# Fedomn/sqlrs

Hardware: AMD Instinct MI355X
Metric: Mrows/sec for filter->hash-join->group-by pipeline; achieved HBM GB/s vs peak (higher is better)
Workload: dtype int64 keys / f64 sum; 1 GPU; C5 filter(val>0.5) -> hash-join(fact x dim on int64 key) -> group-by(key) COUNT,SUM(f64); fact_rows=1000000000, dim_rows=10000000, groups=10000000, parallelism=single GPU

## Files before the change

### sqlrs_amd/csrc/agg_partition.hip

```cpp
#include <algorithm>
#include <cstdlib>
#include <cstring>

#include "agg_partition.hpp"
#include "device_utils.hpp"
#include "radix_part.hpp"

namespace sq {

#ifndef PART_WG_N
#define PART_WG_N 512
#endif
constexpr int PART_WG = PART_WG_N;
#ifndef DENSE_WG_N
#define DENSE_WG_N 1024
#endif
constexpr int DENSE_WG = DENSE_WG_N;
#ifndef HOT_MIN_PEERS_N
#define HOT_MIN_PEERS_N 8
#endif
constexpr int HOT_MIN_PEERS = HOT_MIN_PEERS_N;
constexpr uint64_t LDS_EMPTY = ~0ull;

__device__ __forceinline__ uint32_t bucket_of(uint64_t h, uint32_t P) {
// ... 196 lines not shown
}

struct SplitTables {
  unsigned long long *key = nullptr;
  unsigned int *first = nullptr;
  unsigned long long *acc = nullptr;
  uint32_t nsplit = 0;
};

__global__ void split_init_kernel(SplitTables stb, int64_t total, int n_acc, LdsAggParams prm) {
  int64_t i = blockIdx.x * (int64_t)blockDim.x + threadIdx.x;
  if (i >= total) return;
  stb.key[i] = LDS_EMPTY;
  stb.first[i] = 0xffffffffu;
  for (int a = 0; a < n_acc; a++) stb.acc[(size_t)a * total + i] = acc_identity_cell(prm.code[a] & 7);
}

__global__ void split_emit_kernel(SplitTables stb, uint32_t nslots, uint32_t cap, int n_acc,
                                  unsigned long long *out_count, uint64_t *__restrict__ gkey,
                                  uint32_t *__restrict__ gfirst, uint8_t *__restrict__ gvalid,
                                  uint64_t *__restrict__ gacc, int64_t gcap) {
  const int64_t total = (int64_t)stb.nsplit * nslots;
  int64_t i = blockIdx.x * (int64_t)blockDim.x + threadIdx.x;
  if (i >= total) return;
  unsigned int first = stb.first[i];
  if (first == 0xffffffffu) return;
  const uint32_t s = (uint32_t)(i % nslots);
  unsigned long long base = atomicAdd(out_count, 1ull);
  if ((int64_t)base >= gcap) return;
  gkey[base] = s == cap + 1 ? LDS_EMPTY : stb.key[i];
  gfirst[base] = first;
  if (gvalid) gvalid[base] = s == cap ? 0 : 1;
  for (int a = 0; a < n_acc; a++) gacc[(size_t)a * gcap + base] = stb.acc[(size_t)a * total + i];
}

template <int NV, bool FLAGS, bool JOIN, int NACC, int C0, int C1, bool PACK, bool REC = false>
__global__ __launch_bounds__(PART_WG) void lds_agg_kernel(
    LdsAggParams prm, const uint64_t *__restrict__ pk, const uint32_t *__restrict__ pi,
    const uint64_t *__restrict__ pv0, const uint64_t *__restrict__ pv1,
    const uint8_t *__restrict__ pf, const uint32_t *__restrict__ work , uint32_t P,
    int64_t n, unsigned long long *out_count, uint64_t *__restrict__ gkey,
    uint32_t *__restrict__ gfirst, uint8_t *__restrict__ gvalid, uint64_t *__restrict__ gacc,
    int64_t gcap, unsigned long long *ov_count, uint32_t *__restrict__ ov_rows,
    const uint64_t *__restrict__ bk, const uint8_t *__restrict__ bf, const uint32_t *__restrict__ bbstart,
    KeyPack kp, SplitTables stb) {
  extern __shared__ __attribute__((aligned(16))) unsigned long long tab[];
  __shared__ unsigned int s_cnt, s_join_fail;
  __shared__ unsigned long long s_base;
  const uint32_t b = work[4 * blockIdx.x];
  const int64_t lo = work[4 * blockIdx.x + 1];
  const int64_t hi = work[4 * blockIdx.x + 2];
  const uint32_t split = work[4 * blockIdx.x + 3];
  const uint32_t cap = prm.cap, mask = cap - 1, nslots = cap + 2;
  const int n_acc = NACC >= 0 ? NACC : prm.n_acc;
  auto code_of = [&](int a) { return NACC >= 0 ? (a == 0 ? C0 : C1) : prm.code[a]; };
  unsigned long long *tkey = tab;
  unsigned long long *tacc = tab + nslots;
  unsigned int *tfirst = (unsigned int *)(tacc + (size_t)n_acc * nslots);
  AggRows<NV> cur, nxt;
  if (lo < hi) {
    if (REC) lds_agg_load_rec<NV>(pk, lo + threadIdx.x, hi, cur);
    else lds_agg_load<NV, FLAGS, PACK>(pk, pi, pv0, pv1, pf, lo + threadIdx.x, hi, cur);
  }
  for (uint32_t s = threadIdx.x; s < nslots; s += PART_WG) {
    tkey[s] = LDS_EMPTY;
    tfirst[s] = 0xffffffffu;
#pragma unroll
    for (int a = 0; a < PART_MAX_ACC; a++) {
      if (a >= n_acc) break;
      tacc[(size_t)a * nslots + s] = acc_identity_cell(code_of(a) & 7);
    }
  }
  if (threadIdx.x == 0) {
    s_cnt = 0;
    s_join_fail = 0;
  }
  __syncthreads();
  if (JOIN) {
    if (*(volatile unsigned long long *)(ov_count + 1) != 0) return;
    const int64_t blo = bbstart[b], bhi = bbstart[b + 1];
    for (int64_t i = blo + threadIdx.x; i < bhi; i += PART_WG) {
      uint64_t key = bk[i];
      bool valid = bf ? (bf[i] & 1) : true;
      if (!valid) {
        if (atomicExch(&tkey[cap], 1ull) != LDS_EMPTY) s_join_fail = 1;
      } else if (key == LDS_EMPTY) {
        if (atomicExch(&tkey[cap + 1], 1ull) != LDS_EMPTY) s_join_fail = 1;
      } else {
        uint32_t s = slot_hash(key) & mask;
        uint32_t probes = 0;
        while (true) {
          unsigned long long prev = atomicCAS(&tkey[s], LDS_EMPTY, (unsigned long long)key);
          if (prev == key) s_join_fail = 1;
          if (prev == LDS_EMPTY || prev == key) break;
          s = (s + 1) & mask;
          if (++probes >= cap) {
            s_join_fail = 1;
            break;
          }
        }
      }
    }
    __syncthreads();
    if (s_join_fail) {
      if (threadIdx.x == 0) atomicExch(ov_count + 1, 1ull);
      return;
    }
  }
  __builtin_amdgcn_s_waitcnt(0x0F70);
  for (int64_t base = lo; base < hi; base += (int64_t)LDS_U * PART_WG) {
    const int64_t i0 = base + threadIdx.x;
    if (REC) lds_agg_load_rec<NV>(pk, i0 + (int64_t)LDS_U * PART_WG, hi, nxt);
    else lds_agg_load<NV, FLAGS, PACK>(pk, pi, pv0, pv1, pf, i0 + (int64_t)LDS_U * PART_WG, hi, nxt);
    uint32_t slot[LDS_U];
    unsigned long long seen[LDS_U];
    uint32_t sentinel = 0;
    if (PACK) {
#pragma unroll
      for (int u = 0; u < LDS_U; u++) {
        if (!JOIN && packed_off(kp, cur.k[u]) == kp.kmask) sentinel |= 1u << u;
        cur.id[u] = packed_row(kp, cur.k[u]);
        cur.k[u] = packed_key(kp, cur.k[u]);
      }
    }
#pragma unroll
    for (int u = 0; u < LDS_U; u++) {
      uint32_t s = slot_hash(cur.k[u]) & mask;
      if (FLAGS && !(cur.f[u] & 1)) s = cap;
      else if (cur.k[u] == LDS_EMPTY) s = cap + 1;
      slot[u] = s;
      seen[u] = tkey[s];
    }
#pragma unroll
    for (int u = 0; u < LDS_U; u++) {
      bool act = i0 + (int64_t)u * PART_WG < hi && !((sentinel >> u) & 1u);
      const uint64_t key = cur.k[u];
      uint32_t s = slot[u];
      unsigned long long c = seen[u];
      if (act) {
        if (s >= cap) {
          if (JOIN && c == LDS_EMPTY) act = false;
        } else if (JOIN) {
          uint32_t probes = 0;
          while (c != key && c != LDS_EMPTY && ++probes < cap) {
            s = (s + 1) & mask;
            c = tkey[s];
          }
          if (c != key) act = false;
        } else {
          uint32_t probes = 0;
          while (true) {
            if (c == key) break;
            if (c == LDS_EMPTY) {
              unsigned long long prev = atomicCAS(&tkey[s], LDS_EMPTY, (unsigned long long)key);
              if (prev == LDS_EMPTY || prev == key) break;
            }
            s = (s + 1) & mask;
            if (++probes >= cap) {
              unsigned long long o = atomicAdd(ov_count, 1ull);
              ov_rows[o] = cur.id[u];
              act = false;
              break;
            }
            c = tkey[s];
          }
        }
      }
      const uint64_t actm = __ballot(act);
      if (actm) {
        const int first = __builtin_ctzll(actm);
        const uint32_t s0 = (uint32_t)__shfl((int)s, first, 64);
        const bool hot = act && s == s0;
        const uint64_t peers = __ballot(hot);
        if (__popcll(peers) >= HOT_MIN_PEERS) {
          const uint32_t idmin = wave_min_u32_dpp(hot ? cur.id[u] : 0xffffffffu);
          if (lane_id() == first) atomicMin(&tfirst[s0], idmin);
#pragma unroll
          for (int a = 0; a < PART_MAX_ACC; a++) {
            if (a >= n_acc) break;
            const int code = code_of(a), kind = code & 7, src = code >> 3;
            const bool in = hot && (!FLAGS || (cur.f[u] & (2 << src)));
            const uint64_t v = (NV >= 2 && src) ? cur.v1[u] : cur.v0[u];
            unsigned long long *cell = tacc + (size_t)a * nslots + s0;
            const uint64_t inm = __ballot(in);
            uint64_t red;
            switch (kind) {
            case AK_COUNT: red = (uint64_t)__popcll(inm); break;
            case AK_SUM_I64: red = wave_sum_u64_dpp(in ? v : 0ull); break;
            case AK_SUM_F64: red = (uint64_t)__double_as_longlong(wave_sum_f64_dpp(in ? __longlong_as_double((long long)v) : 0.0)); break;
            case AK_MIN_I64: red = wave_min_u64(in ? i64_to_ordered((int64_t)v) : ~0ull); break;
            case AK_MIN_F64: red = wave_min_u64(in ? f64_to_ordered(__longlong_as_double((long long)v)) : ~0ull); break;
            case AK_MAX_I64: red = wave_max_u64(in ? i64_to_ordered((int64_t)v) : 0ull); break;
            default: red = wave_max_u64(in ? f64_to_ordered(__longlong_as_double((long long)v)) : 0ull);
            }
            if (lane_id() == first && inm) {
              switch (kind) {
              case AK_COUNT:
              case AK_SUM_I64: atomicAdd(cell, (unsigned long long)red); break;
              case AK_SUM_F64: unsafeAtomicAdd((double *)cell, __longlong_as_double((long long)red)); break;
              case AK_MIN_I64:
              case AK_MIN_F64: atomicMin(cell, (unsigned long long)red); break;
              default: atomicMax(cell, (unsigned long long)red);
              }
            }
          }
          act = act && !hot;
        }
      }
      if (act) {
        if (cur.id[u] < tfirst[s]) atomicMin(&tfirst[s], cur.id[u]);
#pragma unroll
        for (int a = 0; a < PART_MAX_ACC; a++) {
          if (a >= n_acc) break;
          const int code = code_of(a);
          const int src = code >> 3;
          if (FLAGS && !(cur.f[u] & (2 << src))) continue;
          uint64_t v = (NV >= 2 && src) ? cur.v1[u] : cur.v0[u];
          acc_apply(code & 7, tacc + (size_t)a * nslots + s, v);
        }
      }
    }
    cur = nxt;
  }
  __syncthreads();
  if (split != 0xffffffffu) {
    unsigned long long *gk = stb.key + (size_t)split * nslots;
    unsigned int *gf = stb.first + (size_t)split * nslots;
    for (uint32_t s = threadIdx.x; s < nslots; s += PART_WG) {
      unsigned int first = tfirst[s];
      if (first == 0xffffffffu) continue;
      uint32_t g = s;
      bool placed = true;
      if (s < cap) {
        const unsigned long long key = tkey[s];
        g = slot_hash(key) & mask;
        uint32_t probes = 0;
        while (true) {
          unsigned long long prev = atomicCAS(&gk[g], LDS_EMPTY, key);
          if (prev == LDS_EMPTY || prev == key) break;
          g = (g + 1) & mask;
          if (++probes >= cap) {
            placed = false;
            break;
          }
        }
      }
      if (!placed) {
        unsigned long long o = atomicAdd(out_count, 1ull);
        if ((int64_t)o < gcap) {
          gkey[o] = tkey[s];
          gfirst[o] = first;
          if (gvalid) gvalid[o] = 1;
#pragma unroll
          for (int a = 0; a < PART_MAX_ACC; a++) {
            if (a >= n_acc) break;
            gacc[(size_t)a * gcap + o] = tacc[(size_t)a * nslots + s];
          }
        }
        atomicExch(ov_count + 2, 1ull);
        continue;
      }
      atomicMin(&gf[g], first);
#pragma unroll
      for (int a = 0; a < PART_MAX_ACC; a++) {
        if (a >= n_acc) break;
        unsigned long long *cell = stb.acc + ((size_t)a * stb.nsplit + split) * nslots + g;
        const unsigned long long v = tacc[(size_t)a * nslots + s];
        switch (code_of(a) & 7) {
        case AK_COUNT:
        case AK_SUM_I64: atomicAdd(cell, v); break;
        case AK_SUM_F64: unsafeAtomicAdd((double *)cell, __longlong_as_double((long long)v)); break;
        case AK_MIN_I64:
        case AK_MIN_F64: atomicMin(cell, v); break;
        default: atomicMax(cell, v);
        }
      }
    }
    return;
  }
  unsigned int mine = 0;
  for (uint32_t s = threadIdx.x; s < nslots; s += PART_WG) mine += tfirst[s] != 0xffffffffu;
  unsigned int my_off = atomicAdd(&s_cnt, mine);
  __syncthreads();
  if (threadIdx.x == 0) s_base = atomicAdd(out_count, (unsigned long long)s_cnt);
  __syncthreads();
  unsigned long long base = s_base + my_off;
  for (uint32_t s = threadIdx.x; s < nslots; s += PART_WG) {
    unsigned int first = tfirst[s];
    if (first == 0xffffffffu) continue;
    if ((int64_t)base < gcap) {
      gkey[base] = s == cap + 1 ? LDS_EMPTY : tkey[s];
      gfirst[base] = first;
      if (gvalid) gvalid[base] = s == cap ? 0 : 1;
#pragma unroll
      for (int a = 0; a < PART_MAX_ACC; a++) {
        if (a >= n_acc) break;
        gacc[(size_t)a * gcap + base] = tacc[(size_t)a * nslots + s];
      }
    }
    base++;
  }
}

constexpr int SED_SLOTS = 16, SED_GROUPS = 16;
__global__ __launch_bounds__(SED_SLOTS * SED_GROUPS) void split_emit_dense_kernel(
    SplitTables stb, const uint32_t *__restrict__ split_bucket, const uint32_t *__restrict__ chunk_lo, uint32_t nbuckets_split,
    uint32_t R, KeyPack kp, LdsAggParams prm, int n_acc, unsigned long long *out_count, uint64_t *__restrict__ gkey,
    uint32_t *__restrict__ gfirst, uint64_t *__restrict__ gacc, int64_t gcap) {
  __shared__ unsigned int s_first[SED_GROUPS][SED_SLOTS];
  __shared__ unsigned long long s_acc[PART_MAX_ACC][SED_GROUPS][SED_SLOTS];
  const uint32_t tiles_per_bucket = (R + SED_SLOTS - 1) / SED_SLOTS;
  const uint32_t t = blockIdx.x / tiles_per_bucket, sl = threadIdx.x % SED_SLOTS, cg = threadIdx.x / SED_SLOTS;
  const uint32_t s = (blockIdx.x % tiles_per_bucket) * SED_SLOTS + sl;
  if (t >= nbuckets_split) return;
  const int64_t total = (int64_t)stb.nsplit * R;
  unsigned int first = 0xffffffffu;
  unsigned long long acc[PART_MAX_ACC];
  for (int a = 0; a < n_acc; a++) acc[a] = acc_identity_cell(prm.code[a] & 7);
  if (s < R) {
    const uint32_t c1 = chunk_lo[t + 1];
    for (uint32_t c = chunk_lo[t] + cg; c < c1; c += SED_GROUPS) {
      const unsigned int f = stb.first[(size_t)c * R + s];
      if (f == 0xffffffffu) continue;
      first = min(first, f);
      for (int a = 0; a < n_acc; a++) {
        const unsigned long long v = stb.acc[(size_t)a * total + (size_t)c * R + s];
        switch (prm.code[a] & 7) {
        case AK_COUNT:
        case AK_SUM_I64: acc[a] += v; break;
        case AK_SUM_F64: acc[a] = (unsigned long long)__double_as_longlong(__longlong_as_double((long long)acc[a]) + __longlong_as_double((long long)v)); break;
        case AK_MIN_I64:
        case AK_MIN_F64: acc[a] = min(acc[a], v); break;
        default: acc[a] = max(acc[a], v);
        }
      }
    }
  }
  s_first[cg][sl] = first;
  for (int a = 0; a < n_acc; a++) s_acc[a][cg][sl] = acc[a];
  __syncthreads();
  if (cg != 0 || s >= R) return;
  for (int g = 1; g < SED_GROUPS; g++) {
    const unsigned int f = s_first[g][sl];
    if (f == 0xffffffffu) continue;
    first = min(first, f);
    for (int a = 0; a < n_acc; a++) {
      const unsigned long long v = s_acc[a][g][sl];
      switch (prm.code[a] & 7) {
      case AK_COUNT:
      case AK_SUM_I64: acc[a] += v; break;
      case AK_SUM_F64: acc[a] = (unsigned long long)__double_as_longlong(__longlong_as_double((long long)acc[a]) + __longlong_as_double((long long)v)); break;
      case AK_MIN_I64:
      case AK_MIN_F64: acc[a] = min(acc[a], v); break;
      default: acc[a] = max(acc[a], v);
      }
    }
  }
  if (first == 0xffffffffu) return;
  unsigned int mlt = 1;
  if (prm.partner_mult) mlt = prm.partner_mult[((uint64_t)split_bucket[t] << kp.rbits) + s];
  unsigned long long base = atomicAdd(out_count, 1ull);
  if ((int64_t)base >= gcap) return;
  gkey[base] = kp.kmin + ((uint64_t)split_bucket[t] << kp.rbits) + s;
  gfirst[base] = first;
  for (int a = 0; a < n_acc; a++) gacc[(size_t)a * gcap + base] = prm.partner_mult ? acc_times(prm.code[a] & 7, acc[a], mlt) : acc[a];
}

template <int NV, bool JOIN, int NACC, int C0, int C1, bool REC = false>
__global__ __launch_bounds__(DENSE_WG) void lds_agg_dense_kernel(
    LdsAggParams prm, const uint64_t *__restrict__ pk, const uint64_t *__restrict__ pv0,
    const uint32_t *__restrict__ work, unsigned long long *out_count, uint64_t *__restrict__ gkey,
    uint32_t *__restrict__ gfirst, uint64_t *__restrict__ gacc, int64_t gcap, KeyPack kp, SplitTables stb) {
  extern __shared__ __attribute__((aligned(16))) unsigned long long tab[];
  __shared__ unsigned int s_cnt;
  __shared__ unsigned long long s_base;
  const uint32_t b = work[4 * blockIdx.x];
  const int64_t lo = work[4 * blockIdx.x + 1];
  const int64_t hi = work[4 * blockIdx.x + 2];
  const uint32_t split = work[4 * blockIdx.x + 3];
  const uint32_t R = prm.cap, mask = R - 1;
  const int n_acc = NACC >= 0 ? NACC : prm.n_acc;
  auto code_of = [&](int a) { return NACC >= 0 ? (a == 0 ? C0 : C1) : prm.code[a]; };
  unsigned long long *tacc = tab;
  unsigned int *tfirst = (unsigned int *)(tacc + (size_t)n_acc * R);
  AggRows<NV> cur, nxt;
  if (lo < hi) {
    if (REC) lds_agg_load_rec<NV, DENSE_WG>(pk, lo + threadIdx.x, hi, cur);
    else lds_agg_load<NV, false, true, DENSE_WG>(pk, nullptr, pv0, nullptr, nullptr, lo + threadIdx.x, hi, cur);
  }
  for (uint32_t s = threadIdx.x; s < R; s += DENSE_WG) {
    tfirst[s] = 0xffffffffu;
#pragma unroll
    for (int a = 0; a < PART_MAX_ACC; a++) {
      if (a >= n_acc) break;
      tacc[(size_t)a * R + s] = acc_identity_cell(code_of(a) & 7);
    }
  }
  if (threadIdx.x == 0) s_cnt = 0;
  __syncthreads();
  uint32_t hc_slot = 0xffffffffu, hc_min = 0xffffffffu;
  uint64_t hc_acc[PART_MAX_ACC];
  auto hot_flush = [&]() {
    if (hc_slot == 0xffffffffu) return;
    if (lane_id() == 0) {
      atomicMin(&tfirst[hc_slot], hc_min);
#pragma unroll
      for (int a = 0; a < PART_MAX_ACC; a++) {
        if (a >= n_acc) break;
        unsigned long long *cell = tacc + (size_t)a * R + hc_slot;
        switch (code_of(a) & 7) {
        case AK_COUNT:
        case AK_SUM_I64: atomicAdd(cell, (unsigned long long)hc_acc[a]); break;
        case AK_SUM_F64: unsafeAtomicAdd((double *)cell, __longlong_as_double((long long)hc_acc[a])); break;
        case AK_MIN_I64:
        case AK_MIN_F64: atomicMin(cell, (unsigned long long)hc_acc[a]); break;
        default: atomicMax(cell, (unsigned long long)hc_acc[a]);
        }
      }
    }
    hc_slot = 0xffffffffu;
  };
  auto hot_take = [&](uint32_t s0, uint32_t idmin) {
    if (hc_slot != s0) {
      hot_flush();
      hc_slot = s0;
      hc_min = 0xffffffffu;
#pragma unroll
      for (int a = 0; a < PART_MAX_ACC; a++) {
        if (a >= n_acc) break;
        hc_acc[a] = acc_identity_cell(code_of(a) & 7);
      }
    }
    hc_min = idmin < hc_min ? idmin : hc_min;
  };
  auto hot_add = [&](int a, int kind, uint64_t red) {
    switch (kind) {
    case AK_COUNT:
    case AK_SUM_I64: hc_acc[a] += red; break;
    case AK_SUM_F64: hc_acc[a] = (uint64_t)__double_as_longlong(__longlong_as_double((long long)hc_acc[a]) + __longlong_as_double((long long)red)); break;
    case AK_MIN_I64:
    case AK_MIN_F64: hc_acc[a] = red < hc_acc[a] ? red : hc_acc[a]; break;
    default: hc_acc[a] = red > hc_acc[a] ? red : hc_acc[a];
    }
  };
  __builtin_amdgcn_s_waitcnt(0x0F70);
  for (int64_t base = lo; base < hi; base += (int64_t)LDS_U * DENSE_WG) {
    const int64_t i0 = base + threadIdx.x;
    if (REC) lds_agg_load_rec<NV, DENSE_WG>(pk, i0 + (int64_t)LDS_U * DENSE_WG, hi, nxt);
    else lds_agg_load<NV, false, true, DENSE_WG>(pk, nullptr, pv0, nullptr, nullptr, i0 + (int64_t)LDS_U * DENSE_WG, hi, nxt);
#pragma unroll
    for (int u = 0; u < LDS_U; u++) {
      const uint64_t off = packed_off(kp, cur.k[u]);
      const uint32_t id = packed_row(kp, cur.k[u]);
      const uint32_t s = (uint32_t)off & mask;
      bool act = i0 + (int64_t)u * DENSE_WG < hi;
      act = act && off <= kp.range;
      const uint64_t actm = __ballot(act);
      if (actm) {
        const int first = __builtin_ctzll(actm);
        const uint32_t s0 = (uint32_t)__shfl((int)s, first, 64);
        const bool hot = act && s == s0;
        const uint64_t peers = __ballot(hot);
        if (__popcll(peers) >= HOT_MIN_PEERS) {
          const uint32_t idmin = wave_min_u32_dpp(hot ? id : 0xffffffffu);
          hot_take(s0, idmin);
#pragma unroll
          for (int a = 0; a < PART_MAX_ACC; a++) {
            if (a >= n_acc) break;
            const int kind = code_of(a) & 7;
            const uint64_t v = NV >= 1 ? cur.v0[u] : 0ull;
            uint64_t red;
            switch (kind) {
            case AK_COUNT: red = (uint64_t)__popcll(peers); break;
            case AK_SUM_I64: red = wave_sum_u64_dpp(hot ? v : 0ull); break;
            case AK_SUM_F64: red = (uint64_t)__double_as_longlong(wave_sum_f64_dpp(hot ? __longlong_as_double((long long)v) : 0.0)); break;
            case AK_MIN_I64: red = wave_min_u64(hot ? i64_to_ordered((int64_t)v) : ~0ull); break;
            case AK_MIN_F64: red = wave_min_u64(hot ? f64_to_ordered(__longlong_as_double((long long)v)) : ~0ull); break;
            case AK_MAX_I64: red = wave_max_u64(hot ? i64_to_ordered((int64_t)v) : 0ull); break;
            default: red = wave_max_u64(hot ? f64_to_ordered(__longlong_as_double((long long)v)) : 0ull);
            }
            hot_add(a, kind, red);
          }
          act = act && !hot;
        }
      }
      if (act) {
        if (id < tfirst[s]) atomicMin(&tfirst[s], id);
#pragma unroll
        for (int a = 0; a < PART_MAX_ACC; a++) {
          if (a >= n_acc) break;
          acc_apply(code_of(a) & 7, tacc + (size_t)a * R + s, NV >= 1 ? cur.v0[u] : 0ull);
        }
      }
    }
    cur = nxt;
  }
  hot_flush();
  __syncthreads();
  if (JOIN && (prm.partner_bits || prm.partner_mult)) {
    const uint64_t off0 = (uint64_t)b << kp.rbits;
    for (uint32_t s = threadIdx.x; s < R; s += DENSE_WG) {
      if (tfirst[s] == 0xffffffffu) continue;
      const uint64_t o = off0 + s;
      const bool partner = prm.partner_mult ? prm.partner_mult[o] != 0 : (((prm.partner_bits[o >> 6] >> (o & 63)) & 1ull) != 0);
      if (!partner) tfirst[s] = 0xffffffffu;
    }
  }
  if (split != 0xffffffffu) {
    unsigned int *gf = stb.first + (size_t)split * R;
    for (uint32_t s = threadIdx.x; s < R; s += DENSE_WG) {
      gf[s] = tfirst[s];
#pragma unroll
      for (int a = 0; a < PART_MAX_ACC; a++) {
        if (a >= n_acc) break;
        stb.acc[((size_t)a * stb.nsplit + split) * R + s] = tacc[(size_t)a * R + s];
      }
    }
    return;
  }
  unsigned int mine = 0;
  for (uint32_t s = threadIdx.x; s < R; s += DENSE_WG) mine += tfirst[s] != 0xffffffffu;
  unsigned int my_off = atomicAdd(&s_cnt, mine);
  __syncthreads();
  if (threadIdx.x == 0) s_base = atomicAdd(out_count, (unsigned long long)s_cnt);
  __syncthreads();
  unsigned long long base = s_base + my_off;
  const uint64_t key0 = kp.kmin + ((uint64_t)b << kp.rbits);
  for (uint32_t s = threadIdx.x; s < R; s += DENSE_WG) {
    unsigned int first = tfirst[s];
    if (first == 0xffffffffu) continue;
    if ((int64_t)base < gcap) {
      gkey[base] = key0 + s;
      gfirst[base] = first;
      const unsigned int mlt = (JOIN && prm.partner_mult) ? prm.partner_mult[((uint64_t)b << kp.rbits) + s] : 1u;
#pragma unroll
      for (int a = 0; a < PART_MAX_ACC; a++) {
        if (a >= n_acc) break;
        const unsigned long long cell = tacc[(size_t)a * R + s];
        gacc[(size_t)a * gcap + base] = (JOIN && prm.partner_mult) ? acc_times(code_of(a) & 7, cell, mlt) : cell;
      }
    }
    base++;
  }
}

struct SlimBucketIn {
  SlimRowsView rows;
  const uint32_t *nzstart, *nzbt, *nzcount, *bcol;
  uint32_t tile;
  uint32_t groups;
  const uint32_t *blk_bt;
  uint32_t log_b;
};
constexpr uint32_t SLIM_BT_CAP = 4096;
struct SlimAggRows {
  uint64_t v[LDS_U];
  uint32_t w[LDS_U], bt[LDS_U];
};

template <bool JOIN, int NACC, int C0, int C1, bool BLK = false>
__global__ __launch_bounds__(DENSE_WG) void lds_agg_dense_slim_kernel(
    LdsAggParams prm, SlimBucketIn in, const uint32_t *__restrict__ work, unsigned long long *out_count,
    uint64_t *__restrict__ gkey, uint32_t *__restrict__ gfirst, uint64_t *__restrict__ gacc, int64_t gcap, KeyPack kp,
    SplitTables stb) {
  extern __shared__ __attribute__((aligned(16))) unsigned long long tab[];
  __shared__ unsigned int s_cnt, s_before, s_inside;
  __shared__ unsigned long long s_base;
  __shared__ uint32_t s_wsum[DENSE_WG / 64];
  const uint32_t b = work[4 * blockIdx.x];
  const int64_t lo = work[4 * blockIdx.x + 1];
  const int64_t hi = work[4 * blockIdx.x + 2];
  const uint32_t split = work[4 * blockIdx.x + 3];
  const uint32_t R = prm.cap, mask = R - 1;
  const int n_acc = NACC >= 0 ? NACC : prm.n_acc;
  auto code_of = [&](int a) { return NACC >= 0 ? (a == 0 ? C0 : C1) : prm.code[a]; };
  unsigned long long *tacc = tab;
  unsigned int *tfirst = (unsigned int *)(tacc + (size_t)n_acc * R);
  unsigned long long *gmask = (unsigned long long *)(tfirst + R);
  uint32_t *gpre = (uint32_t *)(gmask + in.groups);
  uint32_t *gbt = gpre + in.groups;
  const uint32_t col = BLK ? 0u : in.bcol[b], nruns = BLK ? 0u : in.nzcount[b];
  const uint32_t ngroups = BLK ? 0u : (uint32_t)((hi - lo + 63) >> 6);
  const uint64_t le_mask = (2ull << lane_id()) - 1ull;
  const uint32_t rbits = kp.rbits, lmask = (1u << 13) - 1u;

  for (uint32_t s = threadIdx.x; s < R; s += DENSE_WG) {
    tfirst[s] = 0xffffffffu;
#pragma unroll
    for (int a = 0; a < PART_MAX_ACC; a++) {
      if (a >= n_acc) break;
      tacc[(size_t)a * R + s] = acc_identity_cell(code_of(a) & 7);
    }
  }
  for (uint32_t g = threadIdx.x; g < ngroups; g += DENSE_WG) gmask[g] = 0;
  if (threadIdx.x == 0) {
    s_cnt = 0;
    s_before = 0;
    s_inside = 0;
  }
  __syncthreads();
  if (!BLK) {
    uint32_t before = 0, inside = 0;
    for (uint32_t k = threadIdx.x; k < nruns; k += DENSE_WG) {
      const int64_t st = in.nzstart[col + k];
      if (st <= lo) before++;
      else if (st < hi) {
        inside++;
        atomicOr(&gmask[(st - lo) >> 6], 1ull << ((st - lo) & 63));
      }
    }
    before = wave_sum_u32(before);
    inside = wave_sum_u32(inside);
    if (lane_id() == 0 && before) atomicAdd(&s_before, before);
    if (lane_id() == 0 && inside) atomicAdd(&s_inside, inside);
  }
  __syncthreads();
  const uint32_t k_first = s_before - 1u, k_count = s_inside + 1u;
  const bool bt_lds = !BLK && k_count <= SLIM_BT_CAP;
  const bool seg_mode = NACC == 2 && ((C0 == AK_COUNT && C1 == AK_SUM_F64) || (C0 == AK_SUM_F64 && C1 == AK_COUNT)) &&
                        hi - lo >= 4096 && (int64_t)k_count * 2048 <= hi - lo && !prm.seg_off && !BLK;
  if (bt_lds)
    for (uint32_t k = threadIdx.x; k < k_count; k += DENSE_WG) gbt[k] = in.nzbt[col + min(k_first + k, nruns - 1)];
  if (!BLK) {
    constexpr uint32_t GPT = 8;
    uint32_t carry = s_before - 1u;
    for (uint32_t g0 = 0; g0 < ngroups; g0 += DENSE_WG * GPT) {
      const uint32_t gb = g0 + threadIdx.x * GPT;
      uint32_t pc[GPT], sum = 0;
#pragma unroll
      for (uint32_t i = 0; i < GPT; i++) {
        pc[i] = gb + i < ngroups ? (uint32_t)__popcll(gmask[gb + i]) : 0u;
        sum += pc[i];
      }
      const uint32_t inc = wave_iscan_u32(sum);
      if (lane_id() == 63) s_wsum[wave_id()] = inc;
      __syncthreads();
      uint32_t wbase = 0, tot = 0;
      for (int w = 0; w < DENSE_WG / 64; w++) {
        if (w < wave_id()) wbase += s_wsum[w];
        tot += s_wsum[w];
      }
      uint32_t run = carry + wbase + inc - sum;
#pragma unroll
      for (uint32_t i = 0; i < GPT; i++) {
        if (gb + i < ngroups) gpre[gb + i] = run;
        run += pc[i];
      }
      carry += tot;
      __syncthreads();
    }
  }
#ifndef SLIM_WAVE_SPAN
#define SLIM_WAVE_SPAN 1
#endif
  constexpr int64_t SLIM_USTEP = SLIM_WAVE_SPAN ? 64 : DENSE_WG;
  const int64_t slim_toff = SLIM_WAVE_SPAN ? (int64_t)wave_id() * (LDS_U * 64) + lane_id() : (int64_t)threadIdx.x;
  auto load = [&](int64_t i0, SlimAggRows &r) {
#pragma unroll
    for (int u = 0; u < LDS_U; u++) {
      const int64_t i = min(i0 + (int64_t)u * SLIM_USTEP, hi - 1);
      slim_load_nt(in.rows, i, r.w[u], r.v[u]);
      if (BLK) {
        r.bt[u] = in.blk_bt[i >> in.log_b];
        continue;
      }
      const uint32_t g = (uint32_t)((i - lo) >> 6);
      const uint32_t k = gpre[g] + (uint32_t)__popcll(gmask[g] & le_mask);
#if defined(SLIM_DBG) && (SLIM_DBG & 16)
      r.bt[u] = k;
#else
      r.bt[u] = bt_lds ? gbt[min(k - k_first, k_count - 1)] : in.nzbt[col + min(k, nruns - 1)];
#endif
    }
  };
  uint32_t hc_slot = 0xffffffffu, hc_min = 0xffffffffu;
  uint64_t hc_acc[PART_MAX_ACC];
  auto hot_flush = [&]() {
    if (hc_slot == 0xffffffffu) return;
    if (lane_id() == 0) {
      atomicMin(&tfirst[hc_slot], hc_min);
#pragma unroll
      for (int a = 0; a < PART_MAX_ACC; a++) {
        if (a >= n_acc) break;
        unsigned long long *cell = tacc + (size_t)a * R + hc_slot;
        switch (code_of(a) & 7) {
        case AK_COUNT:
        case AK_SUM_I64: atomicAdd(cell, (unsigned long long)hc_acc[a]); break;
        case AK_SUM_F64: unsafeAtomicAdd((double *)cell, __longlong_as_double((long long)hc_acc[a])); break;
        case AK_MIN_I64:
        case AK_MIN_F64: atomicMin(cell, (unsigned long long)hc_acc[a]); break;
        default: atomicMax(cell, (unsigned long long)hc_acc[a]);
        }
      }
    }
    hc_slot = 0xffffffffu;
  };
  auto hot_take = [&](uint32_t s0, uint32_t idmin) {
    if (hc_slot != s0) {
      hot_flush();
      hc_slot = s0;
      hc_min = 0xffffffffu;
#pragma unroll
      for (int a = 0; a < PART_MAX_ACC; a++) {
        if (a >= n_acc) break;
        hc_acc[a] = acc_identity_cell(code_of(a) & 7);
      }
    }
    hc_min = idmin < hc_min ? idmin : hc_min;
  };
  auto hot_add = [&](int a, int kind, uint64_t red) {
    switch (kind) {
    case AK_COUNT:
    case AK_SUM_I64: hc_acc[a] += red; break;
    case AK_SUM_F64: hc_acc[a] = (uint64_t)__double_as_longlong(__longlong_as_double((long long)hc_acc[a]) + __longlong_as_double((long long)red)); break;
    case AK_MIN_I64:
    case AK_MIN_F64: hc_acc[a] = red < hc_acc[a] ? red : hc_acc[a]; break;
    default: hc_acc[a] = red > hc_acc[a] ? red : hc_acc[a];
    }
  };
  SlimAggRows cur, nxt;
  if (lo < hi) load(lo + slim_toff, cur);
  __builtin_amdgcn_s_waitcnt(0x0F70);
  for (int64_t base = lo; base < hi; base += (int64_t)LDS_U * DENSE_WG) {
    const int64_t i0 = base + slim_toff;
    load(i0 + (int64_t)LDS_U * DENSE_WG, nxt);
    uint32_t sl[LDS_U], id[LDS_U], tf[LDS_U];
#pragma unroll
    for (int u = 0; u < LDS_U; u++) {
      const uint32_t w = cur.w[u];
      sl[u] = w & mask;
      id[u] = (cur.bt[u] + (w >> (rbits + 13))) * in.tile + ((w >> rbits) & lmask);
      tf[u] = tfirst[sl[u]];
    }
    constexpr bool SEG_CAPABLE = NACC == 2 && ((C0 == AK_COUNT && C1 == AK_SUM_F64) || (C0 == AK_SUM_F64 && C1 == AK_COUNT));
    const int lane = (int)lane_id();
    auto seg_rows = [&](bool act, uint32_t sl_u, uint64_t v_u, uint32_t id_u, uint32_t tf_u) {
      const uint32_t key = act ? sl_u : (0x80000000u | (uint32_t)lane);
      const uint32_t prevk = (uint32_t)__builtin_amdgcn_update_dpp(0, (int)key, 0x138, 0xf, 0xf, false);
      const uint64_t bm = __ballot(lane == 0 || key != prevk);
      const int headl = 63 - __builtin_clzll(bm & le_mask);
      double incl = act ? __longlong_as_double((long long)v_u) : 0.0;
      uint32_t idh = act ? id_u : 0xffffffffu;
      wave_seg_iscan_f64_min_u32(incl, idh, headl, lane);
      const bool tail = act && (lane == 63 || ((bm >> (lane + 1)) & 1ull));
      if (tail) {
        const uint32_t s = sl_u;
        if (idh < tf_u) atomicMin(&tfirst[s], idh);
        atomicAdd(tacc + (size_t)(C0 == AK_COUNT ? 0 : 1) * R + s, (unsigned long long)(lane - headl + 1));
        unsafeAtomicAdd((double *)(tacc + (size_t)(C0 == AK_COUNT ? 1 : 0) * R + s), incl);
      }
    };
    if (seg_mode) {
#pragma unroll
      for (int u = 0; u < LDS_U; u++) {
        const bool act = i0 + (int64_t)u * SLIM_USTEP < hi;
        {
          const uint32_t s0 = (uint32_t)__builtin_amdgcn_readfirstlane((int)sl[u]);
          if (__ballot(act && sl[u] == s0) == ~0ull) {
            hot_take(s0, wave_min_u32_dpp(id[u]));
            hot_add(C0 == AK_COUNT ? 0 : 1, AK_COUNT, 64ull);
            hot_add(C0 == AK_COUNT ? 1 : 0, AK_SUM_F64, (uint64_t)__double_as_longlong(wave_sum_f64_dpp(__longlong_as_double((long long)cur.v[u]))));
            continue;
          }
        }
        seg_rows(act, sl[u], cur.v[u], id[u], tf[u]);
      }
      cur = nxt;
      continue;
    }
#pragma unroll
    for (int u = 0; u < LDS_U; u++) {
      const uint32_t s = sl[u];
      bool act = i0 + (int64_t)u * SLIM_USTEP < hi;
      if (BLK) act = act && cur.w[u] != 0xffffffffu;
#ifdef SLIM_DBG
      uint64_t actm = (SLIM_DBG & 1) ? 0ull : __ballot(act);
#else
      uint64_t actm = __ballot(act);
#endif
      for (int it = 0; it < 3 && actm; it++) {
        const int first = __builtin_ctzll(actm);
        const uint32_t s0 = (uint32_t)__builtin_amdgcn_readlane((int)s, first);
        const bool hot = act && s == s0;
        const uint64_t peers = __ballot(hot);
        if (__popcll(peers) < HOT_MIN_PEERS) break;
        if (SEG_CAPABLE && it == 0 && peers != actm && (((peers >> first) + 1) & (peers >> first)) == 0 && !prm.seg_off) {
          seg_rows(act, s, cur.v[u], id[u], tf[u]);
          act = false;
          break;
        }
        const uint32_t idmin = wave_min_u32_dpp(hot ? id[u] : 0xffffffffu);
        hot_take(s0, idmin);
#pragma unroll
        for (int a = 0; a < PART_MAX_ACC; a++) {
          if (a >= n_acc) break;
          const int kind = code_of(a) & 7;
          const uint64_t v = cur.v[u];
          uint64_t red;
          switch (kind) {
          case AK_COUNT: red = (uint64_t)__popcll(peers); break;
          case AK_SUM_I64: red = wave_sum_u64_dpp(hot ? v : 0ull); break;
          case AK_SUM_F64: red = (uint64_t)__double_as_longlong(wave_sum_f64_dpp(hot ? __longlong_as_double((long long)v) : 0.0)); break;
          case AK_MIN_I64: red = wave_min_u64(hot ? i64_to_ordered((int64_t)v) : ~0ull); break;
          case AK_MIN_F64: red = wave_min_u64(hot ? f64_to_ordered(__longlong_as_double((long long)v)) : ~0ull); break;
          case AK_MAX_I64: red = wave_max_u64(hot ? i64_to_ordered((int64_t)v) : 0ull); break;
          default: red = wave_max_u64(hot ? f64_to_ordered(__longlong_as_double((long long)v)) : 0ull);
          }
          hot_add(a, kind, red);
        }
        act = act && !hot;
        actm &= ~peers;
      }
      if (act) {
#ifdef SLIM_DBG
        if (!(SLIM_DBG & 8) && id[u] < tf[u]) atomicMin(&tfirst[s], id[u]);
#pragma unroll
        for (int a = 0; a < PART_MAX_ACC; a++) {
          if (a >= n_acc) break;
          if ((SLIM_DBG >> (1 + a)) & 1) continue;
          acc_apply(code_of(a) & 7, tacc + (size_t)a * R + s, cur.v[u]);
        }
#else
        if (id[u] < tf[u]) atomicMin(&tfirst[s], id[u]);
#pragma unroll
        for (int a = 0; a < PART_MAX_ACC; a++) {
          if (a >= n_acc) break;
          acc_apply(code_of(a) & 7, tacc + (size_t)a * R + s, cur.v[u]);
        }
#endif
      }
    }
    cur = nxt;
  }
  hot_flush();
  __syncthreads();
  if (JOIN && (prm.partner_bits || prm.partner_mult)) {
    const uint64_t off0 = (uint64_t)b << kp.rbits;
    for (uint32_t s = threadIdx.x; s < R; s += DENSE_WG) {
      if (tfirst[s] == 0xffffffffu) continue;
      const uint64_t o = off0 + s;
      const bool partner = prm.partner_mult ? prm.partner_mult[o] != 0 : (((prm.partner_bits[o >> 6] >> (o & 63)) & 1ull) != 0);
      if (!partner) tfirst[s] = 0xffffffffu;
    }
  }
  if (split != 0xffffffffu) {
    unsigned int *gf = stb.first + (size_t)split * R;
    for (uint32_t s = threadIdx.x; s < R; s += DENSE_WG) {
      gf[s] = tfirst[s];
#pragma unroll
      for (int a = 0; a < PART_MAX_ACC; a++) {
        if (a >= n_acc) break;
        stb.acc[((size_t)a * stb.nsplit + split) * R + s] = tacc[(size_t)a * R + s];
      }
    }
    return;
  }
  unsigned int mine = 0;
  for (uint32_t s = threadIdx.x; s < R; s += DENSE_WG) mine += tfirst[s] != 0xffffffffu;
  unsigned int my_off = atomicAdd(&s_cnt, mine);
  __syncthreads();
  if (threadIdx.x == 0) s_base = atomicAdd(out_count, (unsigned long long)s_cnt);
  __syncthreads();
  unsigned long long obase = s_base + my_off;
  const uint64_t key0 = kp.kmin + ((uint64_t)b << kp.rbits);
  for (uint32_t s = threadIdx.x; s < R; s += DENSE_WG) {
    unsigned int first = tfirst[s];
    if (first == 0xffffffffu) continue;
    if ((int64_t)obase < gcap) {
      gkey[obase] = key0 + s;
      gfirst[obase] = first;
      const unsigned int mlt = (JOIN && prm.partner_mult) ? prm.partner_mult[((uint64_t)b << kp.rbits) + s] : 1u;
#pragma unroll
      for (int a = 0; a < PART_MAX_ACC; a++) {
        if (a >= n_acc) break;
        const unsigned long long cell = tacc[(size_t)a * R + s];
        gacc[(size_t)a * gcap + obase] = (JOIN && prm.partner_mult) ? acc_times(code_of(a) & 7, cell, mlt) : cell;
      }
    }
    obase++;
  }
}

__global__ void first_to_rowid_kernel(const uint32_t *__restrict__ gfirst, int64_t n, uint64_t offset,
                                      uint64_t *__restrict__ out) {
  int64_t i = blockIdx.x * (int64_t)blockDim.x + threadIdx.x;
  if (i < n) out[i] = offset + gfirst[i];
}
__global__ void bytes_pack_kernel(const uint8_t *__restrict__ bytes, int64_t n, uint64_t *__restrict__ out) {
  int64_t i = blockIdx.x * (int64_t)blockDim.x + threadIdx.x;
  bool b = (i < n) && bytes[i];
  uint64_t m = __ballot(b);
  if (lane_id() == 0 && i < n) out[i >> 6] = m;
}

__global__ __launch_bounds__(256) void key_range_kernel(const uint64_t *__restrict__ keys, int64_t n, unsigned long long *mm) {
  uint64_t kmin = ~0ull, kmax = 0;
  for (int64_t r = blockIdx.x * (int64_t)blockDim.x + threadIdx.x; r < n; r += (int64_t)gridDim.x * blockDim.x) {
    const uint64_t o = keys[r] ^ (1ull << 63);
    kmin = min(kmin, o);
    kmax = max(kmax, o);
  }
  kmin = wave_min_u64(kmin);
  kmax = wave_max_u64(kmax);
  __shared__ unsigned long long s_lo[4], s_hi[4];
  if (lane_id() == 0) {
    s_lo[wave_id()] = kmin;
    s_hi[wave_id()] = kmax;
  }
  __syncthreads();
  if (threadIdx.x == 0) {
    for (int w = 1; w < 4; w++) {
      kmin = min(kmin, (uint64_t)s_lo[w]);
      kmax = max(kmax, (uint64_t)s_hi[w]);
    }
    atomicMin(mm, (unsigned long long)kmin);
    atomicMax(mm + 1, (unsigned long long)kmax);
  }
}

const uint64_t *part_row_ids(Ctx *ctx, PartAggOutput &po) {
  if (!po.row_ids) {
    const int64_t g1 = std::max<int64_t>(po.groups, 1);
    po.row_ids = ctx->alloc(8 * (size_t)g1);
    if (po.groups) {
      first_to_rowid_kernel<<<dim3((unsigned)ceil_div(g1, 256)), dim3(256), 0, ctx->stream>>>(
          po.gfirst->as<uint32_t>(), po.groups, po.row_offset, po.row_ids->as<uint64_t>());
      SQ_HIP(hipGetLastError());
    }
  }
  return po.row_ids->as<uint64_t>();
}

bool partitioned_preaggregate(Ctx *ctx, const PartAggSpec &spec, const PartAggInput &in,
                              uint64_t row_offset, PartAggOutput *out) {
  int64_t n = in.n;
  if (n > 0xffffffffll || spec.n_acc > PART_MAX_ACC || spec.nv > 2) return false;
  const bool join_mode = in.join_keys != nullptr;
  uint64_t omin = ~0ull, omax = 0;
  bool sampled = false;
  const char *kse = hook("SQLRS_KEY_STATS_EXACT");
  const bool stats_exact_env = kse && kse[0] == '1';
  double est = join_mode ? (double)in.join_n
                         : estimate_distinct(ctx, in.keys, in.key_validity, n, &omin, &omax, (in.exact_stats || stats_exact_env) ? nullptr : &sampled);
  BufP ctr = ctx->alloc_zero(48);
  if (sampled && omin <= omax) {
    const uint64_t w = omax - omin, pad = std::max<uint64_t>(w / 8, 65536);
    omin = omin >= pad ? omin - pad : 0;
    omax = omax <= ~0ull - pad ? omax + pad : ~0ull;
  }
  static const double est_scale = [] {
    const char *e = hook("SQLRS_EST_SCALE");
    return e ? std::atof(e) : 1.0;
  }();
  if (!join_mode) est = std::max(1.0, est * est_scale);
  KeyPack kp;
  const bool nullable = in.key_validity || in.val_validity[0] || in.val_validity[1];
  if (!nullable && spec.nv <= 1 && !(join_mode && in.join_validity)) {
    if (join_mode && in.join_range_known) {
      omin = in.join_omin;
      omax = in.join_omax;
    } else if (join_mode) {
      BufP mm = ctx->alloc(16);
      SQ_HIP(hipMemsetAsync(mm->p, 0xff, 8, ctx->stream));
      SQ_HIP(hipMemsetAsync(mm->as<uint8_t>() + 8, 0, 8, ctx->stream));
      unsigned blocks = (unsigned)std::min<int64_t>(ceil_div(in.join_n, 1024), 1024);
      key_range_kernel<<<dim3(std::max(blocks, 1u)), dim3(256), 0, ctx->stream>>>(
          in.join_keys, in.join_n, mm->as<unsigned long long>());
      SQ_HIP(hipGetLastError());
      const uint64_t *h = (const uint64_t *)ctx->fetch(mm->p, 16);
      omin = h[0];
      omax = h[1];
    }
    if (omin <= omax) {
      uint64_t range = omax - omin;
      uint32_t kbits = 1;
      while (kbits < 64 && ((1ull << kbits) - 1) <= range) kbits++;
      int rowbits = 1;
      while (rowbits < 32 && (1ll << rowbits) < n) rowbits++;
      if (kbits + rowbits <= 64) {
        kp.kbits = kbits;
        kp.kmask = (1ull << kbits) - 1;
        kp.kmin = omin ^ (1ull << 63);
        if (sampled) {
          kp.oob = (unsigned int *)(ctr->as<uint64_t>() + 4);
          out->ov_rows = ctx->alloc(4 * (size_t)std::max<int64_t>(n, 1));
          kp.ov_rows = out->ov_rows->as<uint32_t>();
          kp.ov_count = ctr->as<unsigned long long>() + 1;
          kp.ov_cap = (uint32_t)std::min<int64_t>(n, std::max<int64_t>(65536, n / 1024));
        }
      }
    }
  }
  constexpr size_t lds_budget = 72 * 1024;
  const size_t slot_bytes = 8 + 8 * (size_t)spec.n_acc + 4;
  uint32_t cap = 1;
  while ((size_t)(cap * 2 + 2) * slot_bytes <= lds_budget) cap *= 2;
  constexpr double load_factor = 0.275;
  const double groups_per_table = cap * load_factor;
  double want = est * 1.15 / groups_per_table;
  if (!join_mode) est = std::min(est, (double)n);
  const char *dense_e = hook("SQLRS_DENSE_AGG");
  const bool dense_on = !(dense_e && dense_e[0] == '0');
  const uint64_t *partner_bits = nullptr;
  const double want_hashed = want;
  bool dense = false;
  if (dense_on && kp.kbits) {
    const uint64_t range = omax - omin;
    constexpr size_t dense_budget = 150 * 1024;
    const size_t dslot = 8 * (size_t)spec.n_acc + 4;
    uint32_t rbits = 8;
    while (rbits < 14 && ((size_t)2 << rbits) * dslot <= dense_budget) rbits++;
    while (rbits > 8 && (range >> (rbits - 1)) == 0) rbits--;
    const uint64_t pd = (range >> rbits) + 1;
    const bool fills = join_mode ? (in.join_unique_known && (range + 1 == (uint64_t)in.join_n ||
                                                             ((in.join_bits || in.join_mult) && in.join_range_known && range / 16 <= (uint64_t)in.join_n)))
                                 : ((double)range + 1.0 <= 4.0 * est);
    partner_bits = (join_mode && fills && !in.join_mult && range + 1 != (uint64_t)in.join_n) ? in.join_bits : nullptr;
    if (fills && pd <= 65536 && (double)pd <= 1.5 * std::max(1.0, std::ceil(want))) {
      dense = true;
      kp.dense = 1;
      kp.rbits = rbits;
      kp.range = range;
      cap = 1u << rbits;
      want = (double)pd;
    }
  }
  if (join_mode && in.join_mult && !dense) return false;
  if (want > 65536.0) return false;
  uint32_t P = (uint32_t)std::max(1.0, std::ceil(want));
  out->est_groups = est;
  PartitionInput pin;
  pin.pack = kp;
  pin.filter = in.filter;
  pin.keys = in.keys;
  pin.key_validity = in.key_validity;
  pin.n = n;
  pin.nv = spec.nv;
  for (int k = 0; k < 2; k++) {
    pin.vals[k] = in.vals[k];
    pin.val_validity[k] = in.val_validity[k];
  }
  PartitionedRows pr;
  const bool in_place = P == 1 && !join_mode && !nullable && want_hashed <= 1.0 && !in.filter.col;
  if (in_place) {
    dense = false;
    kp = KeyPack();
    cap = 1;
    while ((size_t)(cap * 2 + 2) * slot_bytes <= lds_budget) cap *= 2;
    pr.n = n;
    pr.P = 1;
    auto borrowed = [&](const void *p) {
      BufP b = std::make_shared<Buf>(ctx, const_cast<void *>(p), 0);
      b->owned = false;
      return b;
    };
    pr.key = borrowed(in.keys);
    pr.v0 = spec.nv >= 1 ? borrowed(in.vals[0]) : nullptr;
    pr.v1 = spec.nv >= 2 ? borrowed(in.vals[1]) : nullptr;
    pr.bstart_host = {0u, (uint32_t)n};
    pr.bstart = nullptr;
  } else if (!partition_rows(ctx, pin, P, &pr)) {
    return false;
  }
  P = pr.P;
  n = pr.n;
  if (dense != (pr.pack.dense != 0)) return false;
  if (n == 0) {
    out->groups = out->n_overflow = 0;
    out->gcap = 1;
    out->buckets = (int)P;
    out->gkey = ctx->alloc(8);
    out->gfirst = ctx->alloc(4);
    out->gacc = ctx->alloc(8 * (size_t)std::max(spec.n_acc, 1));
    out->ov_rows = ctx->alloc(4);
    out->row_ids = nullptr;
    out->row_offset = row_offset;
    return true;
  }
  out->buckets = (int)P;
  BufP pk = pr.key, pi = pr.idx, pv0 = pr.v0, pv1 = pr.v1, pf = pr.flags;
  PartitionedRows local_build;
  const PartitionedRows *bp = nullptr;
  if (join_mode && !dense) {
    if (in.join_cache && in.join_cache->P == P && in.join_cache->n == in.join_n) {
      bp = in.join_cache;
    } else {
      PartitionInput bin;
      bin.keys = in.join_keys;
      bin.key_validity = in.join_validity;
      bin.n = in.join_n;
      bin.nv = 0;
      bin.build_side = true;
      PartitionedRows *dst = in.join_cache ? in.join_cache : &local_build;
      if (!partition_rows(ctx, bin, P, dst) || dst->P != P) return false;
      bp = dst;
    }
  }
  LdsAggParams prm;
  prm.n_acc = spec.n_acc;
  for (int a = 0; a < PART_MAX_ACC; a++) {
    int kind = AK_COUNT;
    if (a < spec.n_acc) {
      switch (spec.op[a]) {
      case PART_COUNT: kind = AK_COUNT; break;
      case PART_SUM_I64: kind = AK_SUM_I64; break;
      case PART_SUM_F64: kind = AK_SUM_F64; break;
      case PART_MIN: kind = spec.kind[a] ? AK_MIN_F64 : AK_MIN_I64; break;
      default: kind = spec.kind[a] ? AK_MAX_F64 : AK_MAX_I64;
      }
    }
    prm.code[a] = a < spec.n_acc ? (kind | (spec.src[a] << 3)) : 0;
  }
  prm.cap = cap;
  prm.partner_bits = dense ? (const unsigned long long *)partner_bits : nullptr;
  prm.partner_mult = (dense && join_mode) ? in.join_mult : nullptr;
  {
    const char *seg_e = hook("SQLRS_AGG_SEG");
    prm.seg_off = (seg_e && seg_e[0] == '0') ? 1 : 0;
  }
  int64_t gcap = (int64_t)std::min<double>((double)n, est * 1.5 + 65536.0 + 2.0 * P);
  if (dense) gcap = (int64_t)std::min<uint64_t>((uint64_t)n, join_mode ? (uint64_t)in.join_n : kp.range + 1);
  size_t lds = dense ? round_up((size_t)cap * (slot_bytes - 8), 16) : round_up((size_t)(cap + 2) * slot_bytes, 16);
  const std::vector<uint32_t> &hb = pr.bstart_host;
  if (hb.size() != (size_t)P + 1) return false;
  uint32_t chunk = (uint32_t)std::max<int64_t>(32768, 2 * (n / std::max<uint32_t>(P, 1)));
  uint32_t split_above = chunk;
  if (dense) {
    int64_t nonempty_d = 0;
    for (uint32_t bkt = 0; bkt < P; bkt++) nonempty_d += pr.bucket_end(bkt) > hb[bkt];
    const int64_t avg = n / std::max<int64_t>(nonempty_d, 1);
    const char *cd_e = hook("SQLRS_DENSE_CHUNK_DIV");
    const int cdiv = cd_e ? std::max(1, std::atoi(cd_e)) : 2;
    constexpr int sa_pct = 125;
    chunk = (uint32_t)std::max<int64_t>(32768, avg / cdiv);
    split_above = (uint32_t)std::max<int64_t>(65536, avg * sa_pct / 100);
  }
  {
    const uint32_t slots = (lds > 80 * 1024 - 64 ? 1u : 2u) * (uint32_t)ctx->num_cus;
    uint32_t nonempty = 0;
    for (uint32_t bkt = 0; bkt < P; bkt++) nonempty += pr.bucket_end(bkt) > hb[bkt];
    if (nonempty < slots / 2) {
      chunk = (uint32_t)std::max<int64_t>(32768, n / (2 * (int64_t)slots));
      split_above = chunk;
    }
  }
  if (pr.slim.on && !pr.slim.blk_bt) {
    const size_t table = round_up((size_t)cap * (slot_bytes - 8), 16);
    const size_t room = 159 * 1024 > table + 4 * SLIM_BT_CAP ? 159 * 1024 - table - 4 * SLIM_BT_CAP : 0;
    const uint32_t item_rows = (uint32_t)std::min<size_t>(1u << 18, (room / 12 > 2 ? room / 12 - 2 : 0) * 64);
    if (item_rows < 16384) return false;
    chunk = std::min(chunk, item_rows);
    split_above = std::min(split_above, item_rows);
  }
  std::vector<uint32_t> work, split_bucket, chunk_lo;
  work.reserve(4 * ((size_t)P + 64));
  out->may_dup = false;
  uint32_t nsplit = 0, nchunk_tables = 0;
  for (uint32_t bkt = 0; bkt < P; bkt++) {
    uint32_t lo = hb[bkt], hi = pr.bucket_end(bkt);
    if (dense && lo == hi) continue;
    if (hi - lo <= split_above) {
      work.insert(work.end(), {bkt, lo, hi, 0xffffffffu});
    } else if (dense) {
      chunk_lo.push_back(nchunk_tables);
      const uint32_t pieces = (uint32_t)ceil_div((int64_t)(hi - lo), (int64_t)chunk);
      for (uint32_t q = 0; q < pieces; q++) {
        const uint32_t c0 = lo + (uint32_t)((uint64_t)(hi - lo) * q / pieces), c1 = lo + (uint32_t)((uint64_t)(hi - lo) * (q + 1) / pieces);
        work.insert(work.end(), {bkt, c0, c1, nchunk_tables++});
      }
      split_bucket.push_back(bkt);
      nsplit++;
    } else {
      for (uint32_t c0 = lo; c0 < hi; c0 += chunk) work.insert(work.end(), {bkt, c0, std::min(hi, c0 + chunk), nsplit});
      split_bucket.push_back(bkt);
      nsplit++;
    }
  }
  chunk_lo.push_back(nchunk_tables);
  if (nsplit) {
    std::vector<uint32_t> ord(work.size() / 4), sorted(work.size());
    for (uint32_t i = 0; i < ord.size(); i++) ord[i] = i;
    std::stable_sort(ord.begin(), ord.end(), [&](uint32_t a, uint32_t b) {
      return work[4 * a + 2] - work[4 * a + 1] > work[4 * b + 2] - work[4 * b + 1];
    });
    for (size_t i = 0; i < ord.size(); i++) std::memcpy(&sorted[4 * i], &work[4 * ord[i]], 16);
    work.swap(sorted);
  }
  const uint32_t nwork = (uint32_t)(work.size() / 4);
  BufP dwork = ctx->alloc(4 * work.size() + 16);
  SQ_HIP(hipMemcpyAsync(dwork->p, work.data(), 4 * work.size(), hipMemcpyHostToDevice, ctx->stream));
  const uint32_t nslots_h = dense ? cap : cap + 2;
  SplitTables stb;
  BufP stb_key, stb_first, stb_acc, dsplit;
  BufP dchunk_lo;
  if (nsplit && dense) {
    const int64_t total = (int64_t)nchunk_tables * nslots_h;
    stb_first = ctx->alloc(4 * (size_t)total);
    stb_acc = ctx->alloc(8 * (size_t)total * (size_t)std::max(spec.n_acc, 1));
    stb.first = stb_first->as<unsigned int>();
    stb.acc = stb_acc->as<unsigned long long>();
    stb.nsplit = nchunk_tables;
    dsplit = ctx->alloc(4 * (size_t)nsplit);
    dchunk_lo = ctx->alloc(4 * ((size_t)nsplit + 1));
    SQ_HIP(hipMemcpyAsync(dsplit->p, split_bucket.data(), 4 * (size_t)nsplit, hipMemcpyHostToDevice, ctx->stream));
    SQ_HIP(hipMemcpyAsync(dchunk_lo->p, chunk_lo.data(), 4 * ((size_t)nsplit + 1), hipMemcpyHostToDevice, ctx->stream));
  } else if (nsplit) {
    const int64_t total = (int64_t)nsplit * nslots_h;
    stb_key = ctx->alloc(8 * (size_t)total);
    stb_first = ctx->alloc(4 * (size_t)total);
    stb_acc = ctx->alloc(8 * (size_t)total * (size_t)std::max(spec.n_acc, 1));
    stb.key = stb_key->as<unsigned long long>();
    stb.first = stb_first->as<unsigned int>();
    stb.acc = stb_acc->as<unsigned long long>();
    stb.nsplit = nsplit;
    split_init_kernel<<<dim3((unsigned)ceil_div(total, 256)), dim3(256), 0, ctx->stream>>>(stb, total, spec.n_acc, prm);
    SQ_HIP(hipGetLastError());
  }
  out->gkey = ctx->alloc(8 * (size_t)gcap);
  out->gfirst = ctx->alloc(4 * (size_t)gcap);
  out->gvalid = in.key_validity ? ctx->alloc((size_t)gcap) : nullptr;
  out->gacc = ctx->alloc(8 * (size_t)gcap * (size_t)std::max(spec.n_acc, 1));
  out->gcap = gcap;
  if (!out->ov_rows) out->ov_rows = ctx->alloc(4 * (size_t)std::max<int64_t>(n, 1));
  ctx->agg_route[pr.pack.kbits ? Ctx::AR_PACKED : Ctx::AR_UNPACKED]++;
  ctx->agg_route[Ctx::AR_FLAGS] += pf != nullptr;
  ctx->agg_route[Ctx::AR_REC] += pr.rec != nullptr;
  ctx->agg_route[Ctx::AR_IN_PLACE] += in_place;
  ctx->agg_route[Ctx::AR_JOIN] += join_mode;
  ctx->agg_route[Ctx::AR_JOIN_MULT] += prm.partner_mult != nullptr;
  ctx->agg_route[Ctx::AR_SPLIT] += nsplit > 0;
  {
    ProfScope ps(ctx, "lds_agg");
#define SQ_LA(NV, FL, JN, NA, C0, C1, PK)                                                                        \
  do {                                                                                                         \
    auto kfn = lds_agg_kernel<NV, FL, JN, NA, C0, C1, PK>;                                                      \
    constexpr bool can_rec = NV == 1 && PK && !FL;                                                             \
    if (can_rec && pr.rec) kfn = lds_agg_kernel<NV, FL, JN, NA, C0, C1, PK, can_rec>;                          \
    else if (pr.rec) fail(SQLRS_ERR_INTERNAL, "record-form partition in a column-form bucket pass");           \
    allow_big_lds(ctx, kfn);                                                                                   \
    kfn<<<dim3(nwork), dim3(PART_WG), lds, ctx->stream>>>(                                                     \
        prm, pr.rec ? pr.rec->as<uint64_t>() : pk->as<uint64_t>(), pi ? pi->as<uint32_t>() : nullptr, pv0 ? pv0->as<uint64_t>() : nullptr,       \
        pv1 ? pv1->as<uint64_t>() : nullptr, pf ? pf->as<uint8_t>() : nullptr, dwork->as<uint32_t>(), P, n,    \
        ctr->as<unsigned long long>(), out->gkey->as<uint64_t>(), out->gfirst->as<uint32_t>(),                 \
        out->gvalid ? out->gvalid->as<uint8_t>() : nullptr, out->gacc->as<uint64_t>(), gcap,                   \
        ctr->as<unsigned long long>() + 1, out->ov_rows->as<uint32_t>(),                                       \
        bp ? bp->key->as<uint64_t>() : nullptr, (bp && bp->flags) ? bp->flags->as<uint8_t>() : nullptr,        \
        bp ? bp->bstart->as<uint32_t>() : nullptr, pr.pack, stb);                                              \
    ctx->agg_route[NA < 0 ? Ctx::AR_PROBE_GENERIC : Ctx::AR_PROBE_SPEC]++;                                     \
    launched = true;                                                                                           \
  } while (0)
#define SQ_LA_J(NV, FL, NA, C0, C1)                                                                            \
  do {                                                                                                         \
    if (pr.pack.kbits) {                                                                                       \
      if (join_mode) SQ_LA(NV, FL, true, NA, C0, C1, true);                                                    \
      else SQ_LA(NV, FL, false, NA, C0, C1, true);                                                             \
    } else {                                                                                                   \
      if (join_mode) SQ_LA(NV, FL, true, NA, C0, C1, false);                                                   \
      else SQ_LA(NV, FL, false, NA, C0, C1, false);                                                            \
    }                                                                                                          \
  } while (0)
    const int nvu = pv1 ? 2 : ((pv0 || pr.rec) ? 1 : 0);
    bool launched = false;
    if (dense && pr.slim.on) {
      uint32_t max_item = 64;
      for (uint32_t i = 0; i < nwork; i++) max_item = std::max(max_item, work[4 * i + 2] - work[4 * i + 1]);
      const bool blk = pr.slim.blk_bt != nullptr;
      SlimBucketIn sb;
      sb.rows = pr.slim.rows;
      sb.nzstart = blk ? nullptr : pr.slim.nzstart->as<uint32_t>();
      sb.nzbt = blk ? nullptr : pr.slim.nzbt->as<uint32_t>();
      sb.nzcount = blk ? nullptr : pr.slim.nzcount->as<uint32_t>();
      sb.bcol = blk ? nullptr : pr.slim.bcol->as<uint32_t>();
      sb.tile = pr.slim.tile;
      sb.groups = blk ? 0u : (uint32_t)ceil_div((int64_t)max_item, 64) + 1;
      sb.blk_bt = blk ? pr.slim.blk_bt->as<uint32_t>() : nullptr;
      sb.log_b = pr.slim.log_b;
      const size_t slds = round_up((size_t)cap * (slot_bytes - 8), 16) + (blk ? 16 : 12 * (size_t)sb.groups + 4 * SLIM_BT_CAP);
#define SQ_LS(JN, NA, C0, C1)                                                                                  \
  do {                                                                                                         \
    auto kfn = lds_agg_dense_slim_kernel<JN, NA, C0, C1>;                                                       \
    if (blk) kfn = lds_agg_dense_slim_kernel<JN, NA, C0, C1, true>;                                             \
    allow_big_lds(ctx, kfn, 159 * 1024);                                                                                 \
    kfn<<<dim3(nwork), dim3(DENSE_WG), slds, ctx->stream>>>(prm, sb, dwork->as<uint32_t>(), ctr->as<unsigned long long>(), \
                                                           out->gkey->as<uint64_t>(), out->gfirst->as<uint32_t>(), \
                                                           out->gacc->as<uint64_t>(), gcap, pr.pack, stb);        \
    ctx->agg_route[blk ? Ctx::AR_SLIM_BLK : Ctx::AR_SLIM_RUNS]++;                                              \
    ctx->agg_route[Ctx::AR_INTERPRETED] += NA < 0;                                                             \
    launched = true;                                                                                           \
  } while (0)
#define SQ_LS_J(NA, C0, C1) do { if (join_mode) SQ_LS(true, NA, C0, C1); else SQ_LS(false, NA, C0, C1); } while (0)
      const int c0 = prm.code[0], c1 = spec.n_acc == 2 ? prm.code[1] : -1;
      if (spec.n_acc == 2 && c0 == AK_COUNT && c1 == AK_SUM_F64) SQ_LS_J(2, AK_COUNT, AK_SUM_F64);
      else if (spec.n_acc == 2 && c0 == AK_SUM_F64 && c1 == AK_COUNT) SQ_LS_J(2, AK_SUM_F64, AK_COUNT);
      else if (spec.n_acc == 1 && c0 == AK_SUM_F64) SQ_LS_J(1, AK_SUM_F64, 0);
      else if (spec.n_acc == 1 && c0 == AK_COUNT) SQ_LS_J(1, AK_COUNT, 0);
      else SQ_LS_J(-1, 0, 0);
#undef SQ_LS_J
#undef SQ_LS
      if (nsplit) {
        split_emit_dense_kernel<<<dim3((unsigned)(nsplit * ceil_div((int64_t)nslots_h, SED_SLOTS))), dim3(SED_SLOTS * SED_GROUPS), 0, ctx->stream>>>(
            stb, dsplit->as<uint32_t>(), dchunk_lo->as<uint32_t>(), nsplit, cap, pr.pack, prm, spec.n_acc,
            ctr->as<unsigned long long>(), out->gkey->as<uint64_t>(), out->gfirst->as<uint32_t>(), out->gacc->as<uint64_t>(), gcap);
      }
    } else if (dense) {
#define SQ_LD(NV, JN, NA, C0, C1)                                                                              \
  do {                                                                                                         \
    auto kfn = lds_agg_dense_kernel<NV, JN, NA, C0, C1>;                                                        \
    if (NV == 1 && pr.rec) kfn = lds_agg_dense_kernel<NV, JN, NA, C0, C1, NV == 1>;                            \
    allow_big_lds(ctx, kfn);                                                                                   \
    kfn<<<dim3(nwork), dim3(DENSE_WG), lds, ctx->stream>>>(                                                    \
        prm, pr.rec ? pr.rec->as<uint64_t>() : pk->as<uint64_t>(), pv0 ? pv0->as<uint64_t>() : nullptr, dwork->as<uint32_t>(), \
        ctr->as<unsigned long long>(), out->gkey->as<uint64_t>(), out->gfirst->as<uint32_t>(),                 \
        out->gacc->as<uint64_t>(), gcap, pr.pack, stb);                                                        \
    ctx->agg_route[Ctx::AR_DENSE]++;                                                                           \
    ctx->agg_route[Ctx::AR_INTERPRETED] += NA < 0;                                                             \
    launched = true;                                                                                           \
  } while (0)
#define SQ_LD_J(NV, NA, C0, C1) do { if (join_mode) SQ_LD(NV, true, NA, C0, C1); else SQ_LD(NV, false, NA, C0, C1); } while (0)
      if (nvu == 1 && spec.n_acc <= 2) {
        const int c0 = prm.code[0], c1 = spec.n_acc == 2 ? prm.code[1] : -1;
#define SQ_SIG1(K) if (!launched && spec.n_acc == 1 && c0 == K) SQ_LD_J(1, 1, K, 0)
#define SQ_SIG2(K0, K1) if (!launched && spec.n_acc == 2 && c0 == K0 && c1 == K1) SQ_LD_J(1, 2, K0, K1)
        SQ_SIG1(AK_COUNT); SQ_SIG1(AK_SUM_I64); SQ_SIG1(AK_SUM_F64); SQ_SIG1(AK_MIN_I64); SQ_SIG1(AK_MIN_F64);
        SQ_SIG1(AK_MAX_I64); SQ_SIG1(AK_MAX_F64);
        SQ_SIG2(AK_COUNT, AK_SUM_F64); SQ_SIG2(AK_SUM_F64, AK_COUNT);
        SQ_SIG2(AK_COUNT, AK_SUM_I64); SQ_SIG2(AK_SUM_I64, AK_COUNT);
        SQ_SIG2(AK_MIN_F64, AK_MAX_F64); SQ_SIG2(AK_MIN_I64, AK_MAX_I64);
#undef SQ_SIG1
#undef SQ_SIG2
      }
      if (!launched) { if (nvu == 0) SQ_LD_J(0, -1, 0, 0); else SQ_LD_J(1, -1, 0, 0); }
#undef SQ_LD_J
#undef SQ_LD
      if (nsplit) {
        split_emit_dense_kernel<<<dim3((unsigned)(nsplit * ceil_div((int64_t)nslots_h, SED_SLOTS))), dim3(SED_SLOTS * SED_GROUPS), 0, ctx->stream>>>(
            stb, dsplit->as<uint32_t>(), dchunk_lo->as<uint32_t>(), nsplit, cap, pr.pack, prm, spec.n_acc,
            ctr->as<unsigned long long>(), out->gkey->as<uint64_t>(), out->gfirst->as<uint32_t>(), out->gacc->as<uint64_t>(), gcap);
      }
    }
    if (!launched && !pf && nvu == 1 && spec.n_acc <= 2) {
      const int c0 = prm.code[0], c1 = spec.n_acc == 2 ? prm.code[1] : -1;
#define SQ_SIG1(K) if (!launched && spec.n_acc == 1 && c0 == K) SQ_LA_J(1, false, 1, K, 0)
#define SQ_SIG2(K0, K1) if (!launched && spec.n_acc == 2 && c0 == K0 && c1 == K1) SQ_LA_J(1, false, 2, K0, K1)
      SQ_SIG1(AK_COUNT); SQ_SIG1(AK_SUM_I64); SQ_SIG1(AK_SUM_F64); SQ_SIG1(AK_MIN_I64); SQ_SIG1(AK_MIN_F64);
      SQ_SIG1(AK_MAX_I64); SQ_SIG1(AK_MAX_F64);
      SQ_SIG2(AK_COUNT, AK_SUM_F64); SQ_SIG2(AK_SUM_F64, AK_COUNT);
      SQ_SIG2(AK_COUNT, AK_SUM_I64); SQ_SIG2(AK_SUM_I64, AK_COUNT);
      SQ_SIG2(AK_MIN_F64, AK_MAX_F64); SQ_SIG2(AK_MIN_I64, AK_MAX_I64);
#undef SQ_SIG1
#undef SQ_SIG2
    }
    if (!launched) {
      if (pf) { if (nvu == 0) SQ_LA_J(0, true, -1, 0, 0); else if (nvu == 1) SQ_LA_J(1, true, -1, 0, 0); else SQ_LA_J(2, true, -1, 0, 0); }
      else { if (nvu == 0) SQ_LA_J(0, false, -1, 0, 0); else if (nvu == 1) SQ_LA_J(1, false, -1, 0, 0); else SQ_LA_J(2, false, -1, 0, 0); }
    }
#undef SQ_LA_J
#undef SQ_LA
    if (nsplit && !dense) {
      const int64_t total = (int64_t)nsplit * nslots_h;
      split_emit_kernel<<<dim3((unsigned)ceil_div(total, 256)), dim3(256), 0, ctx->stream>>>(
          stb, nslots_h, cap, spec.n_acc, ctr->as<unsigned long long>(), out->gkey->as<uint64_t>(),
          out->gfirst->as<uint32_t>(), out->gvalid ? out->gvalid->as<uint8_t>() : nullptr,
          out->gacc->as<uint64_t>(), gcap);
    }
    SQ_HIP(hipGetLastError());
  }
  const uint64_t *h = (const uint64_t *)ctx->fetch(ctr->p, 40);
  if (h[4]) {
    out->retry_exact = true;
    return false;
  }
  out->groups = (int64_t)h[0];
  out->n_overflow = (int64_t)h[1];
  ctx->agg_route[Ctx::AR_OVERFLOW_ROWS] += out->n_overflow;
  out->may_dup = h[3] != 0;
  if (join_mode && h[2]) return false;
  if (out->groups > gcap) return false;
  int64_t g1 = std::max<int64_t>(out->groups, 1);
  out->row_offset = row_offset;
  out->row_ids = nullptr;
  if (out->groups) {
    if (out->gvalid) {
      out->gvalid_bits = ctx->alloc(bitmap_bytes(g1));
      int64_t g64 = (int64_t)round_up((size_t)g1, 64);
      bytes_pack_kernel<<<dim3((unsigned)ceil_div(g64, 256)), dim3(256), 0, ctx->stream>>>(
          out->gvalid->as<uint8_t>(), out->groups, out->gvalid_bits->as<uint64_t>());
    }
    SQ_HIP(hipGetLastError());
  }
  return true;
}

}
```

### sqlrs_amd/csrc/agg_partition.hpp

```cpp
#pragma once

#include <cmath>

#include "common.hpp"
#include "prims.hpp"
#include "radix_part.hpp"

namespace sq {

constexpr int PART_MAX_ACC = 6;
enum PartOp { PART_COUNT = 0, PART_SUM_I64 = 1, PART_SUM_F64 = 2, PART_MIN = 3, PART_MAX = 4 };

struct PartAggSpec {
  int n_acc = 0;
  int op[PART_MAX_ACC] = {0};
  int src[PART_MAX_ACC] = {0};
  int kind[PART_MAX_ACC] = {0};
  int nv = 0;
};

struct PartAggInput {
  const uint64_t *keys = nullptr;
  const uint64_t *key_validity = nullptr;
  int64_t n = 0;
  const void *vals[2] = {nullptr, nullptr};
  const uint64_t *val_validity[2] = {nullptr, nullptr};
  const uint64_t *join_keys = nullptr;
  const uint64_t *join_validity = nullptr;
  int64_t join_n = 0;
  struct PartitionedRows *join_cache = nullptr;
  bool join_range_known = false;
  uint64_t join_omin = 0, join_omax = 0;
  bool join_unique_known = true;
  const uint64_t *join_bits = nullptr;
  const uint32_t *join_mult = nullptr;
  RowFilter filter;
  bool exact_stats = false;
};

struct PartAggOutput {
  int64_t groups = 0, gcap = 0;
  BufP gkey, gfirst, gvalid, gvalid_bits, gacc;
  BufP row_ids;
  uint64_t row_offset = 0;
  int64_t n_overflow = 0;
  BufP ov_rows;
  bool may_dup = false;
  double est_groups = 0;
  int buckets = 0;
  bool retry_exact = false;
};

const uint64_t *part_row_ids(Ctx *ctx, PartAggOutput &po);
double estimate_distinct(Ctx *ctx, const uint64_t *keys, const uint64_t *validity, int64_t n,
                         uint64_t *omin = nullptr, uint64_t *omax = nullptr, bool *sampled = nullptr);
bool partitioned_preaggregate(Ctx *ctx, const PartAggSpec &spec, const PartAggInput &in,
                              uint64_t row_offset, PartAggOutput *out);

}
```

### sqlrs_amd/csrc/common.hpp

```cpp
#pragma once

#include <hip/hip_runtime.h>

#include <cstdint>
#include <cstdlib>
#include <cstring>
#include <map>
#include <set>
#include <memory>
#include <string>
#include <vector>

#include "sqlrs_hip.h"

namespace sq {

inline bool hooks_enabled() {
  static const bool on = [] {
    const char *e = std::getenv("SQLRS_HOOKS");
    return e && e[0] == '1';
  }();
  return on;
}
inline const char *hook(const char *name) { return hooks_enabled() ? std::getenv(name) : nullptr; }

struct Error {
  int status;
  std::string msg;
};
[[noreturn]] inline void fail(int status, const std::string &m) { throw Error{status, m}; }

#define SQ_HIP(expr)                                                                              \
  do {                                                                                            \
    hipError_t _e = (expr);                                                                       \
    if (_e != hipSuccess)                                                                         \
      ::sq::fail(SQLRS_ERR_DEVICE, std::string(#expr) + ": " + hipGetErrorString(_e));            \
  } while (0)

inline int64_t ceil_div(int64_t a, int64_t b) { return (a + b - 1) / b; }
inline size_t round_up(size_t a, size_t b) { return (a + b - 1) / b * b; }
inline size_t bitmap_bytes(int64_t rows) { return (size_t)ceil_div(rows, 64) * 8; }

inline size_t width_of(int32_t dtype) {
  switch (dtype) {
  case SQLRS_INT32:
  case SQLRS_UINT32:
    return 4;
  case SQLRS_INT64:
  case SQLRS_UINT64:
  case SQLRS_FLOAT64:
    return 8;
  default:
    return 0;
  }
}

struct Pool {
  std::multimap<size_t, void *> free_blocks;
  size_t live_bytes = 0, cached_bytes = 0;
  bool closed = false;
  int device = 0;
  uint8_t *arena = nullptr;
  size_t arena_bytes = 0, arena_used = 0;
  bool in_arena(const void *p) const { return arena && (const uint8_t *)p >= arena && (const uint8_t *)p < arena + arena_bytes; }
  struct VmmBlock {
    std::vector<hipMemGenericAllocationHandle_t> handles;
    size_t size = 0;
  };
  std::map<void *, VmmBlock> vmm_blocks;
  int vmm = -1;
  void *vmm_alloc(size_t want);
  bool vmm_free(void *p);
  void *alloc(size_t bytes, size_t *cap);
  void release(void *p, size_t cap);
  void trim();
};

struct Ctx;
struct Buf {
  Ctx *ctx;
  std::shared_ptr<Pool> pool;
  void *p;
  size_t cap;
  bool owned = true;
  std::shared_ptr<Buf> parent;
  Buf(Ctx *c, void *ptr, size_t n);
  ~Buf();
  Buf(const Buf &) = delete;
  Buf &operator=(const Buf &) = delete;
  template <class T> T *as() const { return (T *)p; }
};
using BufP = std::shared_ptr<Buf>;
inline BufP buf_view(const BufP &parent, const void *p, size_t bytes) {
  BufP v = std::make_shared<Buf>(parent->ctx, const_cast<void *>(p), bytes);
  v->owned = false;
  v->parent = parent;
  return v;
}

struct ProfEntry {
  const char *name;
  double total_ms = 0;
  int64_t launches = 0;
};
struct ProfPending {
  int entry;
  hipEvent_t a, b;
};

struct Ctx {
  int device = 0;
  hipStream_t stream = nullptr;
  std::string last_error;
  std::shared_ptr<Pool> pool_ref = std::make_shared<Pool>();
  Pool &pool = *pool_ref;
  int num_cus = 256;
  bool prof_on = false;
  std::vector<ProfEntry> prof;
  std::vector<ProfPending> prof_pending;
  std::vector<hipEvent_t> event_pool;
  hipEvent_t order_event = nullptr;
  void *pinned = nullptr;
  size_t pinned_bytes = 0;

  BufP alloc(size_t bytes);
  BufP alloc_zero(size_t bytes);
  BufP zero_block;
  size_t zero_used = 0;
  std::set<const void *> big_lds_set;
  std::map<const void *, int> occ_cache;
  int64_t lb_timeouts = 0;
  int64_t order_lb_fallbacks = 0;
  int lb_backoff = 0;
  int64_t async_conj_batches = 0;
  int64_t async_fast_batches = 0;
  enum AggRoute {
    AR_DENSE, AR_SLIM_RUNS, AR_SLIM_BLK, AR_PROBE_SPEC, AR_PROBE_GENERIC,
    AR_INTERPRETED,
    AR_PACKED, AR_UNPACKED,
    AR_FLAGS,
    AR_REC,
    AR_IN_PLACE,
    AR_JOIN,
    AR_JOIN_MULT,
    AR_SPLIT,
    AR_OVERFLOW_ROWS,
    AR_MERGE_GROUPS,
    AR_PENDING,
    AR_WIDE_PARTS,
    AR_COUNT_
  };
  int64_t agg_route[AR_COUNT_] = {};
  enum JoinRoute {
    JR_DENSE_ADOPTED,
    JR_DENSE_REFUSED,
    JR_DENSE_ONE_FETCH, JR_DENSE_TWO_FETCH,
    JR_DENSE_PACKED, JR_DENSE_PLAIN,
    JR_PROBE_PENDING,
    JR_ALLHIT_KEPT, JR_ALLHIT_REDONE,
    JR_COMPACT_DENSE, JR_COMPACT_SLOTS,
    JR_UNIQUE_OUTER,
    JR_DD_STREAM, JR_DD_ROWS,
    JR_COUNTS_GROUPED, JR_COUNTS_PER_ROW,
    JR_LDS_UNIQUE, JR_LDS_DISTINCT,
    JR_TABLE_LATE,
    JR_COUNT_
  };
  int64_t join_route[JR_COUNT_] = {};
  std::shared_ptr<void> small_ring;
  void sync() { SQ_HIP(hipStreamSynchronize(stream)); }
  const void *fetch(const void *dptr, size_t bytes);
  template <class T> T fetch_value(const T *dptr) { return *(const T *)fetch(dptr, sizeof(T)); }
  void *pinned_early = nullptr;
  hipEvent_t early_event = nullptr;
  bool fetch_early(const void *dptr, size_t bytes);
  const void *fetch_early_wait();
  int prof_entry(const char *name);
  void prof_resolve();
};

template <class K> inline void allow_big_lds(Ctx *ctx, K kfn, int bytes = 150 * 1024) {
  const void *f = (const void *)kfn;
  if (ctx->big_lds_set.count(f)) return;
  SQ_HIP(hipFuncSetAttribute(f, hipFuncAttributeMaxDynamicSharedMemorySize, bytes));
  ctx->big_lds_set.insert(f);
}

struct ProfScope {
  Ctx *ctx;
  int entry = -1;
  hipEvent_t a = nullptr, b = nullptr;
  ProfScope(Ctx *c, const char *name);
  ~ProfScope();
};

struct DCol {
  int32_t dtype = SQLRS_NULLTYPE;
  int64_t length = 0;
  int64_t null_count = 0;
  int stride = 1;
  const void *values = nullptr;
  const uint64_t *validity = nullptr;
  const int32_t *offsets = nullptr;
  int64_t data_bytes = 0;
  uint64_t scalar_bits = 0;
  bool scalar_null = false;
  BufP own_values, own_validity, own_offsets;
  bool has_nulls() const { return validity != nullptr && null_count != 0; }
  template <class T> const T *v() const { return (const T *)values; }
};

struct DBatch {
  int64_t rows = 0;
  std::vector<DCol> cols;
};

struct InBatch {
  Ctx *ctx;
  const sqlrs_batch_t *abi;
  std::vector<DCol> cache;
  std::vector<uint8_t> loaded;
  bool host_upload = false;
  const DBatch *shared = nullptr;
  InBatch(Ctx *c, const sqlrs_batch_t *b);
  ~InBatch();
  InBatch(const InBatch &) = delete;
  InBatch &operator=(const InBatch &) = delete;
  int64_t rows() const { return abi->num_rows; }
  int num_columns() const { return abi->num_columns; }
  int32_t dtype(int i) const { return abi->columns[i].dtype; }
  const DCol &col(int i);
  DBatch materialize(bool owned);
};

DCol upload_column(Ctx *ctx, const sqlrs_column_t &c, bool force_copy);
sqlrs_batch_t *emit_batch(Ctx *ctx, DBatch &&b, int out_mem);
sqlrs_batch_t *emit_host_copy(Ctx *ctx, int ncols, const int32_t *dtypes, int64_t rows, const void *const *values,
                              const uint8_t *const *validity, const int64_t *null_counts, const int32_t *const *offsets = nullptr);
sqlrs_batch_t *emit_host_columns(Ctx *ctx, std::vector<sqlrs_column_t> &&cols, int64_t rows);
bool all_fixed_width(const DBatch &b);
void split_rows_to_host(Ctx *ctx, const DBatch &o, const std::vector<int64_t> &cut, void **pin, size_t *pin_cap, int n,
                        sqlrs_batch_t **out);
DCol make_null_column(Ctx *ctx, int32_t dtype, int64_t n);
int64_t count_nulls(Ctx *ctx, const DCol &c);

template <class F> int guard(Ctx *ctx, F &&f) {
  try {
    f();
    return SQLRS_OK;
  } catch (const Error &e) {
    if (ctx) ctx->last_error = e.msg;
    return e.status;
  } catch (const std::exception &e) {
    if (ctx) ctx->last_error = e.what();
    return SQLRS_ERR_INTERNAL;
  }
}

inline int first_lookback_mode() {
  static const int forced = [] {
    const char *e = hook("SQLRS_FORCE_TICKET");
    return (e && e[0] == '1') ? 1 : 0;
  }();
  return forced;
}

constexpr int LB_BACKOFF_CALLS = 64;
inline int lookback_start_mode(Ctx *ctx) {
  if (first_lookback_mode()) return 1;
  if (ctx->lb_backoff > 0) {
    ctx->lb_backoff--;
    return 1;
  }
  return 0;
}
inline void lookback_timed_out(Ctx *ctx) {
  ctx->lb_timeouts++;
  ctx->lb_backoff = LB_BACKOFF_CALLS;
}

struct Expr {
  std::vector<sqlrs_expr_node_t> nodes;
  std::vector<std::string> strings;
  bool empty() const { return nodes.empty(); }
};
Expr expr_from_abi(const sqlrs_expr_t *e);

}

struct sqlrs_ctx : sq::Ctx {};
```

### sqlrs_amd/csrc/ctx.hip

```cpp
#include <cstdlib>

#include <array>
#include <atomic>
#include <mutex>
#include <unordered_set>

#include "common.hpp"
#include "host_stage.hpp"
#include "prims.hpp"
#include "small_async.hpp"

extern "C" void sqlrs_batch_release(sqlrs_batch_t *batch);
namespace sq {

static size_t pool_size_class(size_t bytes) {
  if (bytes < 512) return 512;
  if (bytes <= (1u << 20)) {
    size_t s = 512;
    while (s < bytes) s <<= 1;
    return s;
  }
  return round_up(bytes, (size_t)2 << 20);
}

// ... 896 lines not shown

struct ExportHolder {
  std::atomic<int> refs{0};
  sqlrs_batch_t *batch = nullptr;
  std::vector<ArrowArray> children;
  std::vector<ArrowArray *> child_ptrs;
  std::vector<std::array<const void *, 3>> bufs;
  const void *top_buf[1] = {nullptr};
  void unref() {
    if (refs.fetch_sub(1) == 1) {
      sqlrs_batch_release(batch);
      delete this;
    }
  }
};
void export_child_release(ArrowArray *a) {
  if (!a || !a->release) return;
  ExportHolder *h = (ExportHolder *)a->private_data;
  a->release = nullptr;
  h->unref();
}
void export_parent_release(ArrowArray *a) {
  if (!a || !a->release) return;
  ExportHolder *h = (ExportHolder *)a->private_data;
  for (int64_t i = 0; i < a->n_children; i++)
    if (a->children[i] && a->children[i]->release) a->children[i]->release(a->children[i]);
  a->release = nullptr;
  h->unref();
}
struct SchemaHolder {
  std::vector<ArrowSchema> children;
  std::vector<ArrowSchema *> child_ptrs;
  std::vector<std::string> names;
};
void export_schema_child_release(ArrowSchema *s) {
  if (s) s->release = nullptr;
}
void export_schema_release(ArrowSchema *s) {
  if (!s || !s->release) return;
  SchemaHolder *h = (SchemaHolder *)s->private_data;
  for (int64_t i = 0; i < s->n_children; i++)
    if (s->children[i] && s->children[i]->release) s->children[i]->release(s->children[i]);
  s->release = nullptr;
  delete h;
}
}

int sqlrs_batch_import_arrow(sqlrs_ctx_t *ctx, struct ArrowArray *array, struct ArrowSchema *schema, sqlrs_batch_t **out) {
  if (out) *out = nullptr;
  return guard(ctx, [&] {
    if (!array || !schema || !out || !array->release || !schema->release) fail(SQLRS_ERR_ARROW, "import_arrow: null or released structure");
    if (!schema->format || std::strcmp(schema->format, "+s") != 0) fail(SQLRS_ERR_ARROW, "import_arrow: a struct array (\"+s\", an exported RecordBatch) is expected");
    if (array->n_children != schema->n_children || array->dictionary || array->length < 0 || array->offset < 0)
      fail(SQLRS_ERR_ARROW, "import_arrow: array and schema do not match");
    if (array->null_count > 0 || (array->null_count < 0 && array->n_buffers > 0 && array->buffers && array->buffers[0]))
      fail(SQLRS_ERR_ARROW, "import_arrow: NULL rows at the struct level");
    if (array->length >= (1ll << 31)) fail(SQLRS_ERR_ARROW, "batch num_rows outside [0, 2^31)");
    const int64_t n = array->length;
    const int nc = (int)array->n_children;
    auto o = std::unique_ptr<OwnedBatch>(new OwnedBatch());
    o->ctx = ctx;
    o->out_mem = SQLRS_MEM_HOST;
    o->descs.resize((size_t)nc);
    for (int c = 0; c < nc; c++) {
      const ArrowArray *a = array->children[c];
      const ArrowSchema *sc = schema->children[c];
      const int32_t dt = (a && sc && !a->dictionary) ? arrow_dtype(sc->format) : -1;
      if (dt < 0) fail(SQLRS_ERR_ARROW, std::string("import_arrow: unsupported column type \"") + ((sc && sc->format) ? sc->format : "?") + "\"");
      const int64_t off = array->offset + a->offset;
      if (a->offset < 0 || a->length < array->offset + n) fail(SQLRS_ERR_ARROW, "import_arrow: child shorter than the struct");
      const int64_t need = dt == SQLRS_UTF8 ? 3 : 2;
      if (a->n_buffers < need || !a->buffers) fail(SQLRS_ERR_ARROW, "import_arrow: missing buffers");
      sqlrs_column_t &d = o->descs[(size_t)c];
      d.dtype = dt;
      d.mem = SQLRS_MEM_HOST;
      d.length = n;
      d.values = nullptr;
      d.validity = nullptr;
      d.offsets = nullptr;
      d.null_count = 0;
      if (a->null_count != 0 && a->buffers[0] && n > 0) {
        d.validity = bits_at(a->buffers[0], off, n, o->host_blocks);
        d.null_count = a->null_count > 0 && a->offset == 0 && a->length == n && array->offset == 0 ? a->null_count : clear_bits(d.validity, n);
        if (d.null_count == 0) d.validity = nullptr;
      }
      if (n > 0 && !a->buffers[1] && dt != SQLRS_UTF8) fail(SQLRS_ERR_ARROW, "import_arrow: missing values buffer");
      switch (dt) {
      case SQLRS_BOOLEAN: d.values = bits_at(a->buffers[1], off, n, o->host_blocks); break;
      case SQLRS_UTF8: {
        static const int32_t zero_off[1] = {0};
        const int32_t *po = a->buffers[1] ? (const int32_t *)a->buffers[1] + off : zero_off;
        if (po[0] != 0) {
          int32_t *no = (int32_t *)std::malloc(4 * (size_t)(n + 1) + 8);
          if (!no) fail(SQLRS_ERR_INTERNAL, "host allocation failed");
          o->host_blocks.push_back(no);
          for (int64_t i = 0; i <= n; i++) no[i] = po[i] - po[0];
          d.values = (const uint8_t *)a->buffers[2] + po[0];
          d.offsets = no;
        } else {
          d.offsets = po;
          d.values = a->buffers[2] ? a->buffers[2] : (const void *)zero_off;
        }
        break;
      }
      default: d.values = (const uint8_t *)a->buffers[1] + (size_t)off * width_of(dt);
      }
    }
    o->abi.num_rows = n;
    o->abi.num_columns = nc;
    o->abi.reserved = 0;
    o->abi.columns = o->descs.data();
    o->abi.owner = o.get();
    o->imported = *array;
    array->release = nullptr;
    schema->release(schema);
    *out = &o.release()->abi;
  });
}

int sqlrs_batch_export_arrow(sqlrs_ctx_t *ctx, sqlrs_batch_t *batch, const char *const *names, struct ArrowArray *out_array,
                             struct ArrowSchema *out_schema) {
  return guard(ctx, [&] {
    if (!batch || !out_array || !out_schema) fail(SQLRS_ERR_ARROW, "export_arrow: null argument");
    SQ_HIP(hipSetDevice(ctx->device));
    bool ours = false;
    if (batch->owner) {
      std::lock_guard<std::mutex> lk(g_owned_mu);
      ours = g_owned.count(batch->owner) != 0;
    }
    bool host = true;
    for (int c = 0; c < batch->num_columns; c++) host = host && batch->columns[c].mem == SQLRS_MEM_HOST;
    sqlrs_batch_t *hb = batch;
    if (!ours || !host) {
      InBatch ib(ctx, batch);
      hb = emit_batch(ctx, ib.materialize(true), SQLRS_MEM_HOST);
    }
    const int nc = hb->num_columns;
    for (int c = 0; c < nc; c++)
      if (!arrow_format(hb->columns[c].dtype)) {
        if (hb != batch) sqlrs_batch_release(hb);
        fail(SQLRS_ERR_ARROW, "export_arrow: column type without an Arrow format");
      }
    auto h = std::unique_ptr<ExportHolder>(new ExportHolder());
    auto sh = std::unique_ptr<SchemaHolder>(new SchemaHolder());
    h->children.resize((size_t)nc);
    h->child_ptrs.resize((size_t)nc);
    h->bufs.resize((size_t)nc);
    sh->children.resize((size_t)nc);
    sh->child_ptrs.resize((size_t)nc);
    sh->names.resize((size_t)nc);
    static const int32_t zero_off[1] = {0};
    for (int c = 0; c < nc; c++) {
      const sqlrs_column_t &col = hb->columns[c];
      ArrowArray &a = h->children[(size_t)c];
      a = ArrowArray{};
      a.length = col.length;
      a.null_count = col.validity ? col.null_count : 0;
      a.offset = 0;
      h->bufs[(size_t)c] = {col.validity && col.null_count != 0 ? col.validity : nullptr, nullptr, nullptr};
      if (col.dtype == SQLRS_UTF8) {
        a.n_buffers = 3;
        h->bufs[(size_t)c][1] = col.offsets ? (const void *)col.offsets : (const void *)zero_off;
        h->bufs[(size_t)c][2] = col.values;
      } else {
        a.n_buffers = 2;
        h->bufs[(size_t)c][1] = col.values;
      }
      a.buffers = h->bufs[(size_t)c].data();
      a.release = export_child_release;
      a.private_data = h.get();
      h->child_ptrs[(size_t)c] = &a;
      ArrowSchema &s = sh->children[(size_t)c];
      s = ArrowSchema{};
      sh->names[(size_t)c] = (names && names[c]) ? names[c] : ("c" + std::to_string(c));
      s.format = arrow_format(col.dtype);
      s.name = sh->names[(size_t)c].c_str();
      s.flags = ARROW_FLAG_NULLABLE;
      s.release = export_schema_child_release;
      sh->child_ptrs[(size_t)c] = &s;
    }
    *out_array = ArrowArray{};
    out_array->length = hb->num_rows;
    out_array->n_buffers = 1;
    out_array->buffers = h->top_buf;
    out_array->n_children = nc;
    out_array->children = h->child_ptrs.data();
    out_array->release = export_parent_release;
    out_array->private_data = h.get();
    *out_schema = ArrowSchema{};
    out_schema->format = "+s";
    out_schema->name = "";
    out_schema->n_children = nc;
    out_schema->children = sh->child_ptrs.data();
    out_schema->release = export_schema_release;
    out_schema->private_data = sh.release();
    h->batch = hb;
    h->refs.store(nc + 1);
    h.release();
    if (hb != batch) sqlrs_batch_release(batch);
  });
}

struct sqlrs_timer {
  Ctx *ctx;
  hipEvent_t a, b;
};
int sqlrs_timer_create(sqlrs_ctx_t *ctx, sqlrs_timer_t **out) {
  return guard(ctx, [&] {
    auto *t = new sqlrs_timer();
    t->ctx = ctx;
    SQ_HIP(hipEventCreate(&t->a));
    SQ_HIP(hipEventCreate(&t->b));
    *out = t;
  });
}
int sqlrs_timer_start(sqlrs_timer_t *t) {
  return guard(t->ctx, [&] { SQ_HIP(hipEventRecord(t->a, t->ctx->stream)); });
}
int sqlrs_timer_stop(sqlrs_timer_t *t) {
  return guard(t->ctx, [&] { SQ_HIP(hipEventRecord(t->b, t->ctx->stream)); });
}
int sqlrs_timer_elapsed_ms(sqlrs_timer_t *t, double *ms) {
  return guard(t->ctx, [&] {
    SQ_HIP(hipEventSynchronize(t->b));
    float f = 0;
    SQ_HIP(hipEventElapsedTime(&f, t->a, t->b));
    *ms = f;
  });
}
void sqlrs_timer_destroy(sqlrs_timer_t *t) {
  if (!t) return;
  (void)hipEventDestroy(t->a);
  (void)hipEventDestroy(t->b);
  delete t;
}

int sqlrs_ctx_profile_enable(sqlrs_ctx_t *ctx, int on) {
  return guard(ctx, [&] {
    ctx->prof_resolve();
    ctx->prof_on = on != 0;
  });
}
int sqlrs_ctx_profile_reset(sqlrs_ctx_t *ctx) {
  return guard(ctx, [&] {
    ctx->prof_resolve();
    for (auto &e : ctx->prof) {
      e.total_ms = 0;
      e.launches = 0;
    }
  });
}
int sqlrs_ctx_profile_read(sqlrs_ctx_t *ctx, int cap, const char **names, double *total_ms,
                           int64_t *launches) {
  try {
    ctx->prof_resolve();
  } catch (...) {
    return 0;
  }
  int n = 0;
  for (auto &e : ctx->prof) {
    if (n < cap) {
      names[n] = e.name;
      total_ms[n] = e.total_ms;
      launches[n] = e.launches;
    }
    n++;
  }
  if (ctx->lb_timeouts) {
    if (n < cap) {
      names[n] = "lookback_ticket_reruns";
      total_ms[n] = 0;
      launches[n] = ctx->lb_timeouts;
    }
    n++;
  }
  if (ctx->async_fast_batches) {
    if (n < cap) {
      names[n] = "async_fast_batches";
      total_ms[n] = 0;
      launches[n] = ctx->async_fast_batches;
    }
    n++;
  }
  if (ctx->async_conj_batches) {
    if (n < cap) {
      names[n] = "async_conj_batches";
      total_ms[n] = 0;
      launches[n] = ctx->async_conj_batches;
    }
    n++;
  }
  if (ctx->order_lb_fallbacks) {
    if (n < cap) {
      names[n] = "order_lookback_fallbacks";
      total_ms[n] = 0;
      launches[n] = ctx->order_lb_fallbacks;
    }
    n++;
  }
  static const char *const AGG_ROUTE_NAMES[Ctx::AR_COUNT_] = {
      "agg_part_dense", "agg_part_slim_runs", "agg_part_slim_blk", "agg_part_probe_spec", "agg_part_probe_generic",
      "agg_part_interpreted", "agg_part_packed", "agg_part_unpacked", "agg_part_flags", "agg_part_rec",
      "agg_part_in_place", "agg_part_join", "agg_part_join_mult", "agg_part_split", "agg_part_overflow_rows",
      "agg_merge_groups", "agg_pending_deferred", "agg_wide_parts"};
  for (int r = 0; r < Ctx::AR_COUNT_; r++) {
    if (!ctx->agg_route[r]) continue;
    if (n < cap) {
      names[n] = AGG_ROUTE_NAMES[r];
      total_ms[n] = 0;
      launches[n] = ctx->agg_route[r];
    }
    n++;
  }
  static const char *const JOIN_ROUTE_NAMES[Ctx::JR_COUNT_] = {
      "join_dense_adopted", "join_dense_refused", "join_dense_one_fetch", "join_dense_two_fetch", "join_dense_packed",
      "join_dense_plain", "join_probe_pending", "join_allhit_kept", "join_allhit_redone", "join_compact_dense",
      "join_compact_slots", "join_unique_outer", "join_dd_stream", "join_dd_rows", "join_counts_grouped",
      "join_counts_per_row", "join_lds_unique", "join_lds_distinct", "join_table_late"};
  for (int r = 0; r < Ctx::JR_COUNT_; r++) {
    if (!ctx->join_route[r]) continue;
    if (n < cap) {
      names[n] = JOIN_ROUTE_NAMES[r];
      total_ms[n] = 0;
      launches[n] = ctx->join_route[r];
    }
    n++;
  }
  return n;
}

const char *sqlrs_version(void) { return "sqlrs-hip 0.1.0 gfx950"; }

}
```

### sqlrs_amd/csrc/gather.hip

```cpp
#include "common.hpp"
#include "device_utils.hpp"
#include "prims.hpp"

namespace sq {

template <class T, class I>
__global__ __launch_bounds__(BLOCK) void gather_kernel(const T *__restrict__ src,
                                                       const uint64_t *__restrict__ src_validity,
                                                       const I *__restrict__ idx,
                                                       const uint64_t *__restrict__ idx_validity,
                                                       int64_t n, T *__restrict__ out,
                                                       uint64_t *__restrict__ out_validity) {
  int64_t i = blockIdx.x * (int64_t)blockDim.x + threadIdx.x;
  bool in_range = i < n;
  bool valid = in_range;
  I s = 0;
  if (in_range) {
    if (idx_validity) valid = (idx_validity[i >> 6] >> (i & 63)) & 1;
    if (valid) {
      s = idx[i];
      if (src_validity) valid = (src_validity[s >> 6] >> (s & 63)) & 1;
    }
    out[i] = valid ? src[s] : T(0);
  }
  if (out_validity) {
    uint64_t m = __ballot(valid);
    if (lane_id() == 0 && (i & ~63ll) < n) out_validity[i >> 6] = m;
  }
}

constexpr int GU = 8;
template <class T, class I>
__global__ __launch_bounds__(BLOCK) void gather_plain_kernel(const T *__restrict__ src, const I *__restrict__ idx, int64_t n,
                                                             T *__restrict__ out) {
  const int64_t base = blockIdx.x * (int64_t)(BLOCK * GU) + threadIdx.x;
  I s[GU];
#pragma unroll
  for (int u = 0; u < GU; u++) s[u] = __builtin_nontemporal_load(idx + min(base + u * BLOCK, n - 1));
  T v[GU];
#pragma unroll
  for (int u = 0; u < GU; u++) v[u] = src[s[u]];
#pragma unroll
  for (int u = 0; u < GU; u++)
    if (base + u * BLOCK < n) __builtin_nontemporal_store(v[u], out + base + u * BLOCK);
}

template <class I>
__global__ __launch_bounds__(BLOCK) void gather_bits_kernel(const uint64_t *__restrict__ src,
                                                            const uint64_t *__restrict__ src_validity,
                                                            const I *__restrict__ idx,
                                                            const uint64_t *__restrict__ idx_validity,
                                                            int64_t n, uint64_t *__restrict__ out,
                                                            uint64_t *__restrict__ out_validity) {
  int64_t i = blockIdx.x * (int64_t)blockDim.x + threadIdx.x;
  bool valid = i < n, bit = false;
  if (valid) {
    if (idx_validity) valid = (idx_validity[i >> 6] >> (i & 63)) & 1;
    if (valid) {
      I s = idx[i];
      if (src_validity) valid = (src_validity[s >> 6] >> (s & 63)) & 1;
      bit = valid && ((src[s >> 6] >> (s & 63)) & 1);
    }
  }
  uint64_t mb = __ballot(bit), mv = __ballot(valid);
  if (lane_id() == 0 && (i & ~63ll) < n) {
    out[i >> 6] = mb;
    if (out_validity) out_validity[i >> 6] = mv;
  }
}

template <class I>
__global__ void utf8_lengths_kernel(const int32_t *__restrict__ offsets,
                                    const uint64_t *__restrict__ src_validity,
                                    const I *__restrict__ idx,
                                    const uint64_t *__restrict__ idx_validity, int64_t n,
                                    uint32_t *__restrict__ len, uint64_t *__restrict__ out_validity) {
  int64_t i = blockIdx.x * (int64_t)blockDim.x + threadIdx.x;
  bool valid = i < n;
  uint32_t l = 0;
  if (valid) {
    if (idx_validity) valid = (idx_validity[i >> 6] >> (i & 63)) & 1;
    if (valid) {
      I s = idx[i];
      if (src_validity) valid = (src_validity[s >> 6] >> (s & 63)) & 1;
      if (valid) l = (uint32_t)(offsets[s + 1] - offsets[s]);
    }
    len[i] = l;
  }
  if (out_validity) {
    uint64_t m = __ballot(valid);
    if (lane_id() == 0 && (i & ~63ll) < n) out_validity[i >> 6] = m;
  }
}
template <class I>
__global__ void utf8_copy_kernel(const uint8_t *__restrict__ src, const int32_t *__restrict__ offsets,
                                 const I *__restrict__ idx, const uint32_t *__restrict__ len,
                                 const uint32_t *__restrict__ new_off, int64_t n,
                                 uint8_t *__restrict__ out, int32_t *__restrict__ out_offsets,
                                 const uint64_t *total) {
  int64_t i = blockIdx.x * (int64_t)blockDim.x + threadIdx.x;
  if (i == 0) out_offsets[n] = (int32_t)*total;
  if (i >= n) return;
  uint32_t o = new_off[i], l = len[i];
  out_offsets[i] = (int32_t)o;
  if (!l) return;
  const uint8_t *s = src + offsets[idx[i]];
  for (uint32_t k = 0; k < l; k++) out[o + k] = s[k];
}

template <class I>
static DCol gather_impl(Ctx *ctx, const DCol &src, const I *idx, const uint64_t *idx_validity,
                        int64_t n) {
  DCol o;
  o.dtype = src.dtype;
  o.length = n;
  const uint64_t *sv = (src.validity && src.null_count != 0) ? src.validity : nullptr;
  bool nullable = sv || idx_validity;
  uint64_t *ov = nullptr;
  if (nullable) {
    o.own_validity = ctx->alloc(bitmap_bytes(std::max<int64_t>(n, 1)));
    o.validity = ov = o.own_validity->as<uint64_t>();
    o.null_count = -1;
  }
  int64_t n64 = (int64_t)round_up((size_t)std::max<int64_t>(n, 1), 64);
  dim3 g((unsigned)ceil_div(n64, BLOCK)), b(BLOCK);
  ProfScope ps(ctx, "gather");
  if (src.dtype == SQLRS_UTF8) {
    BufP len = ctx->alloc(4 * (size_t)std::max<int64_t>(n, 1));
    BufP noff = ctx->alloc(4 * (size_t)std::max<int64_t>(n, 1));
    BufP total = ctx->alloc_zero(8);
    o.own_offsets = ctx->alloc(4 * (size_t)(n + 1));
    o.offsets = o.own_offsets->as<int32_t>();
    if (n == 0) {
      SQ_HIP(hipMemsetAsync(o.own_offsets->p, 0, 4, ctx->stream));
      o.own_values = ctx->alloc(8);
      o.values = o.own_values->p;
      return o;
    }
    utf8_lengths_kernel<I><<<g, b, 0, ctx->stream>>>(src.offsets, sv, idx, idx_validity, n,
                                                     len->as<uint32_t>(), ov);
    SQ_HIP(hipGetLastError());
    exclusive_scan_u32(ctx, len->as<uint32_t>(), n, nullptr, noff->as<uint32_t>(),
                       total->as<uint64_t>());
    uint64_t bytes = ctx->fetch_value(total->as<uint64_t>());
    if (bytes > 0x7fffffffull) fail(SQLRS_ERR_ARROW, "utf8 take overflows int32 offsets");
    o.data_bytes = (int64_t)bytes;
    o.own_values = ctx->alloc((size_t)bytes + 8);
    o.values = o.own_values->p;
    utf8_copy_kernel<I><<<g, b, 0, ctx->stream>>>(src.v<uint8_t>(), src.offsets, idx,
                                                  len->as<uint32_t>(), noff->as<uint32_t>(), n,
                                                  o.own_values->as<uint8_t>(),
                                                  o.own_offsets->as<int32_t>(), total->as<uint64_t>());
    SQ_HIP(hipGetLastError());
    return o;
  }
  if (src.dtype == SQLRS_BOOLEAN) {
    o.own_values = ctx->alloc(bitmap_bytes(std::max<int64_t>(n, 1)));
    o.values = o.own_values->p;
    if (n == 0) return o;
    gather_bits_kernel<I><<<g, b, 0, ctx->stream>>>(src.v<uint64_t>(), sv, idx, idx_validity, n,
                                                    o.own_values->as<uint64_t>(), ov);
    SQ_HIP(hipGetLastError());
    return o;
  }
  size_t w = width_of(src.dtype);
  if (!w) fail(SQLRS_ERR_INTERNAL, "take: unsupported dtype");
  o.own_values = ctx->alloc(w * (size_t)std::max<int64_t>(n, 1) + 16);
  o.values = o.own_values->p;
  if (n == 0) return o;
  if (!nullable) {
    dim3 gp((unsigned)ceil_div(n, BLOCK * GU));
    if (w == 8) gather_plain_kernel<uint64_t, I><<<gp, b, 0, ctx->stream>>>(src.v<uint64_t>(), idx, n, o.own_values->as<uint64_t>());
    else gather_plain_kernel<uint32_t, I><<<gp, b, 0, ctx->stream>>>(src.v<uint32_t>(), idx, n, o.own_values->as<uint32_t>());
    SQ_HIP(hipGetLastError());
    return o;
  }
  if (w == 8)
    gather_kernel<uint64_t, I><<<g, b, 0, ctx->stream>>>(src.v<uint64_t>(), sv, idx, idx_validity, n,
                                                         o.own_values->as<uint64_t>(), ov);
  else
    gather_kernel<uint32_t, I><<<g, b, 0, ctx->stream>>>(src.v<uint32_t>(), sv, idx, idx_validity, n,
                                                         o.own_values->as<uint32_t>(), ov);
  SQ_HIP(hipGetLastError());
  return o;
}

DCol gather_column(Ctx *ctx, const DCol &src_in, const void *idx, bool idx_is_u64,
                   const uint64_t *idx_validity, int64_t n) {
  DCol src = src_in.stride == 0 ? materialize_scalar(ctx, src_in, src_in.length) : src_in;
  if (idx_is_u64) return gather_impl<uint64_t>(ctx, src, (const uint64_t *)idx, idx_validity, n);
  return gather_impl<uint32_t>(ctx, src, (const uint32_t *)idx, idx_validity, n);
}

template <int K>
__global__ __launch_bounds__(BLOCK) void pack_rows_kernel(const uint64_t *__restrict__ c0, const uint64_t *__restrict__ c1,
                                                          const uint64_t *__restrict__ c2, const uint64_t *__restrict__ c3,
                                                          int64_t n, uint64_t *__restrict__ rows) {
  constexpr int W = K <= 2 ? 2 : 4;
  const int64_t i = blockIdx.x * (int64_t)BLOCK + threadIdx.x;
  if (i >= n) return;
  u64x2 a;
  a.x = c0[i];
  a.y = c1[i];
  *(u64x2 *)(rows + (size_t)W * i) = a;
  if (K > 2) {
    u64x2 b;
    b.x = c2[i];
    b.y = K > 3 ? c3[i] : 0ull;
    *(u64x2 *)(rows + (size_t)W * i + 2) = b;
  }
}
template <int K>
__global__ __launch_bounds__(BLOCK) void gather_rows_kernel(const uint64_t *__restrict__ rows, const uint32_t *__restrict__ idx,
                                                            int64_t n, uint64_t *__restrict__ o0, uint64_t *__restrict__ o1,
                                                            uint64_t *__restrict__ o2, uint64_t *__restrict__ o3) {
  constexpr int W = K <= 2 ? 2 : 4, U = 4;
  const int64_t base = blockIdx.x * (int64_t)(BLOCK * U) + threadIdx.x;
  uint32_t s[U];
#pragma unroll
  for (int u = 0; u < U; u++) s[u] = __builtin_nontemporal_load(idx + min(base + u * BLOCK, n - 1));
  u64x2 a[U], b[U];
#pragma unroll
  for (int u = 0; u < U; u++) {
    a[u] = *(const u64x2 *)(rows + (size_t)W * s[u]);
    if (K > 2) b[u] = *(const u64x2 *)(rows + (size_t)W * s[u] + 2);
  }
#pragma unroll
  for (int u = 0; u < U; u++) {
    const int64_t i = base + u * BLOCK;
    if (i >= n) continue;
    o0[i] = a[u].x;
    o1[i] = a[u].y;
    if (K > 2) o2[i] = b[u].x;
    if (K > 3) o3[i] = b[u].y;
  }
}

bool gather_columns_packed(Ctx *ctx, std::vector<DCol> &cols, int64_t src_rows, const uint32_t *idx, int64_t n) {
  const int k = (int)cols.size();
  if (k < 2 || k > 4 || n < (1 << 18)) return false;
  for (const DCol &c : cols)
    if (width_of(c.dtype) != 8 || c.stride == 0 || (c.validity && c.null_count != 0) || c.length != src_rows) return false;
  const int w = k <= 2 ? 2 : 4;
  BufP rows = ctx->alloc(8 * (size_t)w * (size_t)src_rows);
  const uint64_t *p[4] = {nullptr, nullptr, nullptr, nullptr};
  for (int i = 0; i < k; i++) p[i] = cols[(size_t)i].v<uint64_t>();
  dim3 b(BLOCK), gp((unsigned)ceil_div(src_rows, BLOCK)), gg((unsigned)ceil_div(n, BLOCK * 4));
  std::vector<DCol> outs((size_t)k);
  uint64_t *o[4] = {nullptr, nullptr, nullptr, nullptr};
  for (int i = 0; i < k; i++) {
    DCol &d = outs[(size_t)i];
    d.dtype = cols[(size_t)i].dtype;
    d.length = n;
    d.null_count = 0;
    d.own_values = ctx->alloc(8 * (size_t)n + 16);
    d.values = d.own_values->p;
    o[i] = d.own_values->as<uint64_t>();
  }
  uint64_t *r = rows->as<uint64_t>();
  switch (k) {
  case 2:
    pack_rows_kernel<2><<<gp, b, 0, ctx->stream>>>(p[0], p[1], p[2], p[3], src_rows, r);
    gather_rows_kernel<2><<<gg, b, 0, ctx->stream>>>(r, idx, n, o[0], o[1], o[2], o[3]);
    break;
  case 3:
    pack_rows_kernel<3><<<gp, b, 0, ctx->stream>>>(p[0], p[1], p[2], p[3], src_rows, r);
    gather_rows_kernel<3><<<gg, b, 0, ctx->stream>>>(r, idx, n, o[0], o[1], o[2], o[3]);
    break;
  default:
    pack_rows_kernel<4><<<gp, b, 0, ctx->stream>>>(p[0], p[1], p[2], p[3], src_rows, r);
    gather_rows_kernel<4><<<gg, b, 0, ctx->stream>>>(r, idx, n, o[0], o[1], o[2], o[3]);
  }
  SQ_HIP(hipGetLastError());
  cols = std::move(outs);
  return true;
}

__global__ void count_clear_kernel(const uint64_t *__restrict__ bits, int64_t rows, int64_t nwords,
                                   unsigned long long *out) {
  int64_t i = blockIdx.x * (int64_t)blockDim.x + threadIdx.x;
  uint64_t c = 0;
  for (int64_t w = i; w < nwords; w += (int64_t)gridDim.x * blockDim.x) {
    uint64_t v = ~bits[w];
    int64_t rem = rows - w * 64;
    if (rem < 64) v &= (1ull << rem) - 1;
    c += (uint64_t)__popcll(v);
  }
  c = wave_sum_u64(c);
  if (lane_id() == 0 && c) atomicAdd(out, (unsigned long long)c);
}
int64_t count_clear_bits(Ctx *ctx, const uint64_t *bits, int64_t rows) {
  if (!bits || rows == 0) return 0;
  BufP out = ctx->alloc_zero(8);
  int64_t nwords = ceil_div(rows, 64);
  unsigned blocks = (unsigned)std::min<int64_t>(ceil_div(nwords, 256), 2048);
  count_clear_kernel<<<dim3(blocks), dim3(256), 0, ctx->stream>>>(
      bits, rows, nwords, out->as<unsigned long long>());
  SQ_HIP(hipGetLastError());
  return (int64_t)ctx->fetch_value(out->as<uint64_t>());
}

__global__ void append_bits_kernel(const uint64_t *__restrict__ src, int64_t n, int64_t dst_off,
                                   unsigned long long *__restrict__ dst, int all_ones) {
  int64_t i = blockIdx.x * (int64_t)blockDim.x + threadIdx.x;
  int64_t nw = (n + 63) >> 6;
  if (i >= nw) return;
  uint64_t v = all_ones ? ~0ull : src[i];
  int64_t rem = n - i * 64;
  if (rem < 64) v &= (1ull << rem) - 1;
  int64_t pos = dst_off + i * 64;
  int sh = (int)(pos & 63);
  int64_t dw = pos >> 6;
  if (v << sh) atomicOr(&dst[dw], (unsigned long long)(v << sh));
  if (sh && (v >> (64 - sh))) atomicOr(&dst[dw + 1], (unsigned long long)(v >> (64 - sh)));
}

__global__ void rebase_offsets_kernel(const int32_t *__restrict__ src, int64_t n, int32_t add,
                                      int32_t *__restrict__ dst) {
  int64_t i = blockIdx.x * (int64_t)blockDim.x + threadIdx.x;
  if (i <= n) dst[i] = src[i] + add;
}

DCol copy_column(Ctx *ctx, const DCol &c_in) {
  DCol c = c_in.stride == 0 ? materialize_scalar(ctx, c_in, c_in.length) : c_in;
  DCol o = c;
  auto dup = [&](const void *src, size_t bytes) -> BufP {
    BufP b = ctx->alloc(bytes + 16);
    if (bytes) SQ_HIP(hipMemcpyAsync(b->p, src, bytes, hipMemcpyDeviceToDevice, ctx->stream));
    return b;
  };
  auto dup_bits = [&](const void *src) -> BufP {
    BufP b = ctx->alloc_zero(bitmap_bytes(c.length) + 8);
    size_t nbytes = (size_t)ceil_div(c.length, 8);
    if (nbytes) SQ_HIP(hipMemcpyAsync(b->p, src, nbytes, hipMemcpyDeviceToDevice, ctx->stream));
    return b;
  };
  if (c.validity && c.null_count != 0) {
    o.own_validity = dup_bits(c.validity);
    o.validity = o.own_validity->as<uint64_t>();
  } else {
    o.validity = nullptr;
    o.own_validity.reset();
    o.null_count = 0;
  }
  if (c.dtype == SQLRS_BOOLEAN) {
    o.own_values = dup_bits(c.values);
  } else if (c.dtype == SQLRS_UTF8) {
    o.own_offsets = dup(c.offsets, 4 * (size_t)(c.length + 1));
    o.offsets = o.own_offsets->as<int32_t>();
    o.own_values = dup(c.values, (size_t)c.data_bytes);
  } else {
    o.own_values = dup(c.values, width_of(c.dtype) * (size_t)c.length);
  }
  o.values = o.own_values->p;
  return o;
}

DCol concat_columns(Ctx *ctx, const std::vector<const DCol *> &parts_in) {
  if (parts_in.empty()) fail(SQLRS_ERR_INTERNAL, "concat of nothing");
  std::vector<DCol> mat;
  mat.reserve(parts_in.size());
  for (const DCol *p : parts_in) mat.push_back(p->stride == 0 ? materialize_scalar(ctx, *p, p->length) : *p);
  if (mat.size() == 1) return mat[0];
  DCol o;
  o.dtype = mat[0].dtype;
  bool any_nulls = false;
  int64_t total = 0, total_bytes = 0;
  for (const DCol &p : mat) {
    if (p.dtype != o.dtype) fail(SQLRS_ERR_ARROW, "concat_batches: schema mismatch");
    total += p.length;
    total_bytes += p.data_bytes;
    any_nulls |= (p.validity && p.null_count != 0);
  }
  o.length = total;
  ProfScope ps(ctx, "concat");
  auto bits_concat = [&](bool validity) -> BufP {
    BufP out = ctx->alloc_zero(bitmap_bytes(std::max<int64_t>(total, 1)) + 8);
    int64_t off = 0;
    for (const DCol &p : mat) {
      const uint64_t *src = validity ? p.validity : p.v<uint64_t>();
      int ones = validity && !(p.validity && p.null_count != 0);
      int64_t nw = ceil_div(p.length, 64);
      if (nw)
        append_bits_kernel<<<dim3((unsigned)ceil_div(nw, 256)), dim3(256), 0, ctx->stream>>>(
            src, p.length, off, out->as<unsigned long long>(), ones);
      off += p.length;
    }
    SQ_HIP(hipGetLastError());
    return out;
  };
  if (any_nulls) {
    o.own_validity = bits_concat(true);
    o.validity = o.own_validity->as<uint64_t>();
    o.null_count = -1;
  }
  if (o.dtype == SQLRS_BOOLEAN) {
    o.own_values = bits_concat(false);
    o.values = o.own_values->p;
    return o;
  }
  if (o.dtype == SQLRS_UTF8) {
    if (total_bytes > 0x7fffffffll) fail(SQLRS_ERR_ARROW, "concat overflows int32 offsets");
    o.own_offsets = ctx->alloc(4 * (size_t)(total + 1));
    o.own_values = ctx->alloc((size_t)total_bytes + 8);
    o.offsets = o.own_offsets->as<int32_t>();
    o.values = o.own_values->p;
    o.data_bytes = total_bytes;
    int64_t roff = 0, boff = 0;
    for (const DCol &p : mat) {
      rebase_offsets_kernel<<<dim3((unsigned)ceil_div(p.length + 1, 256)), dim3(256), 0,
                              ctx->stream>>>(p.offsets, p.length, (int32_t)boff,
                                             o.own_offsets->as<int32_t>() + roff);
      if (p.data_bytes)
        SQ_HIP(hipMemcpyAsync(o.own_values->as<uint8_t>() + boff, p.values, (size_t)p.data_bytes,
                              hipMemcpyDeviceToDevice, ctx->stream));
      roff += p.length;
      boff += p.data_bytes;
    }
    SQ_HIP(hipGetLastError());
    return o;
  }
  size_t w = width_of(o.dtype);
  o.own_values = ctx->alloc(w * (size_t)std::max<int64_t>(total, 1) + 16);
  o.values = o.own_values->p;
  size_t off = 0;
  for (const DCol &p : mat) {
    if (p.length)
      SQ_HIP(hipMemcpyAsync(o.own_values->as<uint8_t>() + off, p.values, w * (size_t)p.length,
                            hipMemcpyDeviceToDevice, ctx->stream));
    off += w * (size_t)p.length;
  }
  return o;
}

template <class T> __global__ void fill_kernel(T *out, int64_t n, T v) {
  int64_t i = blockIdx.x * (int64_t)blockDim.x + threadIdx.x;
  if (i < n) out[i] = v;
}

DCol materialize_scalar(Ctx *ctx, const DCol &c, int64_t rows) {
  if (c.stride != 0) return c;
  if (c.scalar_null) return make_null_column(ctx, c.dtype, rows);
  DCol o;
  o.dtype = c.dtype;
  o.length = rows;
  int64_t n1 = std::max<int64_t>(rows, 1);
  int64_t nw = ceil_div(n1, 64);
  if (c.dtype == SQLRS_BOOLEAN) {
    o.own_values = ctx->alloc(8 * (size_t)nw);
    fill_kernel<uint64_t><<<dim3((unsigned)ceil_div(nw, 256)), dim3(256), 0, ctx->stream>>>(
        o.own_values->as<uint64_t>(), nw, c.scalar_bits ? ~0ull : 0ull);
    o.values = o.own_values->p;
  } else if (c.dtype == SQLRS_UTF8) {
    fail(SQLRS_ERR_INTERNAL, "utf8 constants are not supported on the device path");
  } else {
    size_t w = width_of(c.dtype);
    if (!w) fail(SQLRS_ERR_INTERNAL, "constant of unsupported dtype");
    o.own_values = ctx->alloc(w * (size_t)n1 + 16);
    o.values = o.own_values->p;
    if (w == 8)
      fill_kernel<uint64_t><<<dim3((unsigned)ceil_div(n1, 256)), dim3(256), 0, ctx->stream>>>(
          o.own_values->as<uint64_t>(), rows, c.scalar_bits);
    else
      fill_kernel<uint32_t><<<dim3((unsigned)ceil_div(n1, 256)), dim3(256), 0, ctx->stream>>>(
          o.own_values->as<uint32_t>(), rows, (uint32_t)c.scalar_bits);
  }
  SQ_HIP(hipGetLastError());
  return o;
}

DCol make_null_column(Ctx *ctx, int32_t dtype, int64_t n) {
  DCol o;
  o.dtype = dtype;
  o.length = n;
  o.null_count = n;
  int64_t n1 = std::max<int64_t>(n, 1);
  if (n > 0) {
    o.own_validity = ctx->alloc_zero(bitmap_bytes(n1));
    o.validity = o.own_validity->as<uint64_t>();
  }
  if (dtype == SQLRS_UTF8) {
    o.own_offsets = ctx->alloc_zero(4 * (size_t)(n + 1));
    o.offsets = o.own_offsets->as<int32_t>();
    o.own_values = ctx->alloc(8);
  } else if (dtype == SQLRS_BOOLEAN) {
    o.own_values = ctx->alloc_zero(bitmap_bytes(n1));
  } else {
    size_t w = width_of(dtype);
    if (!w) fail(SQLRS_ERR_INTERNAL, "null array of unsupported dtype");
    o.own_values = ctx->alloc_zero(w * (size_t)n1);
  }
  o.values = o.own_values->p;
  return o;
}

template <class T> __global__ void iota_kernel(T *out, int64_t n) {
  int64_t i = blockIdx.x * (int64_t)blockDim.x + threadIdx.x;
  if (i < n) out[i] = (T)i;
}
void iota_u32(Ctx *ctx, uint32_t *out, int64_t n) {
  if (n <= 0) return;
  iota_kernel<uint32_t><<<dim3((unsigned)ceil_div(n, 256)), dim3(256), 0, ctx->stream>>>(out, n);
  SQ_HIP(hipGetLastError());
}

}
```

### sqlrs_amd/csrc/hashagg_op.hip

```cpp
#include <cstdlib>

#include "agg_partition.hpp"
#include "agg_state.hpp"
#include "common.hpp"
#include "device_utils.hpp"
#include "host_stage.hpp"
#include "prims.hpp"

using namespace sq;

namespace {

struct AggSpec {
  int func = 0, distinct = 0;
  int32_t return_dtype = 0;
  Expr arg;
  GrowBuf acc, nn;
  bool track_nn = false;
  int32_t acc_dtype = 0;
  int argcol = -1;
  struct StrBatch {
    DCol col;
    BufP gid;
    int64_t n;
  };
  std::vector<StrBatch> strs;
};

uint64_t acc_identity(const AggSpec &a) { return a.func == SQLRS_AGG_MIN ? ~0ull : 0ull; }

bool same_expr(const Expr &x, const Expr &y) {
  if (x.nodes.size() != y.nodes.size()) return false;
  for (size_t i = 0; i < x.nodes.size(); i++) {
    const sqlrs_expr_node_t &p = x.nodes[i], &q = y.nodes[i];
    if (p.op != q.op || p.dtype != q.dtype || p.index != q.index || p.is_null != q.is_null || p.i != q.i ||
        std::memcmp(&p.f, &q.f, 8) != 0 || x.strings[i] != y.strings[i])
      return false;
  }
  return true;
}

}

struct PendingGroups {
  bool active = false;
  PartAggOutput po;
  std::vector<DCol> keyvals;
  std::vector<int> cnt_of_col, acc_of_agg, col_of_agg;
  std::vector<uint8_t> col_nullable;
  std::vector<int32_t> col_dtype;
  bool exact = true;
  int32_t key_dtype = SQLRS_INT64;
};

struct sqlrs_hash_agg {
  Ctx *ctx = nullptr;
  HostStage hstage;
  PendingGroups pending;
  std::vector<Expr> group_by;
  std::vector<AggSpec> aggs;
  AggState st;
  bool saw_batch = false, in_order = true;
  struct Staged {
    std::vector<DCol> kcols, acols;
    int64_t n = 0;
  };
  std::vector<Staged> staged;
  int64_t staged_rows = 0;
  bool any_order = false;
  bool strong_keys = false;
  int64_t rows_seen = 0;
  std::vector<int32_t> key_dtypes;
  std::vector<std::vector<DCol>> key_parts;
  std::vector<Expr> arg_exprs;
  std::vector<int32_t> arg_cast;
  struct DistinctAgg {
    int func = 0;
    int32_t return_dtype = 0;
    sqlrs_hash_agg *dedup = nullptr;
  };
  std::vector<DistinctAgg> distinct_aggs;
  std::vector<std::pair<int, int>> out_order;
  bool has_filter = false;
  Expr filter;
  int64_t filter_fused_batches = 0;
  std::vector<sqlrs_hash_agg *> parts;
  std::vector<std::pair<int, int>> part_col;
  ~sqlrs_hash_agg() {
    for (auto &d : distinct_aggs) delete d.dedup;
    for (auto *p : parts) delete p;
  }
};

extern "C" int sqlrs_hash_agg_push(sqlrs_hash_agg_t *a, const sqlrs_batch_t *in);
extern "C" int sqlrs_hash_agg_finish(sqlrs_hash_agg_t *a, int out_mem, sqlrs_batch_t **out);
extern "C" int sqlrs_hash_agg_create(sqlrs_ctx_t *ctx, int num_group_by, const sqlrs_expr_t *group_by, int num_aggs,
                                     const sqlrs_agg_func_t *aggs, sqlrs_hash_agg_t **out);
extern "C" void sqlrs_hash_agg_destroy(sqlrs_hash_agg_t *a);
extern "C" void sqlrs_batch_release(sqlrs_batch_t *batch);
extern "C" int sqlrs_filter_create(sqlrs_ctx_t *, const sqlrs_expr_t *, sqlrs_filter_t **);
extern "C" int sqlrs_filter_push(sqlrs_filter_t *, const sqlrs_batch_t *, int, sqlrs_batch_t **);
extern "C" void sqlrs_filter_destroy(sqlrs_filter_t *);

namespace sq {
bool fusable_row_filter(const Expr &e, InBatch &ib, RowFilter *rf);

__global__ void gather_u32_kernel(const uint32_t *__restrict__ src, const uint32_t *__restrict__ idx,
                                  int64_t n, uint32_t *__restrict__ out) {
  int64_t i = blockIdx.x * (int64_t)blockDim.x + threadIdx.x;
  if (i < n) out[i] = src[idx[i]];
}
__global__ void rowid_from_u32_kernel(const uint32_t *__restrict__ rows, int64_t n, uint64_t offset,
                                      uint64_t *__restrict__ out) {
  int64_t i = blockIdx.x * (int64_t)blockDim.x + threadIdx.x;
  if (i < n) out[i] = offset + rows[i];
}

struct ArgView {
  const void *values = nullptr;
  const uint64_t *validity = nullptr;
  int32_t dtype = 0;
  const DCol *col = nullptr;
};

static BufP resolve_groups(sqlrs_hash_agg *a, const NKeys &nk, const uint64_t *row_ids,
                           const uint32_t *local_map, const std::vector<DCol> &kcols, int64_t *nnew_out) {
  Ctx *ctx = a->ctx;
  BufP new_rows;
  int64_t nnew = 0;
  BufP row_gid = agg_resolve_rows(ctx, a->st, nk, row_ids, (uint64_t)a->rows_seen, &new_rows, &nnew);
  if (nnew) {
    const void *idx = new_rows->p;
    BufP mapped;
    if (local_map) {
      mapped = ctx->alloc(4 * (size_t)nnew);
      gather_u32_kernel<<<dim3((unsigned)ceil_div(nnew, 256)), dim3(256), 0, ctx->stream>>>(
          local_map, new_rows->as<uint32_t>(), nnew, mapped->as<uint32_t>());
      SQ_HIP(hipGetLastError());
      idx = mapped->p;
    }
    for (size_t c = 0; c < kcols.size(); c++)
      a->key_parts[c].push_back(gather_column(ctx, kcols[c], idx, false, nullptr, nnew));
  }
  if (row_ids) a->in_order = false;
  *nnew_out = nnew;
  return row_gid;
}

static void start_tracking(Ctx *ctx, AggSpec &s, int64_t G, int64_t nnew) {
  if (s.track_nn) return;
  s.track_nn = true;
  s.nn.ensure(ctx, std::max<int64_t>(G, 1), 0);
  if (G - nnew > 0) fill_u64(ctx, s.nn.buf->as<uint64_t>(), G - nnew, 1);
}

__global__ void rank_of_perm_kernel(const uint32_t *__restrict__ perm, int64_t n, uint32_t *__restrict__ rank) {
  int64_t i = blockIdx.x * (int64_t)blockDim.x + threadIdx.x;
  if (i < n) rank[perm[i]] = (uint32_t)i;
}
__global__ void best_rank_kernel(const uint32_t *__restrict__ gid, const uint32_t *__restrict__ rank,
                                 const uint64_t *__restrict__ validity, int64_t n, int is_min,
                                 uint32_t *__restrict__ best) {
  int64_t i = blockIdx.x * (int64_t)blockDim.x + threadIdx.x;
  if (i >= n) return;
  if (validity && !((validity[i >> 6] >> (i & 63)) & 1)) return;
  if (is_min) atomicMin(&best[gid[i]], rank[i] + 1);
  else atomicMax(&best[gid[i]], rank[i] + 1);
}
__global__ void winner_row_kernel(const uint32_t *__restrict__ best, const uint32_t *__restrict__ perm, int64_t G,
                                  int is_min, uint32_t *__restrict__ row, uint64_t *__restrict__ has) {
  int64_t g = blockIdx.x * (int64_t)blockDim.x + threadIdx.x;
  uint32_t b = g < G ? best[g] : 0;
  bool ok = g < G && b != (is_min ? 0xffffffffu : 0u);
  if (g < G) row[g] = ok ? perm[b - 1] : 0;
  uint64_t m = __ballot(ok);
  if (lane_id() == 0 && g < G) has[g >> 6] = m;
}

static DCol finalize_utf8_minmax(Ctx *ctx, AggSpec &s, int64_t G) {
  const int is_min = s.func == SQLRS_AGG_MIN;
  int64_t G1 = std::max<int64_t>(G, 1);
  std::vector<const DCol *> parts;
  int64_t N = 0;
  for (auto &sb : s.strs) {
    parts.push_back(&sb.col);
    N += sb.n;
  }
  if (parts.empty() || N == 0) return make_null_column(ctx, SQLRS_UTF8, G);
  if (N > 0xfffffffell) fail(SQLRS_ERR_INTERNAL, "utf8 min/max: more than 2^32 rows");
  DCol all = concat_columns(ctx, parts);
  BufP gid = ctx->alloc(4 * (size_t)N);
  size_t off = 0;
  for (auto &sb : s.strs) {
    if (sb.n) SQ_HIP(hipMemcpyAsync(gid->as<uint8_t>() + off, sb.gid->p, 4 * (size_t)sb.n, hipMemcpyDeviceToDevice, ctx->stream));
    off += 4 * (size_t)sb.n;
  }
  const uint64_t *valid = (all.validity && all.null_count != 0) ? all.validity : nullptr;
  BufP perm = ctx->alloc(4 * (size_t)N), keys = ctx->alloc(8 * (size_t)N), rank = ctx->alloc(4 * (size_t)N);
  iota_u32(ctx, perm->as<uint32_t>(), N);
  sort_perm_by_utf8(ctx, all, valid, 0, perm->as<uint32_t>(), keys->as<uint64_t>(), N);
  dim3 b(256), gn((unsigned)ceil_div(N, 256));
  rank_of_perm_kernel<<<gn, b, 0, ctx->stream>>>(perm->as<uint32_t>(), N, rank->as<uint32_t>());
  BufP best = ctx->alloc(4 * (size_t)G1);
  SQ_HIP(hipMemsetAsync(best->p, is_min ? 0xff : 0, 4 * (size_t)G1, ctx->stream));
  best_rank_kernel<<<gn, b, 0, ctx->stream>>>(gid->as<uint32_t>(), rank->as<uint32_t>(), valid, N, is_min,
                                               best->as<uint32_t>());
  BufP row = ctx->alloc(4 * (size_t)G1), has = ctx->alloc_zero(bitmap_bytes(G1));
  int64_t G64 = (int64_t)round_up((size_t)G1, 64);
  winner_row_kernel<<<dim3((unsigned)ceil_div(G64, 256)), b, 0, ctx->stream>>>(
      best->as<uint32_t>(), perm->as<uint32_t>(), G, is_min, row->as<uint32_t>(), has->as<uint64_t>());
  SQ_HIP(hipGetLastError());
  DCol out = gather_column(ctx, all, row->p, false, has->as<uint64_t>(), G);
  out.dtype = SQLRS_UTF8;
  return out;
}

static void update_from_rows(sqlrs_hash_agg *a, const BufP &rgbuf, const std::vector<ArgView> &args,
                             int64_t n, int64_t nnew) {
  Ctx *ctx = a->ctx;
  int64_t G = a->st.ngroups;
  const uint32_t *rg = rgbuf->as<uint32_t>();
  for (AggSpec &s : a->aggs) {
    const ArgView &v = args[(size_t)s.argcol];
    if (v.dtype == SQLRS_UTF8 && (s.func == SQLRS_AGG_MIN || s.func == SQLRS_AGG_MAX)) {
      if (s.return_dtype != SQLRS_UTF8 || !v.col) fail(SQLRS_ERR_INTERNAL, "unsupported min_max scalar type");
      AggSpec::StrBatch sb;
      bool borrowed = (v.col->values && !v.col->own_values) || (v.col->validity && !v.col->own_validity) ||
                      (v.col->offsets && !v.col->own_offsets);
      sb.col = borrowed ? copy_column(ctx, *v.col) : *v.col;
      sb.gid = rgbuf;
      sb.n = n;
      s.strs.push_back(std::move(sb));
      continue;
    }
    if (s.func == SQLRS_AGG_COUNT) {
      s.nn.ensure(ctx, G, 0);
      agg_update_count(ctx, s.nn, rg, v.validity, nullptr, n);
      continue;
    }
    if (v.validity) start_tracking(ctx, s, G, nnew);
    if (s.track_nn) {
      s.nn.ensure(ctx, G, 0);
      agg_update_count(ctx, s.nn, rg, v.validity, nullptr, n);
    }
    if (s.func == SQLRS_AGG_SUM) {
      s.acc_dtype = s.return_dtype;
      s.acc.ensure(ctx, G, 0);
      agg_update_sum(ctx, s.acc, s.acc_dtype, rg, v.values, v.validity, n);
    } else {
      if (v.dtype != s.return_dtype) fail(SQLRS_ERR_INTERNAL, "unsupported min_max scalar type");
      s.acc_dtype = v.dtype;
      s.acc.ensure(ctx, G, acc_identity(s));
      agg_update_minmax(ctx, s.acc, s.acc_dtype, s.func == SQLRS_AGG_MIN, rg, v.values, v.validity, n);
    }
  }
}

static void merge_groups(sqlrs_hash_agg *a, PendingGroups &pg) {
  Ctx *ctx = a->ctx;
  ctx->agg_route[Ctx::AR_MERGE_GROUPS]++;
  PartAggOutput &po = pg.po;
  NKeys gk;
  gk.rows = po.groups;
  gk.keys = po.gkey;
  gk.exact = pg.exact;
  gk.dtype = pg.key_dtype;
  if (po.gvalid_bits) {
    gk.validity = po.gvalid_bits->as<uint64_t>();
    gk.own_validity = po.gvalid_bits;
  }
  int64_t nnew = 0;
  BufP rgid = resolve_groups(a, gk, part_row_ids(ctx, po), nullptr, pg.keyvals, &nnew);
  const uint32_t *rg = rgid->as<uint32_t>();
  int64_t G = a->st.ngroups, g = po.groups;
  auto cell = [&](int acc) { return po.gacc->as<uint64_t>() + (size_t)acc * (size_t)po.gcap; };
  for (size_t i = 0; i < a->aggs.size(); i++) {
    AggSpec &s = a->aggs[i];
    int col = pg.col_of_agg[i];
    int cc = pg.cnt_of_col[(size_t)col];
    if (s.func == SQLRS_AGG_COUNT) {
      s.nn.ensure(ctx, G, 0);
      agg_update_count(ctx, s.nn, rg, nullptr, (const int64_t *)cell(cc), g);
      continue;
    }
    if (pg.col_nullable[(size_t)col]) start_tracking(ctx, s, G, nnew);
    if (s.track_nn) {
      s.nn.ensure(ctx, G, 0);
      agg_update_count(ctx, s.nn, rg, nullptr, (const int64_t *)cell(cc), g);
    }
    int ac = pg.acc_of_agg[i];
    if (s.func == SQLRS_AGG_SUM) {
      s.acc_dtype = s.return_dtype;
      s.acc.ensure(ctx, G, 0);
      agg_update_sum(ctx, s.acc, s.acc_dtype, rg, cell(ac), nullptr, g);
    } else {
      s.acc_dtype = pg.col_dtype[(size_t)col];
      s.acc.ensure(ctx, G, acc_identity(s));
      agg_update_minmax(ctx, s.acc, SQLRS_UINT64 , s.func == SQLRS_AGG_MIN, rg,
                        cell(ac), nullptr, g);
    }
  }
}

static void flush_pending(sqlrs_hash_agg *a) {
  if (!a->pending.active) return;
  PendingGroups pg = std::move(a->pending);
  a->pending = PendingGroups();
  merge_groups(a, pg);
}

static DBatch emit_pending(sqlrs_hash_agg *a) {
  Ctx *ctx = a->ctx;
  PendingGroups &pg = a->pending;
  PartAggOutput &po = pg.po;
  int64_t G = po.groups;
  DBatch o;
  o.rows = G;
  for (const DCol &k : pg.keyvals) o.cols.push_back(k);
  auto cell = [&](int acc) { return po.gacc->as<uint64_t>() + (size_t)acc * (size_t)po.gcap; };
  for (size_t i = 0; i < a->aggs.size(); i++) {
    AggSpec &s = a->aggs[i];
    int col = pg.col_of_agg[i];
    int cc = pg.cnt_of_col[(size_t)col];
    if (s.func == SQLRS_AGG_COUNT) {
      o.cols.push_back(agg_finalize_raw(ctx, s.func, SQLRS_INT64, cell(cc), nullptr, G, po.gacc));
      continue;
    }
    const uint64_t *nn = pg.col_nullable[(size_t)col] ? cell(cc) : nullptr;
    int32_t dt = s.func == SQLRS_AGG_SUM ? s.return_dtype : pg.col_dtype[(size_t)col];
    DCol c = agg_finalize_raw(ctx, s.func, dt, cell(pg.acc_of_agg[i]), nn, G, po.gacc);
    c.dtype = s.return_dtype;
    o.cols.push_back(c);
  }
  if (G > 1 && !a->any_order) {
    ProfScope ps(ctx, "agg_order_groups");
    BufP perm = ctx->alloc(4 * (size_t)G);
    int bits = 1;
    while (bits < 32 && (1ull << bits) <= (uint64_t)std::max<int64_t>(a->rows_seen, 1)) bits++;
    radix_sort_index_u32(ctx, po.gfirst->as<uint32_t>(), G, bits, perm->as<uint32_t>());
    if (!gather_columns_packed(ctx, o.cols, G, perm->as<uint32_t>(), G))
      for (DCol &c : o.cols) c = gather_column(ctx, c, perm->p, false, nullptr, G);
  }
  return o;
}

static DCol distinct_column(sqlrs_hash_agg *a, sqlrs_hash_agg::DistinctAgg &d, int64_t G) {
  Ctx *ctx = a->ctx;
  sqlrs_batch_t *dd = nullptr, *res = nullptr;
  int st = sqlrs_hash_agg_finish(d.dedup, SQLRS_MEM_DEVICE, &dd);
  if (st != SQLRS_OK) fail(st, ctx->last_error);
  const int nk = (int)a->group_by.size();
  std::vector<sqlrs_expr_node_t> nodes((size_t)nk + 1);
  std::vector<sqlrs_expr_t> gb((size_t)nk);
  std::memset(nodes.data(), 0, sizeof(sqlrs_expr_node_t) * nodes.size());
  for (int i = 0; i < nk; i++) {
    nodes[(size_t)i].op = SQLRS_EXPR_INPUT_REF;
    nodes[(size_t)i].index = i;
    gb[(size_t)i].nodes = &nodes[(size_t)i];
    gb[(size_t)i].num_nodes = 1;
    gb[(size_t)i].reserved = 0;
  }
  sqlrs_agg_func_t af;
  std::memset(&af, 0, sizeof(af));
  if (d.func == SQLRS_AGG_COUNT) {
    nodes[(size_t)nk].op = SQLRS_EXPR_CONSTANT;
    nodes[(size_t)nk].dtype = SQLRS_INT64;
    nodes[(size_t)nk].i = 1;
    af.func = SQLRS_AGG_COUNT;
    af.return_dtype = SQLRS_INT64;
  } else {
    nodes[(size_t)nk].op = SQLRS_EXPR_INPUT_REF;
    nodes[(size_t)nk].index = nk;
    af.func = SQLRS_AGG_SUM;
    af.return_dtype = d.return_dtype;
  }
  af.arg.nodes = &nodes[(size_t)nk];
  af.arg.num_nodes = 1;
  sqlrs_hash_agg_t *b = nullptr;
  st = sqlrs_hash_agg_create((sqlrs_ctx_t *)ctx, nk, gb.data(), 1, &af, &b);
  if (st == SQLRS_OK) st = sqlrs_hash_agg_push(b, dd);
  if (st == SQLRS_OK) st = sqlrs_hash_agg_finish(b, SQLRS_MEM_DEVICE, &res);
  std::string err = ctx->last_error;
  if (b) sqlrs_hash_agg_destroy(b);
  DCol out;
  if (st == SQLRS_OK) {
    if (res->num_rows != G) {
      st = SQLRS_ERR_INTERNAL;
      err = "distinct aggregate produced a different number of groups";
    } else {
      const sqlrs_column_t &c = res->columns[nk];
      out.dtype = c.dtype;
      out.length = G;
      size_t w = width_of(c.dtype);
      out.own_values = ctx->alloc(w * (size_t)std::max<int64_t>(G, 1));
      out.values = out.own_values->p;
      if (G) SQ_HIP(hipMemcpyAsync(out.own_values->p, c.values, w * (size_t)G, hipMemcpyDeviceToDevice, ctx->stream));
      if (c.validity && c.null_count != 0) {
        out.own_validity = ctx->alloc(bitmap_bytes(std::max<int64_t>(G, 1)));
        SQ_HIP(hipMemcpyAsync(out.own_validity->p, c.validity, bitmap_bytes(G), hipMemcpyDeviceToDevice, ctx->stream));
        out.validity = out.own_validity->as<uint64_t>();
        out.null_count = c.null_count;
      }
      ctx->sync();
    }
  }
  if (dd) sqlrs_batch_release(dd);
  if (res) sqlrs_batch_release(res);
  if (st != SQLRS_OK) fail(st, err);
  return out;
}

static void place_aggregate_columns(sqlrs_hash_agg *a, DBatch &o) {
  if (a->distinct_aggs.empty()) return;
  const size_t nk = a->group_by.size();
  std::vector<DCol> cols(o.cols.begin(), o.cols.begin() + (long)nk);
  for (auto &e : a->out_order) {
    if (e.first == 0)
      cols.push_back(o.cols[nk + (size_t)e.second]);
    else
      cols.push_back(distinct_column(a, a->distinct_aggs[(size_t)e.second], o.rows));
  }
  o.cols = std::move(cols);
}

static std::vector<DCol> eval_arg_columns(sqlrs_hash_agg *a, const std::function<const DCol &(int)> &colfn,
                                          int64_t n, int shift) {
  Ctx *ctx = a->ctx;
  std::vector<DCol> acols;
  for (size_t k = 0; k < a->arg_exprs.size(); k++) {
    Expr e = a->arg_exprs[k];
    if (shift)
      for (auto &nd : e.nodes)
        if (nd.op == SQLRS_EXPR_INPUT_REF) nd.index -= shift;
    DCol c = eval_expr(ctx, e, colfn, n, true);
    if (a->arg_cast[k] && c.dtype != a->arg_cast[k]) {
      sqlrs_expr_node_t cn[2];
      std::memset(cn, 0, sizeof(cn));
      cn[0].op = SQLRS_EXPR_INPUT_REF;
      cn[1].op = SQLRS_EXPR_TYPE_CAST;
      cn[1].dtype = a->arg_cast[k];
      Expr ce;
      ce.nodes.assign(cn, cn + 2);
      ce.strings.resize(2);
      auto one = [&](int) -> const DCol & { return c; };
      DCol casted = eval_expr(ctx, ce, one, n, true);
      c = casted;
    }
    acols.push_back(c);
  }
  return acols;
}

struct JoinSide {
  const uint64_t *keys;
  const uint64_t *validity;
  int64_t n;
  PartitionedRows *cache;
  bool unique_known = true;
  bool range_known = false;
  uint64_t omin = 0, omax = 0;
  const uint64_t *bits = nullptr;
  const uint32_t *mult = nullptr;
};

static bool agg_consume(sqlrs_hash_agg *a, int64_t n, const std::vector<DCol> &kcols, const NKeys &nk,
                        const std::vector<DCol> &acols, const JoinSide *js, const RowFilter *rf = nullptr) {
  Ctx *ctx = a->ctx;
    auto views_of = [&](const std::vector<DCol> &cols) {
      std::vector<ArgView> v;
      for (const DCol &c : cols) {
        ArgView x;
        x.values = c.values;
        x.validity = (c.validity && c.null_count != 0) ? c.validity : nullptr;
        x.dtype = c.dtype;
        x.col = &c;
        v.push_back(x);
      }
      return v;
    };

    std::vector<DCol> pcols;
    std::vector<int> pidx(acols.size(), -1);
    for (size_t k = 0; k < acols.size(); k++) {
      for (size_t j = 0; j < k && pidx[k] < 0; j++)
        if (same_expr(a->arg_exprs[j], a->arg_exprs[k]) && acols[j].dtype == acols[k].dtype) pidx[k] = pidx[j];
      if (pidx[k] < 0) {
        pidx[k] = (int)pcols.size();
        pcols.push_back(acols[k]);
      }
    }
    bool done = false;
    const int64_t PART_MIN_ROWS = 1ll << 21;
    if ((n >= PART_MIN_ROWS || js) && pcols.size() <= 2) {
      PartAggSpec spec;
      bool ok = true;
      std::vector<int> acc_of_agg(a->aggs.size(), -1), cnt_of_col(pcols.size(), -1);
      for (const DCol &c : pcols)
        ok &= (c.dtype == SQLRS_INT64 || c.dtype == SQLRS_FLOAT64);
      for (size_t k = 0; ok && k < pcols.size(); k++) {
        bool need = pcols[k].validity && pcols[k].null_count != 0;
        for (const AggSpec &s : a->aggs)
          if (pidx[(size_t)s.argcol] == (int)k && (s.func == SQLRS_AGG_COUNT || s.track_nn)) need = true;
        if (need) {
          if (spec.n_acc >= PART_MAX_ACC) { ok = false; break; }
          cnt_of_col[k] = spec.n_acc;
          spec.op[spec.n_acc] = PART_COUNT;
          spec.src[spec.n_acc++] = (int)k;
        }
      }
      for (size_t i = 0; ok && i < a->aggs.size(); i++) {
        const AggSpec &s = a->aggs[i];
        if (s.func == SQLRS_AGG_COUNT) {
          acc_of_agg[i] = cnt_of_col[(size_t)pidx[(size_t)s.argcol]];
          continue;
        }
        if (spec.n_acc >= PART_MAX_ACC) { ok = false; break; }
        const DCol &c = pcols[(size_t)pidx[(size_t)s.argcol]];
        if (s.func != SQLRS_AGG_SUM && c.dtype != s.return_dtype) { ok = false; break; }
        acc_of_agg[i] = spec.n_acc;
        spec.op[spec.n_acc] = s.func == SQLRS_AGG_SUM ? (c.dtype == SQLRS_FLOAT64 ? PART_SUM_F64 : PART_SUM_I64)
                              : s.func == SQLRS_AGG_MIN ? PART_MIN : PART_MAX;
        spec.kind[spec.n_acc] = c.dtype == SQLRS_FLOAT64 ? 1 : 0;
        spec.src[spec.n_acc++] = pidx[(size_t)s.argcol];
      }
      spec.nv = (int)pcols.size();
      if (ok) {
        PartAggInput pin;
        pin.keys = nk.keys->as<uint64_t>();
        pin.key_validity = nk.validity;
        pin.n = n;
        for (size_t k = 0; k < pcols.size(); k++) {
          pin.vals[k] = pcols[k].values;
          pin.val_validity[k] = (pcols[k].validity && pcols[k].null_count != 0) ? pcols[k].validity : nullptr;
        }
        if (js) {
          pin.join_keys = js->keys;
          pin.join_validity = js->validity;
          pin.join_n = js->n;
          pin.join_cache = js->cache;
          pin.join_range_known = js->range_known;
          pin.join_unique_known = js->unique_known;
          pin.join_omin = js->omin;
          pin.join_omax = js->omax;
          pin.join_bits = js->bits;
          pin.join_mult = js->mult;
        }
        if (rf) pin.filter = *rf;
        PartAggOutput po;
        flush_pending(a);
        bool part_ok = partitioned_preaggregate(ctx, spec, pin, (uint64_t)a->rows_seen, &po);
        if (!part_ok && po.retry_exact) {
          pin.exact_stats = true;
          po = PartAggOutput();
          part_ok = partitioned_preaggregate(ctx, spec, pin, (uint64_t)a->rows_seen, &po);
        }
        if (part_ok) {
          PendingGroups pg;
          pg.active = true;
          pg.exact = nk.exact;
          pg.key_dtype = nk.dtype;
          pg.cnt_of_col = cnt_of_col;
          pg.acc_of_agg = acc_of_agg;
          for (const AggSpec &s : a->aggs) pg.col_of_agg.push_back(pidx[(size_t)s.argcol]);
          for (size_t k = 0; k < pcols.size(); k++) {
            pg.col_nullable.push_back(pin.val_validity[k] != nullptr);
            pg.col_dtype.push_back(pcols[k].dtype);
          }
          if (nk.exact && kcols.size() == 1 && (kcols[0].dtype == SQLRS_INT64 || kcols[0].dtype == SQLRS_FLOAT64) &&
              kcols[0].dtype == nk.dtype) {
            DCol kv;
            kv.dtype = kcols[0].dtype;
            kv.length = po.groups;
            kv.values = po.gkey->p;
            kv.own_values = po.gkey;
            if (po.gvalid_bits) {
              kv.validity = po.gvalid_bits->as<uint64_t>();
              kv.own_validity = po.gvalid_bits;
              kv.null_count = -1;
            }
            pg.keyvals.push_back(kv);
          } else {
            for (const DCol &kc : kcols)
              pg.keyvals.push_back(gather_column(ctx, kc, po.gfirst->p, false, nullptr, po.groups));
          }
          pg.po = po;
          if (a->st.ngroups == 0 && po.n_overflow == 0 && !po.may_dup) {
            a->pending = std::move(pg);
            ctx->agg_route[Ctx::AR_PENDING]++;
          } else
            merge_groups(a, pg);
          if (po.n_overflow) {
            int64_t m = po.n_overflow;
            DCol kc;
            kc.dtype = SQLRS_UINT64;
            kc.length = n;
            kc.values = nk.keys->p;
            kc.validity = nk.validity;
            kc.null_count = nk.validity ? -1 : 0;
            DCol sub = gather_column(ctx, kc, po.ov_rows->p, false, nullptr, m);
            NKeys ok_;
            ok_.rows = m;
            ok_.keys = sub.own_values;
            ok_.exact = nk.exact;
            ok_.dtype = nk.dtype;
            if (sub.validity) {
              ok_.validity = sub.validity;
              ok_.own_validity = sub.own_validity;
            }
            BufP rid = ctx->alloc(8 * (size_t)m);
            rowid_from_u32_kernel<<<dim3((unsigned)ceil_div(m, 256)), dim3(256), 0, ctx->stream>>>(
                po.ov_rows->as<uint32_t>(), m, (uint64_t)a->rows_seen, rid->as<uint64_t>());
            SQ_HIP(hipGetLastError());
            std::vector<DCol> sub_args;
            for (const DCol &c : acols) sub_args.push_back(gather_column(ctx, c, po.ov_rows->p, false, nullptr, m));
            int64_t nn2 = 0;
            BufP rg2 = resolve_groups(a, ok_, rid->as<uint64_t>(), po.ov_rows->as<uint32_t>(), kcols, &nn2);
            for (DCol &c : sub_args)
              if (c.validity && c.null_count < 0) c.null_count = count_nulls(ctx, c);
            update_from_rows(a, rg2, views_of(sub_args), m, nn2);
          }
          done = true;
        }
      }
    }
    if (!done && (js || rf)) return false;
    if (!done) {
      flush_pending(a);
      int64_t nnew = 0;
      BufP row_gid = resolve_groups(a, nk, nullptr, nullptr, kcols, &nnew);
      update_from_rows(a, row_gid, views_of(acols), n, nnew);
    }
    return true;
}

static const int64_t STAGE_DIRECT_ROWS = [] {
  const char *e = hook("SQLRS_STAGE_DIRECT_ROWS");
  return e ? std::atoll(e) : (1ll << 26);
}();
static const int64_t STAGE_FLUSH_ROWS = [] {
  const char *e = hook("SQLRS_STAGE_FLUSH_ROWS");
  return e ? std::atoll(e) : (1ll << 28);
}();

static DCol own_column(Ctx *ctx, const DCol &c, int64_t n) {
  DCol m = c.stride == 0 ? materialize_scalar(ctx, c, n) : c;
  bool borrowed = (m.values && !m.own_values) || (m.validity && !m.own_validity) || (m.offsets && !m.own_offsets);
  return borrowed ? copy_column(ctx, m) : m;
}

static void flush_staged(sqlrs_hash_agg *a) {
  if (a->staged.empty()) return;
  Ctx *ctx = a->ctx;
  std::vector<sqlrs_hash_agg::Staged> st = std::move(a->staged);
  a->staged.clear();
  int64_t n = a->staged_rows;
  a->staged_rows = 0;
  std::vector<DCol> kcols, acols;
  if (st.size() == 1) {
    kcols = std::move(st[0].kcols);
    acols = std::move(st[0].acols);
  } else {
    for (size_t c = 0; c < st[0].kcols.size(); c++) {
      std::vector<const DCol *> parts;
      for (auto &b : st) parts.push_back(&b.kcols[c]);
      kcols.push_back(concat_columns(ctx, parts));
    }
    for (size_t c = 0; c < st[0].acols.size(); c++) {
      std::vector<const DCol *> parts;
      for (auto &b : st) parts.push_back(&b.acols[c]);
      acols.push_back(concat_columns(ctx, parts));
    }
  }
  NKeys nk = a->strong_keys ? normalize_keys_strong(ctx, kcols, n) : normalize_keys(ctx, kcols, n);
  agg_consume(a, n, kcols, nk, acols, nullptr);
  a->rows_seen += n;
}

}

extern "C" {

static int hash_agg_create_impl(sqlrs_ctx_t *ctx, int num_group_by, const sqlrs_expr_t *group_by, int num_aggs,
                                const sqlrs_agg_func_t *aggs, bool allow_split, sqlrs_hash_agg_t **out);
int sqlrs_hash_agg_create(sqlrs_ctx_t *ctx, int num_group_by, const sqlrs_expr_t *group_by,
                          int num_aggs, const sqlrs_agg_func_t *aggs, sqlrs_hash_agg_t **out) {
  return hash_agg_create_impl(ctx, num_group_by, group_by, num_aggs, aggs, true, out);
}

static void hash_agg_plan_parts(sqlrs_hash_agg *a, sqlrs_ctx_t *ctx, int num_group_by, const sqlrs_expr_t *group_by,
                                const sqlrs_agg_func_t *aggs) {
  const char *env = hook("SQLRS_AGG_SPLIT");
  if (env && std::atoi(env) == 0) return;
  if (!a->distinct_aggs.empty() || a->aggs.size() < 3) return;
  std::vector<int> col_of((size_t)a->aggs.size(), -1);
  int ncols = 0;
  for (size_t i = 0; i < a->aggs.size(); i++) {
    if (a->aggs[i].return_dtype == SQLRS_UTF8) return;
    for (size_t k = 0; k < i && col_of[i] < 0; k++)
      if (same_expr(a->aggs[k].arg, a->aggs[i].arg)) col_of[i] = col_of[k];
    if (col_of[i] < 0) col_of[i] = ncols++;
  }
  struct Part {
    std::vector<int> cols, aggs;
    int cells = 0;
  };
  std::vector<Part> plan;
  for (size_t i = 0; i < a->aggs.size(); i++) {
    const int c = col_of[i], own = a->aggs[i].func != SQLRS_AGG_COUNT ? 1 : 0;
    size_t at = plan.size();
    for (size_t q = 0; q < plan.size() && at == plan.size(); q++) {
      const bool has = std::find(plan[q].cols.begin(), plan[q].cols.end(), c) != plan[q].cols.end();
      if (has && plan[q].cells + own <= PART_MAX_ACC) at = q;
    }
    if (at == plan.size()) plan.emplace_back();
    Part &pt = plan[at];
    if (std::find(pt.cols.begin(), pt.cols.end(), c) == pt.cols.end()) {
      pt.cols.push_back(c);
      pt.cells++;
    }
    pt.cells += own;
    pt.aggs.push_back((int)i);
  }
  if (plan.size() < 2) return;
  if (ncols <= 2) {
    int cells = ncols;
    for (const AggSpec &sp : a->aggs) cells += sp.func != SQLRS_AGG_COUNT ? 1 : 0;
    if (cells <= PART_MAX_ACC) return;
  }
  a->part_col.assign(a->aggs.size(), {0, 0});
  for (size_t q = 0; q < plan.size(); q++) {
    std::vector<sqlrs_agg_func_t> sub;
    for (size_t k = 0; k < plan[q].aggs.size(); k++) {
      sub.push_back(aggs[plan[q].aggs[k]]);
      a->part_col[(size_t)plan[q].aggs[k]] = {(int)q, (int)k};
    }
    sqlrs_hash_agg_t *p = nullptr;
    int st = hash_agg_create_impl(ctx, num_group_by, group_by, (int)sub.size(), sub.data(), false, &p);
    if (st != SQLRS_OK) fail(st, ctx->last_error);
    a->parts.push_back(p);
  }
}

static int hash_agg_create_impl(sqlrs_ctx_t *ctx, int num_group_by, const sqlrs_expr_t *group_by, int num_aggs,
                                const sqlrs_agg_func_t *aggs, bool allow_split, sqlrs_hash_agg_t **out) {
  return guard(ctx, [&] {
    if (num_group_by < 1)
      fail(SQLRS_ERR_INTERNAL, "HashAgg needs at least one group-by expression");
    auto a = std::unique_ptr<sqlrs_hash_agg>(new sqlrs_hash_agg());
    a->ctx = ctx;
    for (int i = 0; i < num_group_by; i++) a->group_by.push_back(expr_from_abi(&group_by[i]));
    for (int i = 0; i < num_aggs; i++) {
      AggSpec s;
      s.func = aggs[i].func;
      s.distinct = aggs[i].distinct;
      s.return_dtype = aggs[i].return_dtype;
      s.arg = expr_from_abi(&aggs[i].arg);
      if (s.func < SQLRS_AGG_COUNT || s.func > SQLRS_AGG_MAX)
        fail(SQLRS_ERR_INTERNAL, "unknown aggregate function");
      if (s.distinct && (s.func == SQLRS_AGG_COUNT || s.func == SQLRS_AGG_SUM)) {
        if (s.func == SQLRS_AGG_SUM && s.return_dtype != SQLRS_INT64 && s.return_dtype != SQLRS_FLOAT64)
          fail(SQLRS_ERR_INTERNAL, "not expected types for sum");
        sqlrs_hash_agg::DistinctAgg d;
        d.func = s.func;
        d.return_dtype = s.return_dtype;
        d.dedup = new sqlrs_hash_agg();
        d.dedup->ctx = ctx;
        d.dedup->strong_keys = true;
        d.dedup->group_by = a->group_by;
        d.dedup->group_by.push_back(s.arg);
        d.dedup->key_parts.resize(d.dedup->group_by.size());
        a->out_order.emplace_back(1, (int)a->distinct_aggs.size());
        a->distinct_aggs.push_back(d);
        continue;
      }
      a->out_order.emplace_back(0, (int)a->aggs.size());
      if (s.func == SQLRS_AGG_SUM && s.return_dtype != SQLRS_INT64 && s.return_dtype != SQLRS_FLOAT64)
        fail(SQLRS_ERR_INTERNAL, "not expected types for sum");
      int32_t cast = s.func == SQLRS_AGG_SUM ? s.return_dtype : 0;
      int found = -1;
      for (size_t k = 0; k < a->arg_exprs.size(); k++)
        if (a->arg_cast[k] == cast && same_expr(a->arg_exprs[k], s.arg)) found = (int)k;
      if (found < 0) {
        a->arg_exprs.push_back(s.arg);
        a->arg_cast.push_back(cast);
        found = (int)a->arg_exprs.size() - 1;
      }
      s.argcol = found;
      a->aggs.push_back(std::move(s));
    }
    a->key_parts.resize((size_t)num_group_by);
    if (allow_split) hash_agg_plan_parts(a.get(), ctx, num_group_by, group_by, aggs);
    *out = a.release();
  });
}

static int hash_agg_push_device(sqlrs_hash_agg_t *a, const sqlrs_batch_t *in, bool filtered = false);
static int hash_agg_flush_host(sqlrs_hash_agg_t *a) {
  if (!a->hstage.has_schema) return SQLRS_OK;
  sqlrs_batch_t *dev = nullptr;
  int st = guard(a->ctx, [&] {
    SQ_HIP(hipSetDevice(a->ctx->device));
    dev = a->hstage.take();
  });
  if (st != SQLRS_OK) return st;
  st = hash_agg_push_device(a, dev);
  sqlrs_batch_release(dev);
  return st;
}

int sqlrs_hash_agg_push(sqlrs_hash_agg_t *a, const sqlrs_batch_t *in) {
  if (!a->parts.empty()) a->saw_batch = true;
  a->hstage.ctx = a->ctx;
  if (a->hstage.accepts(in)) {
    int st = guard(a->ctx, [&] { a->hstage.append(in); });
    if (st != SQLRS_OK || a->hstage.rows < HOST_STAGE_FLUSH_ROWS) return st;
    return hash_agg_flush_host(a);
  }
  int st = hash_agg_flush_host(a);
  return st != SQLRS_OK ? st : hash_agg_push_device(a, in);
}

static bool hash_agg_try_fused_filter(sqlrs_hash_agg_t *a, const sqlrs_batch_t *in) {
  Ctx *ctx = a->ctx;
  const int64_t n = in->num_rows;
  if (!a->staged.empty() || n < STAGE_DIRECT_ROWS || !a->distinct_aggs.empty()) return false;
  for (const Expr &e : a->group_by)
    for (const sqlrs_expr_node_t &nd : e.nodes)
      if (nd.op == SQLRS_EXPR_DIVIDE) return false;
  for (const Expr &e : a->arg_exprs)
    for (const sqlrs_expr_node_t &nd : e.nodes)
      if (nd.op == SQLRS_EXPR_DIVIDE) return false;
  InBatch ib(ctx, in);
  RowFilter rf;
  if (!fusable_row_filter(a->filter, ib, &rf)) return false;
  auto colfn = [&](int i) -> const DCol & { return ib.col(i); };
  std::vector<DCol> kcols;
  for (const Expr &e : a->group_by) kcols.push_back(eval_expr(ctx, e, colfn, n, true));
  std::vector<DCol> acols = eval_arg_columns(a, colfn, n, 0);
  NKeys nk = a->strong_keys ? normalize_keys_strong(ctx, kcols, n) : normalize_keys(ctx, kcols, n);
  if (!agg_consume(a, n, kcols, nk, acols, nullptr, &rf)) return false;
  if (!a->saw_batch) {
    a->saw_batch = true;
    for (const DCol &k : kcols) a->key_dtypes.push_back(k.dtype);
  }
  a->rows_seen += n;
  a->filter_fused_batches++;
  return true;
}

static bool any_host_column(const sqlrs_batch_t *b) {
  for (int c = 0; c < b->num_columns; c++)
    if (b->columns[c].mem == SQLRS_MEM_HOST && b->columns[c].length > 0) return true;
  return false;
}
static int hash_agg_push_parts(sqlrs_hash_agg_t *a, const sqlrs_batch_t *in0) {
  const sqlrs_batch_t *in = in0;
  sqlrs_batch_t *dev = nullptr, *kept = nullptr;
  bool filtered = false;
  int st = SQLRS_OK;
  if (a->has_filter) {
    bool fusable = false;
    st = guard(a->ctx, [&] {
      SQ_HIP(hipSetDevice(a->ctx->device));
      if (any_host_column(in0) || in0->num_rows < STAGE_DIRECT_ROWS) return;
      InBatch ib(a->ctx, in0);
      RowFilter rf;
      fusable = fusable_row_filter(a->filter, ib, &rf);
    });
    if (st != SQLRS_OK) return st;
    if (!fusable) {
      std::vector<sqlrs_expr_node_t> nodes = a->filter.nodes;
      for (size_t i = 0; i < nodes.size(); i++) nodes[i].s = a->filter.strings[i].empty() ? nullptr : a->filter.strings[i].c_str();
      sqlrs_expr_t fe{nodes.data(), (int32_t)nodes.size(), 0};
      sqlrs_filter_t *f = nullptr;
      st = sqlrs_filter_create((sqlrs_ctx_t *)a->ctx, &fe, &f);
      if (st != SQLRS_OK) return st;
      st = sqlrs_filter_push(f, in0, SQLRS_MEM_DEVICE, &kept);
      sqlrs_filter_destroy(f);
      if (st != SQLRS_OK) return st;
      in = kept;
      filtered = true;
    }
  }
// ... 610 lines not shown
```

### sqlrs_amd/csrc/prims.hpp

```cpp
#pragma once

#include <functional>

#include "common.hpp"

namespace sq {

void exclusive_scan_u32(Ctx *ctx, const uint32_t *in, int64_t n, uint64_t *out64, uint32_t *out32,
                        uint64_t *total);

struct Selection {
  int64_t rows = 0;
  int64_t count = 0;
  const uint64_t *bits = nullptr;
  BufP own_bits;
  BufP tile_off;
};
Selection selection_from_mask(Ctx *ctx, const DCol &mask);
Selection selection_from_clear_bits(Ctx *ctx, const uint64_t *bits, int64_t rows);
Selection selection_from_set_bits(Ctx *ctx, const uint64_t *bits, int64_t rows);
void selection_finish(Ctx *ctx, Selection &s);
DCol compact_column(Ctx *ctx, const DCol &c, const Selection &s);
BufP selection_indices_u32(Ctx *ctx, const Selection &s);
BufP selection_indices_u64(Ctx *ctx, const Selection &s);

bool filter_fast_path(Ctx *ctx, const Expr &e, const std::function<const DCol &(int)> &col,
                      int64_t rows, int *col_index, Selection *sel, DCol *out_col);

DCol gather_column(Ctx *ctx, const DCol &src, const void *idx, bool idx_is_u64,
                   const uint64_t *idx_validity, int64_t n);
bool gather_columns_packed(Ctx *ctx, std::vector<DCol> &cols, int64_t src_rows, const uint32_t *idx, int64_t n);
DCol concat_columns(Ctx *ctx, const std::vector<const DCol *> &parts);
DCol copy_column(Ctx *ctx, const DCol &c);
void sort_perm_by_utf8(Ctx *ctx, const DCol &c, const uint64_t *valid, int desc, uint32_t *perm, uint64_t *keys,
                       int64_t n);
DCol materialize_scalar(Ctx *ctx, const DCol &c, int64_t rows);
int64_t count_clear_bits(Ctx *ctx, const uint64_t *bits, int64_t rows);

DCol eval_expr(Ctx *ctx, const Expr &e, const std::function<const DCol &(int)> &col, int64_t rows,
               bool materialize);

struct NKeys {
  int64_t rows = 0;
  BufP keys;
  const uint64_t *validity = nullptr;
  BufP own_validity;
  bool exact = true;
  int32_t dtype = SQLRS_INT64;
};
NKeys normalize_keys(Ctx *ctx, const std::vector<DCol> &cols, int64_t rows);
NKeys normalize_keys_strong(Ctx *ctx, const std::vector<DCol> &cols, int64_t rows);

void radix_sort_pairs(Ctx *ctx, uint64_t *keys, uint32_t *vals, int64_t n, int begin_bit,
                      int end_bit, bool keys_below_end_bit = false);
void radix_sort_index_u32(Ctx *ctx, const uint32_t *keys, int64_t n, int bits, uint32_t *perm);
void iota_u32(Ctx *ctx, uint32_t *out, int64_t n);
bool order_fast(Ctx *ctx, const DCol &key, int desc, const DCol *carry, int64_t n, DCol *key_out, DCol *carry_out,
                BufP *perm, bool want_perm, bool *in_order = nullptr);
bool order_composite(Ctx *ctx, const std::vector<const DCol *> &keys, const std::vector<int> &desc, const DCol *carry, int64_t n,
                     std::vector<DCol> *keys_out, DCol *carry_out, BufP *perm, bool want_perm, bool *in_order);

}
```

### sqlrs_amd/csrc/sort.hip

```cpp
#include "common.hpp"
#include "device_utils.hpp"
#include "prims.hpp"

namespace sq {

constexpr int RS_WG = 512;
constexpr int RS_WAVES = RS_WG / 64;
constexpr int RS_ITEMS = 8;
constexpr int RS_TILE = RS_WG * RS_ITEMS;

template <bool KEY32 = false>
__global__ __launch_bounds__(RS_WG) void rs_hist_kernel(const uint64_t *__restrict__ keys, int64_t n,
                                                        int shift, int64_t nblocks,
                                                        uint32_t *__restrict__ hist) {
  __shared__ uint32_t h[256];
  if (threadIdx.x < 256) h[threadIdx.x] = 0;
  const int64_t base = (int64_t)blockIdx.x * RS_TILE + threadIdx.x;
  uint64_t k[RS_ITEMS];
#pragma unroll
  for (int r = 0; r < RS_ITEMS; r++)
    k[r] = KEY32 ? (uint64_t)__builtin_nontemporal_load((const uint32_t *)keys + min(base + r * RS_WG, n - 1))
                 : __builtin_nontemporal_load(keys + min(base + r * RS_WG, n - 1));
  __syncthreads();
#pragma unroll
  for (int r = 0; r < RS_ITEMS; r++)
    if (base + r * RS_WG < n) atomicAdd(&h[(k[r] >> shift) & 255], 1u);
  __syncthreads();
  if (threadIdx.x < 256) hist[(int64_t)threadIdx.x * nblocks + blockIdx.x] = h[threadIdx.x];
}

enum { RS_PAIR = 0, RS_PACKED = 1 };
template <int IN, int OUT, bool KEY32 = false>
__global__ __launch_bounds__(RS_WG) void rs_scatter_kernel(
    const uint64_t *__restrict__ keys, const uint32_t *__restrict__ vals, int64_t n, int shift,
    int64_t nblocks, const uint32_t *__restrict__ offsets, uint64_t *__restrict__ keys_out,
    uint32_t *__restrict__ vals_out, int key_lo, uint64_t key_const) {
  __shared__ uint64_t skey[RS_TILE];
  __shared__ uint32_t sval[(IN == RS_PAIR && OUT == RS_PAIR) ? RS_TILE : 1];
  __shared__ uint32_t wcnt[RS_WAVES][256];
  __shared__ uint32_t dstart[256];
  __shared__ int64_t gbase[256];
  __shared__ uint32_t s_wsum[4];
  const int w = wave_id(), lane = lane_id();
  const int64_t tbase = (int64_t)blockIdx.x * RS_TILE;
  const int64_t wrow = tbase + (int64_t)w * (RS_ITEMS * 64) + lane;
  uint64_t k[RS_ITEMS];
  uint32_t v[RS_ITEMS];
#pragma unroll
  for (int j = 0; j < RS_ITEMS; j++) {
    const int64_t i = min(wrow + j * 64, n - 1);
    k[j] = KEY32 ? (uint64_t)__builtin_nontemporal_load((const uint32_t *)keys + i) : __builtin_nontemporal_load(keys + i);
    v[j] = KEY32 ? (uint32_t)i : (IN == RS_PAIR ? __builtin_nontemporal_load(vals + i) : 0u);
  }
  uint32_t goff = threadIdx.x < 256 ? offsets[(int64_t)threadIdx.x * nblocks + blockIdx.x] : 0;
#pragma unroll
  for (int q = 0; q < 4; q++) wcnt[w][lane + 64 * q] = 0;
  uint32_t rnk[RS_ITEMS];
#pragma unroll
  for (int j = 0; j < RS_ITEMS; j++) {
    const bool valid = wrow + j * 64 < n;
    const uint32_t d = (uint32_t)(k[j] >> shift) & 255u;
    uint64_t peers = __ballot(valid);
    uint32_t dlo = 0, dhi = 0;
#pragma unroll
    for (int b = 0; b < 8; b++) {
      const int32_t mask = ((int32_t)(d << (31 - b))) >> 31;
      const uint64_t bm = __ballot(mask != 0);
      dlo |= (uint32_t)bm ^ (uint32_t)mask;
      dhi |= (uint32_t)(bm >> 32) ^ (uint32_t)mask;
    }
    peers &= ~(((uint64_t)dhi << 32) | dlo);
    const uint32_t r = (uint32_t)mbcnt(peers);
    uint32_t old = 0;
    if (valid && r == 0) {
      old = wcnt[w][d];
      wcnt[w][d] = old + (uint32_t)__popcll(peers);
    }
    old = (uint32_t)__shfl((int)old, valid ? __builtin_ctzll(peers) : 0, 64);
    rnk[j] = old + r;
  }
  __syncthreads();
  if (threadIdx.x < 256) {
    uint32_t acc = 0;
#pragma unroll
    for (int q = 0; q < RS_WAVES; q++) {
      uint32_t c = wcnt[q][threadIdx.x];
      wcnt[q][threadIdx.x] = acc;
      acc += c;
    }
    uint32_t inc = wave_iscan_u32(acc);
    if (lane == 63) s_wsum[w] = inc;
    dstart[threadIdx.x] = inc - acc;
  }
  __syncthreads();
  if (threadIdx.x < 256) {
    uint32_t wb = 0;
    for (int q = 0; q < w; q++) wb += s_wsum[q];
    uint32_t ds = dstart[threadIdx.x] + wb;
    dstart[threadIdx.x] = ds;
    gbase[threadIdx.x] = (int64_t)goff - (int64_t)ds;
  }
  __syncthreads();
#pragma unroll
  for (int j = 0; j < RS_ITEMS; j++) {
    if (wrow + j * 64 >= n) continue;
    const uint32_t d = (uint32_t)(k[j] >> shift) & 255u;
    const uint32_t p = dstart[d] + wcnt[w][d] + rnk[j];
    if (IN == RS_PAIR && OUT == RS_PACKED) skey[p] = ((k[j] >> key_lo) << 32) | v[j];
    else skey[p] = k[j];
    if (IN == RS_PAIR && OUT == RS_PAIR) sval[p] = v[j];
  }
  __syncthreads();
  const uint32_t len = (uint32_t)min<int64_t>(RS_TILE, n - tbase);
#pragma unroll
  for (int j = 0; j < RS_ITEMS; j++) {
    const uint32_t p = j * RS_WG + threadIdx.x;
    if (p < len) {
      const uint64_t kk = skey[p];
      const int sh = (IN == RS_PAIR && OUT == RS_PACKED) ? shift - key_lo + 32 : shift;
      const int64_t g = gbase[(uint32_t)(kk >> sh) & 255u] + p;
      if (OUT == RS_PACKED) {
        keys_out[g] = kk;
      } else if (IN == RS_PACKED) {
        if (keys_out) keys_out[g] = ((kk >> 32) << key_lo) | key_const;
        vals_out[g] = (uint32_t)kk;
      } else {
        if (keys_out) keys_out[g] = kk;
        vals_out[g] = sval[p];
      }
    }
  }
}

__global__ __launch_bounds__(256) void rs_diff_kernel(const uint64_t *__restrict__ keys, int64_t n,
                                                      unsigned long long *diff_or) {
  const uint64_t k0 = keys[0];
  uint64_t d = 0;
  for (int64_t i = blockIdx.x * (int64_t)(256 * 8) + threadIdx.x; i < n; i += (int64_t)gridDim.x * (256 * 8)) {
    uint64_t k[8];
#pragma unroll
    for (int u = 0; u < 8; u++) k[u] = keys[min(i + u * 256, n - 1)];
#pragma unroll
    for (int u = 0; u < 8; u++) d |= k[u] ^ k0;
  }
  for (int m = 32; m >= 1; m >>= 1) d |= shfl_xor_u64(d, m);
  __shared__ unsigned long long s_d[4];
  if (lane_id() == 0) s_d[wave_id()] = d;
  __syncthreads();
  if (threadIdx.x == 0) {
    d = s_d[0] | s_d[1] | s_d[2] | s_d[3];
    if (d) atomicOr(diff_or, (unsigned long long)d);
  }
  if (blockIdx.x == 0 && threadIdx.x == 0) diff_or[1] = k0;
}

void radix_sort_pairs(Ctx *ctx, uint64_t *keys, uint32_t *vals, int64_t n, int begin_bit,
                      int end_bit, bool keys_below_end_bit) {
  if (n <= 1 || end_bit <= begin_bit) return;
  if (n > 0xffffffffll) fail(SQLRS_ERR_INTERNAL, "radix sort: more than 2^32 rows");
  ProfScope ps(ctx, "radix_sort");
  uint64_t varying = ~0ull, key0 = 0;
  if (keys_below_end_bit && begin_bit == 0 && end_bit <= 32) {
    varying = (1ull << end_bit) - 1;
    key0 = 0;
  } else if ((end_bit - begin_bit > 16 && n >= (1 << 22)) || (end_bit - begin_bit > 32 && n >= (1 << 15))) {
    BufP diff = ctx->alloc_zero(16);
    unsigned blocks = (unsigned)std::min<int64_t>(ceil_div(n, 256 * 8), 4 * (int64_t)ctx->num_cus);
    rs_diff_kernel<<<dim3(blocks), dim3(256), 0, ctx->stream>>>(keys, n, diff->as<unsigned long long>());
    SQ_HIP(hipGetLastError());
    const uint64_t *h = (const uint64_t *)ctx->fetch(diff->p, 16);
    varying = h[0];
    key0 = h[1];
  }
  int64_t nblocks = ceil_div(n, RS_TILE);
  BufP k2 = ctx->alloc(8 * (size_t)n), v2 = ctx->alloc(4 * (size_t)n);
  BufP hist = ctx->alloc(4 * (size_t)(256 * nblocks)), offs = ctx->alloc(4 * (size_t)(256 * nblocks));
  BufP total = ctx->alloc(8);
  uint64_t *ka = keys, *kb = k2->as<uint64_t>();
  uint32_t *va = vals, *vb = v2->as<uint32_t>();
  std::vector<int> shifts;
  for (int shift = begin_bit; shift < end_bit; shift += 8)
    if (((varying >> shift) & 0xff) != 0) shifts.push_back(shift);
  int key_lo = 0;
  uint64_t key_const = 0;
  bool packed = false;
  if (varying != ~0ull && varying != 0 && shifts.size() >= 2) {
    key_lo = shifts.front();
    int key_hi = 64 - __builtin_clzll(varying);
    const bool low_bits_constant = key_lo == 0 || (varying & ((1ull << key_lo) - 1)) == 0;
    if (key_hi - key_lo <= 32 && low_bits_constant) {
      packed = true;
      uint64_t k0 = key0;
      uint64_t span = (key_hi - key_lo == 64) ? ~0ull : (((1ull << (key_hi - key_lo)) - 1) << key_lo);
      key_const = k0 & ~span;
    }
  }
  for (size_t pi = 0; pi < shifts.size(); pi++) {
    const int shift = shifts[pi];
    const bool in_packed = packed && pi > 0, out_packed = packed && pi + 1 < shifts.size();
    const int eff = in_packed ? shift - key_lo + 32 : shift;
    rs_hist_kernel<false><<<dim3((unsigned)nblocks), dim3(RS_WG), 0, ctx->stream>>>(ka, n, eff, nblocks,
                                                                                   hist->as<uint32_t>());
    SQ_HIP(hipGetLastError());
    exclusive_scan_u32(ctx, hist->as<uint32_t>(), 256 * nblocks, nullptr, offs->as<uint32_t>(),
                       total->as<uint64_t>());
    dim3 g((unsigned)nblocks), b(RS_WG);
    if (!in_packed && !out_packed)
      rs_scatter_kernel<RS_PAIR, RS_PAIR><<<g, b, 0, ctx->stream>>>(ka, va, n, shift, nblocks, offs->as<uint32_t>(), kb, vb, 0, 0);
    else if (!in_packed)
      rs_scatter_kernel<RS_PAIR, RS_PACKED><<<g, b, 0, ctx->stream>>>(ka, va, n, shift, nblocks, offs->as<uint32_t>(), kb, vb, key_lo, key_const);
    else if (out_packed)
      rs_scatter_kernel<RS_PACKED, RS_PACKED><<<g, b, 0, ctx->stream>>>(ka, va, n, eff, nblocks, offs->as<uint32_t>(), kb, vb, key_lo, key_const);
    else
      rs_scatter_kernel<RS_PACKED, RS_PAIR><<<g, b, 0, ctx->stream>>>(ka, va, n, eff, nblocks, offs->as<uint32_t>(), kb, vb, key_lo, key_const);
    SQ_HIP(hipGetLastError());
    std::swap(ka, kb);
    std::swap(va, vb);
  }
  if (ka != keys) {
    SQ_HIP(hipMemcpyAsync(keys, ka, 8 * (size_t)n, hipMemcpyDeviceToDevice, ctx->stream));
    SQ_HIP(hipMemcpyAsync(vals, va, 4 * (size_t)n, hipMemcpyDeviceToDevice, ctx->stream));
  }
}

void radix_sort_index_u32(Ctx *ctx, const uint32_t *keys, int64_t n, int bits, uint32_t *perm) {
  if (n <= 0) return;
  if (n > 0xffffffffll) fail(SQLRS_ERR_INTERNAL, "radix sort: more than 2^32 rows");
  ProfScope ps(ctx, "radix_sort");
  const int passes = std::max(1, (std::min(bits, 32) + 7) / 8);
  const int64_t nblocks = ceil_div(n, RS_TILE);
  BufP w0 = ctx->alloc(8 * (size_t)n), w1 = passes > 2 ? ctx->alloc(8 * (size_t)n) : nullptr;
  BufP hist = ctx->alloc(4 * (size_t)(256 * nblocks)), offs = ctx->alloc(4 * (size_t)(256 * nblocks));
  BufP total = ctx->alloc(8);
  dim3 g((unsigned)nblocks), b(RS_WG);
  const uint64_t *in = (const uint64_t *)keys;
  uint64_t *out = w0->as<uint64_t>();
  for (int pi = 0; pi < passes; pi++) {
    const bool first = pi == 0, last = pi + 1 == passes;
    const int shift = first ? 0 : 32 + 8 * pi;
    if (first) rs_hist_kernel<true><<<g, b, 0, ctx->stream>>>(in, n, shift, nblocks, hist->as<uint32_t>());
    else rs_hist_kernel<false><<<g, b, 0, ctx->stream>>>(in, n, shift, nblocks, hist->as<uint32_t>());
    SQ_HIP(hipGetLastError());
    exclusive_scan_u32(ctx, hist->as<uint32_t>(), 256 * nblocks, nullptr, offs->as<uint32_t>(), total->as<uint64_t>());
    if (first && last)
      rs_scatter_kernel<RS_PAIR, RS_PAIR, true><<<g, b, 0, ctx->stream>>>(in, nullptr, n, shift, nblocks, offs->as<uint32_t>(), nullptr, perm, 0, 0);
    else if (first)
      rs_scatter_kernel<RS_PAIR, RS_PACKED, true><<<g, b, 0, ctx->stream>>>(in, nullptr, n, shift, nblocks, offs->as<uint32_t>(), out, nullptr, 0, 0);
    else if (last)
      rs_scatter_kernel<RS_PACKED, RS_PAIR><<<g, b, 0, ctx->stream>>>(in, nullptr, n, shift, nblocks, offs->as<uint32_t>(), nullptr, perm, 0, 0);
    else
      rs_scatter_kernel<RS_PACKED, RS_PACKED><<<g, b, 0, ctx->stream>>>(in, nullptr, n, shift, nblocks, offs->as<uint32_t>(), out, nullptr, 0, 0);
    SQ_HIP(hipGetLastError());
    in = out;
    out = (out == w0->as<uint64_t>() && w1) ? w1->as<uint64_t>() : w0->as<uint64_t>();
  }
}

}
```

Measured before the change: 97230 Mrows/s.

## Emit group results as packed 32-byte rows and fuse ordering gather into radix sort

For dense two-accumulator COUNT/SUM group-bys, the aggregation kernels now write key and both accumulators into one 32-byte row per group instead of separate key and accumulator columns. The final first-row ordering then fuses the gather of these rows into the last radix-sort scatter pass, replacing a separate perm write and gather kernel. The aim is fewer scattered global writes and one less pass over the 10M groups. It adds a padding word per row and an unpack fallback kernel when merging or when another ordering is required.

```diff
diff --git a/sqlrs_amd/csrc/agg_partition.hip b/sqlrs_amd/csrc/agg_partition.hip
--- a/sqlrs_amd/csrc/agg_partition.hip
+++ b/sqlrs_amd/csrc/agg_partition.hip
@@ -522,11 +522,21 @@
   }
 }
 
+__device__ __forceinline__ void store_group_row(uint64_t *__restrict__ grows, unsigned long long i, uint64_t key,
+                                                unsigned long long c0, unsigned long long c1) {
+  u64x2 lo, hi;
+  lo.x = key;
+  lo.y = c0;
+  hi.x = c1;
+  hi.y = 0ull;
+  *(u64x2 *)(grows + 4 * (size_t)i) = lo;
+  *(u64x2 *)(grows + 4 * (size_t)i + 2) = hi;
+}
 constexpr int SED_SLOTS = 16, SED_GROUPS = 16;
 __global__ __launch_bounds__(SED_SLOTS * SED_GROUPS) void split_emit_dense_kernel(
     SplitTables stb, const uint32_t *__restrict__ split_bucket, const uint32_t *__restrict__ chunk_lo, uint32_t nbuckets_split,
     uint32_t R, KeyPack kp, LdsAggParams prm, int n_acc, unsigned long long *out_count, uint64_t *__restrict__ gkey,
-    uint32_t *__restrict__ gfirst, uint64_t *__restrict__ gacc, int64_t gcap) {
+    uint32_t *__restrict__ gfirst, uint64_t *__restrict__ gacc, int64_t gcap, uint64_t *__restrict__ grows) {
   __shared__ unsigned int s_first[SED_GROUPS][SED_SLOTS];
   __shared__ unsigned long long s_acc[PART_MAX_ACC][SED_GROUPS][SED_SLOTS];
   const uint32_t tiles_per_bucket = (R + SED_SLOTS - 1) / SED_SLOTS;
@@ -581,16 +591,24 @@
   if (prm.partner_mult) mlt = prm.partner_mult[((uint64_t)split_bucket[t] << kp.rbits) + s];
   unsigned long long base = atomicAdd(out_count, 1ull);
   if ((int64_t)base >= gcap) return;
-  gkey[base] = kp.kmin + ((uint64_t)split_bucket[t] << kp.rbits) + s;
   gfirst[base] = first;
-  for (int a = 0; a < n_acc; a++) gacc[(size_t)a * gcap + base] = prm.partner_mult ? acc_times(prm.code[a] & 7, acc[a], mlt) : acc[a];
+  for (int a = 0; a < n_acc; a++)
+    if (prm.partner_mult) acc[a] = acc_times(prm.code[a] & 7, acc[a], mlt);
+  const uint64_t key = kp.kmin + ((uint64_t)split_bucket[t] << kp.rbits) + s;
+  if (grows) {
+    store_group_row(grows, base, key, acc[0], acc[1]);
+    return;
+  }
+  gkey[base] = key;
+  for (int a = 0; a < n_acc; a++) gacc[(size_t)a * gcap + base] = acc[a];
 }
 
 template <int NV, bool JOIN, int NACC, int C0, int C1, bool REC = false>
 __global__ __launch_bounds__(DENSE_WG) void lds_agg_dense_kernel(
     LdsAggParams prm, const uint64_t *__restrict__ pk, const uint64_t *__restrict__ pv0,
     const uint32_t *__restrict__ work, unsigned long long *out_count, uint64_t *__restrict__ gkey,
-    uint32_t *__restrict__ gfirst, uint64_t *__restrict__ gacc, int64_t gcap, KeyPack kp, SplitTables stb) {
+    uint32_t *__restrict__ gfirst, uint64_t *__restrict__ gacc, int64_t gcap, KeyPack kp, SplitTables stb,
+    uint64_t *__restrict__ grows) {
   extern __shared__ __attribute__((aligned(16))) unsigned long long tab[];
   __shared__ unsigned int s_cnt;
   __shared__ unsigned long long s_base;
@@ -750,9 +768,16 @@
     unsigned int first = tfirst[s];
     if (first == 0xffffffffu) continue;
     if ((int64_t)base < gcap) {
-      gkey[base] = key0 + s;
       gfirst[base] = first;
       const unsigned int mlt = (JOIN && prm.partner_mult) ? prm.partner_mult[((uint64_t)b << kp.rbits) + s] : 1u;
+      if (grows) {
+        const unsigned long long c0 = tacc[s], c1 = tacc[(size_t)R + s];
+        store_group_row(grows, base, key0 + s, (JOIN && prm.partner_mult) ? acc_times(code_of(0) & 7, c0, mlt) : c0,
+                        (JOIN && prm.partner_mult) ? acc_times(code_of(1) & 7, c1, mlt) : c1);
+        base++;
+        continue;
+      }
+      gkey[base] = key0 + s;
 #pragma unroll
       for (int a = 0; a < PART_MAX_ACC; a++) {
         if (a >= n_acc) break;
@@ -782,7 +807,7 @@
 __global__ __launch_bounds__(DENSE_WG) void lds_agg_dense_slim_kernel(
     LdsAggParams prm, SlimBucketIn in, const uint32_t *__restrict__ work, unsigned long long *out_count,
     uint64_t *__restrict__ gkey, uint32_t *__restrict__ gfirst, uint64_t *__restrict__ gacc, int64_t gcap, KeyPack kp,
-    SplitTables stb) {
+    SplitTables stb, uint64_t *__restrict__ grows) {
   extern __shared__ __attribute__((aligned(16))) unsigned long long tab[];
   __shared__ unsigned int s_cnt, s_before, s_inside;
   __shared__ unsigned long long s_base;
@@ -1087,9 +1112,16 @@
     unsigned int first = tfirst[s];
     if (first == 0xffffffffu) continue;
     if ((int64_t)obase < gcap) {
-      gkey[obase] = key0 + s;
       gfirst[obase] = first;
       const unsigned int mlt = (JOIN && prm.partner_mult) ? prm.partner_mult[((uint64_t)b << kp.rbits) + s] : 1u;
+      if (grows) {
+        const unsigned long long c0 = tacc[s], c1 = tacc[(size_t)R + s];
+        store_group_row(grows, obase, key0 + s, (JOIN && prm.partner_mult) ? acc_times(code_of(0) & 7, c0, mlt) : c0,
+                        (JOIN && prm.partner_mult) ? acc_times(code_of(1) & 7, c1, mlt) : c1);
+        obase++;
+        continue;
+      }
+      gkey[obase] = key0 + s;
 #pragma unroll
       for (int a = 0; a < PART_MAX_ACC; a++) {
         if (a >= n_acc) break;
@@ -1436,10 +1468,17 @@
     split_init_kernel<<<dim3((unsigned)ceil_div(total, 256)), dim3(256), 0, ctx->stream>>>(stb, total, spec.n_acc, prm);
     SQ_HIP(hipGetLastError());
   }
-  out->gkey = ctx->alloc(8 * (size_t)gcap);
+  const bool rows_out = in.want_rows && dense && spec.n_acc == 2 && !in.key_validity;
   out->gfirst = ctx->alloc(4 * (size_t)gcap);
   out->gvalid = in.key_validity ? ctx->alloc((size_t)gcap) : nullptr;
-  out->gacc = ctx->alloc(8 * (size_t)gcap * (size_t)std::max(spec.n_acc, 1));
+  if (rows_out) {
+    out->grows = ctx->alloc(32 * (size_t)gcap);
+  } else {
+    out->gkey = ctx->alloc(8 * (size_t)gcap);
+    out->gacc = ctx->alloc(8 * (size_t)gcap * (size_t)std::max(spec.n_acc, 1));
+  }
+  uint64_t *const d_gkey = rows_out ? nullptr : out->gkey->as<uint64_t>(), *const d_gacc = rows_out ? nullptr : out->gacc->as<uint64_t>();
+  uint64_t *const d_grows = rows_out ? out->grows->as<uint64_t>() : nullptr;
   out->gcap = gcap;
   if (!out->ov_rows) out->ov_rows = ctx->alloc(4 * (size_t)std::max<int64_t>(n, 1));
   ctx->agg_route[pr.pack.kbits ? Ctx::AR_PACKED : Ctx::AR_UNPACKED]++;
@@ -1449,6 +1488,7 @@
   ctx->agg_route[Ctx::AR_JOIN] += join_mode;
   ctx->agg_route[Ctx::AR_JOIN_MULT] += prm.partner_mult != nullptr;
   ctx->agg_route[Ctx::AR_SPLIT] += nsplit > 0;
+  ctx->agg_route[Ctx::AR_GROUP_ROWS] += rows_out;
   {
     ProfScope ps(ctx, "lds_agg");
 #define SQ_LA(NV, FL, JN, NA, C0, C1, PK)                                                                        \
@@ -1502,8 +1542,8 @@
     if (blk) kfn = lds_agg_dense_slim_kernel<JN, NA, C0, C1, true>;                                             \
     allow_big_lds(ctx, kfn, 159 * 1024);                                                                                 \
     kfn<<<dim3(nwork), dim3(DENSE_WG), slds, ctx->stream>>>(prm, sb, dwork->as<uint32_t>(), ctr->as<unsigned long long>(), \
-                                                           out->gkey->as<uint64_t>(), out->gfirst->as<uint32_t>(), \
-                                                           out->gacc->as<uint64_t>(), gcap, pr.pack, stb);        \
+                                                           d_gkey, out->gfirst->as<uint32_t>(), \
+                                                           d_gacc, gcap, pr.pack, stb, d_grows);        \
     ctx->agg_route[blk ? Ctx::AR_SLIM_BLK : Ctx::AR_SLIM_RUNS]++;                                              \
     ctx->agg_route[Ctx::AR_INTERPRETED] += NA < 0;                                                             \
     launched = true;                                                                                           \
@@ -1520,7 +1560,7 @@
       if (nsplit) {
         split_emit_dense_kernel<<<dim3((unsigned)(nsplit * ceil_div((int64_t)nslots_h, SED_SLOTS))), dim3(SED_SLOTS * SED_GROUPS), 0, ctx->stream>>>(
             stb, dsplit->as<uint32_t>(), dchunk_lo->as<uint32_t>(), nsplit, cap, pr.pack, prm, spec.n_acc,
-            ctr->as<unsigned long long>(), out->gkey->as<uint64_t>(), out->gfirst->as<uint32_t>(), out->gacc->as<uint64_t>(), gcap);
+            ctr->as<unsigned long long>(), d_gkey, out->gfirst->as<uint32_t>(), d_gacc, gcap, d_grows);
       }
     } else if (dense) {
 #define SQ_LD(NV, JN, NA, C0, C1)                                                                              \
@@ -1530,8 +1570,8 @@
     allow_big_lds(ctx, kfn);                                                                                   \
     kfn<<<dim3(nwork), dim3(DENSE_WG), lds, ctx->stream>>>(                                                    \
         prm, pr.rec ? pr.rec->as<uint64_t>() : pk->as<uint64_t>(), pv0 ? pv0->as<uint64_t>() : nullptr, dwork->as<uint32_t>(), \
-        ctr->as<unsigned long long>(), out->gkey->as<uint64_t>(), out->gfirst->as<uint32_t>(),                 \
-        out->gacc->as<uint64_t>(), gcap, pr.pack, stb);                                                        \
+        ctr->as<unsigned long long>(), d_gkey, out->gfirst->as<uint32_t>(),                                    \
+        d_gacc, gcap, pr.pack, stb, d_grows);                                                                  \
     ctx->agg_route[Ctx::AR_DENSE]++;                                                                           \
     ctx->agg_route[Ctx::AR_INTERPRETED] += NA < 0;                                                             \
     launched = true;                                                                                           \
@@ -1555,7 +1595,7 @@
       if (nsplit) {
         split_emit_dense_kernel<<<dim3((unsigned)(nsplit * ceil_div((int64_t)nslots_h, SED_SLOTS))), dim3(SED_SLOTS * SED_GROUPS), 0, ctx->stream>>>(
             stb, dsplit->as<uint32_t>(), dchunk_lo->as<uint32_t>(), nsplit, cap, pr.pack, prm, spec.n_acc,
-            ctr->as<unsigned long long>(), out->gkey->as<uint64_t>(), out->gfirst->as<uint32_t>(), out->gacc->as<uint64_t>(), gcap);
+            ctr->as<unsigned long long>(), d_gkey, out->gfirst->as<uint32_t>(), d_gacc, gcap, d_grows);
       }
     }
     if (!launched && !pf && nvu == 1 && spec.n_acc <= 2) {
diff --git a/sqlrs_amd/csrc/agg_partition.hpp b/sqlrs_amd/csrc/agg_partition.hpp
--- a/sqlrs_amd/csrc/agg_partition.hpp
+++ b/sqlrs_amd/csrc/agg_partition.hpp
@@ -35,12 +35,14 @@
   const uint64_t *join_bits = nullptr;
   const uint32_t *join_mult = nullptr;
   RowFilter filter;
+  bool want_rows = false;
   bool exact_stats = false;
 };
 
 struct PartAggOutput {
   int64_t groups = 0, gcap = 0;
   BufP gkey, gfirst, gvalid, gvalid_bits, gacc;
+  BufP grows;
   BufP row_ids;
   uint64_t row_offset = 0;
   int64_t n_overflow = 0;
diff --git a/sqlrs_amd/csrc/common.hpp b/sqlrs_amd/csrc/common.hpp
--- a/sqlrs_amd/csrc/common.hpp
+++ b/sqlrs_amd/csrc/common.hpp
@@ -148,6 +148,8 @@
     AR_MERGE_GROUPS,
     AR_PENDING,
     AR_WIDE_PARTS,
+    AR_GROUP_ROWS,
+    AR_GROUP_ROWS_UNPACKED,
     AR_COUNT_
   };
   int64_t agg_route[AR_COUNT_] = {};
diff --git a/sqlrs_amd/csrc/ctx.hip b/sqlrs_amd/csrc/ctx.hip
--- a/sqlrs_amd/csrc/ctx.hip
+++ b/sqlrs_amd/csrc/ctx.hip
@@ -1222,7 +1222,7 @@
       "agg_part_dense", "agg_part_slim_runs", "agg_part_slim_blk", "agg_part_probe_spec", "agg_part_probe_generic",
       "agg_part_interpreted", "agg_part_packed", "agg_part_unpacked", "agg_part_flags", "agg_part_rec",
       "agg_part_in_place", "agg_part_join", "agg_part_join_mult", "agg_part_split", "agg_part_overflow_rows",
-      "agg_merge_groups", "agg_pending_deferred", "agg_wide_parts"};
+      "agg_merge_groups", "agg_pending_deferred", "agg_wide_parts", "agg_part_group_rows", "agg_group_rows_unpacked"};
   for (int r = 0; r < Ctx::AR_COUNT_; r++) {
     if (!ctx->agg_route[r]) continue;
     if (n < cap) {
diff --git a/sqlrs_amd/csrc/gather.hip b/sqlrs_amd/csrc/gather.hip
--- a/sqlrs_amd/csrc/gather.hip
+++ b/sqlrs_amd/csrc/gather.hip
@@ -274,6 +274,51 @@
   SQ_HIP(hipGetLastError());
   cols = std::move(outs);
   return true;
+}
+
+#ifndef GROUP_ROWS_FUSED_LAST_PASS
+#define GROUP_ROWS_FUSED_LAST_PASS 1
+#endif
+std::vector<DCol> order_group_rows(Ctx *ctx, const BufP &rows32, const uint32_t *first_rows, int64_t n, int bits,
+                                   const int32_t *dtypes) {
+  std::vector<DCol> outs(3);
+  uint64_t *o[3];
+  for (int i = 0; i < 3; i++) {
+    DCol &d = outs[(size_t)i];
+    d.dtype = dtypes[i];
+    d.length = n;
+    d.null_count = 0;
+    d.own_values = ctx->alloc(8 * (size_t)std::max<int64_t>(n, 1) + 16);
+    d.values = d.own_values->p;
+    o[i] = d.own_values->as<uint64_t>();
+  }
+#if GROUP_ROWS_FUSED_LAST_PASS
+  radix_sort_gather_rows_u32(ctx, first_rows, n, bits, rows32->as<uint64_t>(), o[0], o[1], o[2]);
+#else
+  if (n > 0) {
+    BufP perm = ctx->alloc(4 * (size_t)n);
+    radix_sort_index_u32(ctx, first_rows, n, bits, perm->as<uint32_t>());
+    gather_rows_kernel<3><<<dim3((unsigned)ceil_div(n, BLOCK * 4)), dim3(BLOCK), 0, ctx->stream>>>(
+        rows32->as<uint64_t>(), perm->as<uint32_t>(), n, o[0], o[1], o[2], nullptr);
+    SQ_HIP(hipGetLastError());
+  }
+#endif
+  return outs;
+}
+
+__global__ __launch_bounds__(BLOCK) void unpack_rows3_kernel(const uint64_t *__restrict__ rows, int64_t n, uint64_t *__restrict__ o0,
+                                                             uint64_t *__restrict__ o1, uint64_t *__restrict__ o2) {
+  const int64_t i = blockIdx.x * (int64_t)BLOCK + threadIdx.x;
+  if (i >= n) return;
+  const u64x2 a = *(const u64x2 *)(rows + 4 * (size_t)i);
+  o0[i] = a.x;
+  o1[i] = a.y;
+  o2[i] = rows[4 * (size_t)i + 2];
+}
+void unpack_rows3(Ctx *ctx, const uint64_t *rows32, int64_t n, uint64_t *o0, uint64_t *o1, uint64_t *o2) {
+  if (n <= 0) return;
+  unpack_rows3_kernel<<<dim3((unsigned)ceil_div(n, BLOCK)), dim3(BLOCK), 0, ctx->stream>>>(rows32, n, o0, o1, o2);
+  SQ_HIP(hipGetLastError());
 }
 
 __global__ void count_clear_kernel(const uint64_t *__restrict__ bits, int64_t rows, int64_t nwords,
diff --git a/sqlrs_amd/csrc/hashagg_op.hip b/sqlrs_amd/csrc/hashagg_op.hip
--- a/sqlrs_amd/csrc/hashagg_op.hip
+++ b/sqlrs_amd/csrc/hashagg_op.hip
@@ -256,9 +256,37 @@
   }
 }
 
+static DCol group_key_view(const PartAggOutput &po, int32_t dtype) {
+  DCol kv;
+  kv.dtype = dtype;
+  kv.length = po.groups;
+  kv.values = po.gkey->p;
+  kv.own_values = po.gkey;
+  if (po.gvalid_bits) {
+    kv.validity = po.gvalid_bits->as<uint64_t>();
+    kv.own_validity = po.gvalid_bits;
+    kv.null_count = -1;
+  }
+  return kv;
+}
+
+static void leave_group_rows(sqlrs_hash_agg *a, PendingGroups &pg) {
+  PartAggOutput &po = pg.po;
+  if (!po.grows) return;
+  Ctx *ctx = a->ctx;
+  ctx->agg_route[Ctx::AR_GROUP_ROWS_UNPACKED]++;
+  po.gkey = ctx->alloc(8 * (size_t)po.gcap);
+  po.gacc = ctx->alloc(8 * 2 * (size_t)po.gcap);
+  unpack_rows3(ctx, po.grows->as<uint64_t>(), po.groups, po.gkey->as<uint64_t>(), po.gacc->as<uint64_t>(),
+               po.gacc->as<uint64_t>() + (size_t)po.gcap);
+  po.grows = nullptr;
+  pg.keyvals.assign(1, group_key_view(po, pg.key_dtype));
+}
+
 static void merge_groups(sqlrs_hash_agg *a, PendingGroups &pg) {
   Ctx *ctx = a->ctx;
   ctx->agg_route[Ctx::AR_MERGE_GROUPS]++;
+  leave_group_rows(a, pg);
   PartAggOutput &po = pg.po;
   NKeys gk;
   gk.rows = po.groups;
@@ -316,6 +344,19 @@
   int64_t G = po.groups;
   DBatch o;
   o.rows = G;
+  if (po.grows && a->any_order) leave_group_rows(a, pg);
+  if (po.grows) {
+    ProfScope ps(ctx, "agg_order_groups");
+    int bits = 1;
+    while (bits < 32 && (1ull << bits) <= (uint64_t)std::max<int64_t>(a->rows_seen, 1)) bits++;
+    int32_t dts[3] = {pg.key_dtype, 0, 0};
+    for (size_t i = 0; i < 2; i++)
+      dts[1 + pg.acc_of_agg[i]] = a->aggs[i].func == SQLRS_AGG_COUNT ? SQLRS_INT64 : a->aggs[i].return_dtype;
+    std::vector<DCol> by_word = order_group_rows(ctx, po.grows, po.gfirst->as<uint32_t>(), G, bits, dts);
+    o.cols.push_back(by_word[0]);
+    for (size_t i = 0; i < 2; i++) o.cols.push_back(by_word[(size_t)(1 + pg.acc_of_agg[i])]);
+    return o;
+  }
   for (const DCol &k : pg.keyvals) o.cols.push_back(k);
   auto cell = [&](int acc) { return po.gacc->as<uint64_t>() + (size_t)acc * (size_t)po.gcap; };
   for (size_t i = 0; i < a->aggs.size(); i++) {
@@ -548,6 +589,14 @@
         if (rf) pin.filter = *rf;
         PartAggOutput po;
         flush_pending(a);
+        if (a->st.ngroups == 0 && !a->any_order && !nk.validity && nk.exact && kcols.size() == 1 && kcols[0].dtype == nk.dtype &&
+            (nk.dtype == SQLRS_INT64 || nk.dtype == SQLRS_FLOAT64) && a->aggs.size() == 2 && spec.n_acc == 2 &&
+            acc_of_agg[0] != acc_of_agg[1]) {
+          bool raw = true;
+          for (const AggSpec &s : a->aggs) raw &= s.func == SQLRS_AGG_COUNT || s.func == SQLRS_AGG_SUM;
+          for (size_t k = 0; k < pcols.size(); k++) raw &= pin.val_validity[k] == nullptr;
+          pin.want_rows = raw;
+        }
         bool part_ok = partitioned_preaggregate(ctx, spec, pin, (uint64_t)a->rows_seen, &po);
         if (!part_ok && po.retry_exact) {
           pin.exact_stats = true;
@@ -566,19 +615,10 @@
             pg.col_nullable.push_back(pin.val_validity[k] != nullptr);
             pg.col_dtype.push_back(pcols[k].dtype);
           }
-          if (nk.exact && kcols.size() == 1 && (kcols[0].dtype == SQLRS_INT64 || kcols[0].dtype == SQLRS_FLOAT64) &&
-              kcols[0].dtype == nk.dtype) {
-            DCol kv;
-            kv.dtype = kcols[0].dtype;
-            kv.length = po.groups;
-            kv.values = po.gkey->p;
-            kv.own_values = po.gkey;
-            if (po.gvalid_bits) {
-              kv.validity = po.gvalid_bits->as<uint64_t>();
-              kv.own_validity = po.gvalid_bits;
-              kv.null_count = -1;
-            }
-            pg.keyvals.push_back(kv);
+          if (po.grows) {
+          } else if (nk.exact && kcols.size() == 1 && (kcols[0].dtype == SQLRS_INT64 || kcols[0].dtype == SQLRS_FLOAT64) &&
+                     kcols[0].dtype == nk.dtype) {
+            pg.keyvals.push_back(group_key_view(po, kcols[0].dtype));
           } else {
             for (const DCol &kc : kcols)
               pg.keyvals.push_back(gather_column(ctx, kc, po.gfirst->p, false, nullptr, po.groups));
diff --git a/sqlrs_amd/csrc/prims.hpp b/sqlrs_amd/csrc/prims.hpp
--- a/sqlrs_amd/csrc/prims.hpp
+++ b/sqlrs_amd/csrc/prims.hpp
@@ -30,6 +30,9 @@
 DCol gather_column(Ctx *ctx, const DCol &src, const void *idx, bool idx_is_u64,
                    const uint64_t *idx_validity, int64_t n);
 bool gather_columns_packed(Ctx *ctx, std::vector<DCol> &cols, int64_t src_rows, const uint32_t *idx, int64_t n);
+std::vector<DCol> order_group_rows(Ctx *ctx, const BufP &rows32, const uint32_t *first_rows, int64_t n, int bits,
+                                   const int32_t *dtypes);
+void unpack_rows3(Ctx *ctx, const uint64_t *rows32, int64_t n, uint64_t *o0, uint64_t *o1, uint64_t *o2);
 DCol concat_columns(Ctx *ctx, const std::vector<const DCol *> &parts);
 DCol copy_column(Ctx *ctx, const DCol &c);
 void sort_perm_by_utf8(Ctx *ctx, const DCol &c, const uint64_t *valid, int desc, uint32_t *perm, uint64_t *keys,
@@ -54,6 +57,8 @@
 void radix_sort_pairs(Ctx *ctx, uint64_t *keys, uint32_t *vals, int64_t n, int begin_bit,
                       int end_bit, bool keys_below_end_bit = false);
 void radix_sort_index_u32(Ctx *ctx, const uint32_t *keys, int64_t n, int bits, uint32_t *perm);
+void radix_sort_gather_rows_u32(Ctx *ctx, const uint32_t *first_rows, int64_t n, int bits, const uint64_t *rows32,
+                                uint64_t *out0, uint64_t *out1, uint64_t *out2);
 void iota_u32(Ctx *ctx, uint32_t *out, int64_t n);
 bool order_fast(Ctx *ctx, const DCol &key, int desc, const DCol *carry, int64_t n, DCol *key_out, DCol *carry_out,
                 BufP *perm, bool want_perm, bool *in_order = nullptr);
diff --git a/sqlrs_amd/csrc/sort.hip b/sqlrs_amd/csrc/sort.hip
--- a/sqlrs_amd/csrc/sort.hip
+++ b/sqlrs_amd/csrc/sort.hip
@@ -29,14 +29,18 @@
   if (threadIdx.x < 256) hist[(int64_t)threadIdx.x * nblocks + blockIdx.x] = h[threadIdx.x];
 }
 
-enum { RS_PAIR = 0, RS_PACKED = 1 };
+enum { RS_PAIR = 0, RS_PACKED = 1, RS_ROWS = 2 };
+struct RsRowsOut {
+  const uint64_t *rows = nullptr;
+  uint64_t *out0 = nullptr, *out1 = nullptr, *out2 = nullptr;
+};
 template <int IN, int OUT, bool KEY32 = false>
 __global__ __launch_bounds__(RS_WG) void rs_scatter_kernel(
     const uint64_t *__restrict__ keys, const uint32_t *__restrict__ vals, int64_t n, int shift,
     int64_t nblocks, const uint32_t *__restrict__ offsets, uint64_t *__restrict__ keys_out,
-    uint32_t *__restrict__ vals_out, int key_lo, uint64_t key_const) {
+    uint32_t *__restrict__ vals_out, int key_lo, uint64_t key_const, RsRowsOut ro) {
   __shared__ uint64_t skey[RS_TILE];
-  __shared__ uint32_t sval[(IN == RS_PAIR && OUT == RS_PAIR) ? RS_TILE : 1];
+  __shared__ uint32_t sval[(IN == RS_PAIR && OUT != RS_PACKED) ? RS_TILE : 1];
   __shared__ uint32_t wcnt[RS_WAVES][256];
   __shared__ uint32_t dstart[256];
   __shared__ int64_t gbase[256];
@@ -108,10 +112,32 @@
     const uint32_t p = dstart[d] + wcnt[w][d] + rnk[j];
     if (IN == RS_PAIR && OUT == RS_PACKED) skey[p] = ((k[j] >> key_lo) << 32) | v[j];
     else skey[p] = k[j];
-    if (IN == RS_PAIR && OUT == RS_PAIR) sval[p] = v[j];
+    if (IN == RS_PAIR && OUT != RS_PACKED) sval[p] = v[j];
   }
   __syncthreads();
   const uint32_t len = (uint32_t)min<int64_t>(RS_TILE, n - tbase);
+  if (OUT == RS_ROWS) {
+    int64_t g[RS_ITEMS];
+    u64x2 ra[RS_ITEMS], rb[RS_ITEMS];
+#pragma unroll
+    for (int j = 0; j < RS_ITEMS; j++) {
+      const uint32_t p = j * RS_WG + threadIdx.x;
+      const uint32_t q = p < len ? p : 0u;
+      const uint64_t kk = skey[q];
+      const uint32_t src = IN == RS_PACKED ? (uint32_t)kk : sval[q];
+      g[j] = p < len ? gbase[(uint32_t)(kk >> shift) & 255u] + p : -1;
+      ra[j] = *(const u64x2 *)(ro.rows + 4 * (size_t)src);
+      rb[j] = *(const u64x2 *)(ro.rows + 4 * (size_t)src + 2);
+    }
+#pragma unroll
+    for (int j = 0; j < RS_ITEMS; j++) {
+      if (g[j] < 0) continue;
+      ro.out0[g[j]] = ra[j].x;
+      ro.out1[g[j]] = ra[j].y;
+      ro.out2[g[j]] = rb[j].x;
+    }
+    return;
+  }
 #pragma unroll
   for (int j = 0; j < RS_ITEMS; j++) {
     const uint32_t p = j * RS_WG + threadIdx.x;
@@ -206,13 +232,13 @@
                        total->as<uint64_t>());
     dim3 g((unsigned)nblocks), b(RS_WG);
     if (!in_packed && !out_packed)
-      rs_scatter_kernel<RS_PAIR, RS_PAIR><<<g, b, 0, ctx->stream>>>(ka, va, n, shift, nblocks, offs->as<uint32_t>(), kb, vb, 0, 0);
+      rs_scatter_kernel<RS_PAIR, RS_PAIR><<<g, b, 0, ctx->stream>>>(ka, va, n, shift, nblocks, offs->as<uint32_t>(), kb, vb, 0, 0, RsRowsOut{});
     else if (!in_packed)
-      rs_scatter_kernel<RS_PAIR, RS_PACKED><<<g, b, 0, ctx->stream>>>(ka, va, n, shift, nblocks, offs->as<uint32_t>(), kb, vb, key_lo, key_const);
+      rs_scatter_kernel<RS_PAIR, RS_PACKED><<<g, b, 0, ctx->stream>>>(ka, va, n, shift, nblocks, offs->as<uint32_t>(), kb, vb, key_lo, key_const, RsRowsOut{});
     else if (out_packed)
-      rs_scatter_kernel<RS_PACKED, RS_PACKED><<<g, b, 0, ctx->stream>>>(ka, va, n, eff, nblocks, offs->as<uint32_t>(), kb, vb, key_lo, key_const);
+      rs_scatter_kernel<RS_PACKED, RS_PACKED><<<g, b, 0, ctx->stream>>>(ka, va, n, eff, nblocks, offs->as<uint32_t>(), kb, vb, key_lo, key_const, RsRowsOut{});
     else
-      rs_scatter_kernel<RS_PACKED, RS_PAIR><<<g, b, 0, ctx->stream>>>(ka, va, n, eff, nblocks, offs->as<uint32_t>(), kb, vb, key_lo, key_const);
+      rs_scatter_kernel<RS_PACKED, RS_PAIR><<<g, b, 0, ctx->stream>>>(ka, va, n, eff, nblocks, offs->as<uint32_t>(), kb, vb, key_lo, key_const, RsRowsOut{});
     SQ_HIP(hipGetLastError());
     std::swap(ka, kb);
     std::swap(va, vb);
@@ -223,7 +249,7 @@
   }
 }
 
-void radix_sort_index_u32(Ctx *ctx, const uint32_t *keys, int64_t n, int bits, uint32_t *perm) {
+static void sort_index_u32(Ctx *ctx, const uint32_t *keys, int64_t n, int bits, uint32_t *perm, const RsRowsOut &ro) {
   if (n <= 0) return;
   if (n > 0xffffffffll) fail(SQLRS_ERR_INTERNAL, "radix sort: more than 2^32 rows");
   ProfScope ps(ctx, "radix_sort");
@@ -242,18 +268,34 @@
     else rs_hist_kernel<false><<<g, b, 0, ctx->stream>>>(in, n, shift, nblocks, hist->as<uint32_t>());
     SQ_HIP(hipGetLastError());
     exclusive_scan_u32(ctx, hist->as<uint32_t>(), 256 * nblocks, nullptr, offs->as<uint32_t>(), total->as<uint64_t>());
-    if (first && last)
-      rs_scatter_kernel<RS_PAIR, RS_PAIR, true><<<g, b, 0, ctx->stream>>>(in, nullptr, n, shift, nblocks, offs->as<uint32_t>(), nullptr, perm, 0, 0);
+    if (last && ro.rows) {
+      if (first) rs_scatter_kernel<RS_PAIR, RS_ROWS, true><<<g, b, 0, ctx->stream>>>(in, nullptr, n, shift, nblocks, offs->as<uint32_t>(), nullptr, nullptr, 0, 0, ro);
+      else rs_scatter_kernel<RS_PACKED, RS_ROWS><<<g, b, 0, ctx->stream>>>(in, nullptr, n, shift, nblocks, offs->as<uint32_t>(), nullptr, nullptr, 0, 0, ro);
+    } else if (first && last)
+      rs_scatter_kernel<RS_PAIR, RS_PAIR, true><<<g, b, 0, ctx->stream>>>(in, nullptr, n, shift, nblocks, offs->as<uint32_t>(), nullptr, perm, 0, 0, RsRowsOut{});
     else if (first)
-      rs_scatter_kernel<RS_PAIR, RS_PACKED, true><<<g, b, 0, ctx->stream>>>(in, nullptr, n, shift, nblocks, offs->as<uint32_t>(), out, nullptr, 0, 0);
+      rs_scatter_kernel<RS_PAIR, RS_PACKED, true><<<g, b, 0, ctx->stream>>>(in, nullptr, n, shift, nblocks, offs->as<uint32_t>(), out, nullptr, 0, 0, RsRowsOut{});
     else if (last)
-      rs_scatter_kernel<RS_PACKED, RS_PAIR><<<g, b, 0, ctx->stream>>>(in, nullptr, n, shift, nblocks, offs->as<uint32_t>(), nullptr, perm, 0, 0);
+      rs_scatter_kernel<RS_PACKED, RS_PAIR><<<g, b, 0, ctx->stream>>>(in, nullptr, n, shift, nblocks, offs->as<uint32_t>(), nullptr, perm, 0, 0, RsRowsOut{});
     else
-      rs_scatter_kernel<RS_PACKED, RS_PACKED><<<g, b, 0, ctx->stream>>>(in, nullptr, n, shift, nblocks, offs->as<uint32_t>(), out, nullptr, 0, 0);
+      rs_scatter_kernel<RS_PACKED, RS_PACKED><<<g, b, 0, ctx->stream>>>(in, nullptr, n, shift, nblocks, offs->as<uint32_t>(), out, nullptr, 0, 0, RsRowsOut{});
     SQ_HIP(hipGetLastError());
     in = out;
     out = (out == w0->as<uint64_t>() && w1) ? w1->as<uint64_t>() : w0->as<uint64_t>();
   }
 }
-
-}
+void radix_sort_index_u32(Ctx *ctx, const uint32_t *keys, int64_t n, int bits, uint32_t *perm) {
+  sort_index_u32(ctx, keys, n, bits, perm, RsRowsOut{});
+}
+
+void radix_sort_gather_rows_u32(Ctx *ctx, const uint32_t *first_rows, int64_t n, int bits, const uint64_t *rows32,
+                                uint64_t *out0, uint64_t *out1, uint64_t *out2) {
+  RsRowsOut ro;
+  ro.rows = rows32;
+  ro.out0 = out0;
+  ro.out1 = out1;
+  ro.out2 = out2;
+  sort_index_u32(ctx, first_rows, n, bits, nullptr, ro);
+}
+
+}
```

New measurement: 97180 Mrows/s. Within noise of the previous version (-0.1%).
